# paurrodri/DuplexUMIConsensusReads

Hardware: AMD Instinct MI355X
Metric: consensus bases/sec (whole node) + SSCS kernel HBM GB/s vs peak, 1/2/4/8 GPUs (higher is better)
Workload: dtype f64

## Files before the change

### duplexumiconsensusreads_amd/_lib.py

```python
from __future__ import annotations

import ctypes
import os

import numpy as np

from .batch import DcrBatch, DcrOut, DcrReadInfo, OutArrays, PackedBatch
from .params import ConsensusParams, DcrParams, build_dcr_params

HERE = os.path.dirname(os.path.abspath(__file__))
LIB_PATH = os.environ.get("DCR_LIB", os.path.join(HERE, "libdcr.so"))

EXPORTS = {
    "dcr_abi_version": (ctypes.c_int, []),
    "dcr_last_error": (ctypes.c_char_p, []),
    "dcr_create": (ctypes.c_void_p, [ctypes.c_int, ctypes.c_void_p]),
    "dcr_destroy": (None, [ctypes.c_void_p]),
    "dcr_set_params": (ctypes.c_int, [ctypes.c_void_p, ctypes.c_void_p]),
    "dcr_set_options": (ctypes.c_int, [ctypes.c_void_p, ctypes.c_int]),
    "dcr_reserve": (ctypes.c_int, [ctypes.c_void_p, ctypes.c_void_p]),
    "dcr_stream": (ctypes.c_void_p, [ctypes.c_void_p]),
    "dcr_run_batch": (ctypes.c_int, [ctypes.c_void_p, ctypes.c_void_p, ctypes.c_void_p, ctypes.c_void_p]),
    "dcr_run_batch_host": (ctypes.c_int, [ctypes.c_void_p, ctypes.c_void_p, ctypes.c_void_p,
                                          ctypes.c_void_p]),
    "dcr_sync": (ctypes.c_int, [ctypes.c_void_p]),
    "dcr_read_info_host": (ctypes.c_int, [ctypes.c_void_p, ctypes.c_void_p, ctypes.c_int64]),
    "dcr_last_timing": (ctypes.c_int, [ctypes.c_void_p, ctypes.c_void_p]),
    "dcr_last_kernel_timing": (ctypes.c_int, [ctypes.c_void_p, ctypes.c_void_p]),
    "dcr_host_alloc": (ctypes.c_void_p, [ctypes.c_size_t]),
    "dcr_host_free": (None, [ctypes.c_void_p]),
    "dcr_submit": (ctypes.c_int, [ctypes.c_void_p, ctypes.c_int, ctypes.c_void_p, ctypes.c_void_p, ctypes.c_void_p,
                                  ctypes.c_void_p]),
    "dcr_wait": (ctypes.c_int, [ctypes.c_void_p, ctypes.c_int]),
    "dcr_submit_write": (ctypes.c_int, [ctypes.c_void_p, ctypes.c_int, ctypes.c_void_p, ctypes.c_void_p,
                                        ctypes.c_void_p]),
    "dcr_wait_write": (ctypes.c_int, [ctypes.c_void_p, ctypes.c_int, ctypes.c_void_p]),
    "dcr_submit_write_ss": (ctypes.c_int, [ctypes.c_void_p, ctypes.c_int, ctypes.c_void_p, ctypes.c_void_p,
                                           ctypes.c_void_p, ctypes.c_void_p, ctypes.c_void_p]),
    "dcr_wait_write_ss": (ctypes.c_int, [ctypes.c_void_p, ctypes.c_int, ctypes.c_void_p, ctypes.c_void_p]),
    "dcr_slot_fetch": (ctypes.c_int, [ctypes.c_void_p, ctypes.c_int, ctypes.c_int, ctypes.c_int64, ctypes.c_int64,
                                      ctypes.c_void_p]),
    "dcr_set_filter": (ctypes.c_int, [ctypes.c_void_p, ctypes.c_void_p]),
    "dcr_slot_filter_out": (ctypes.c_int, [ctypes.c_void_p, ctypes.c_int, ctypes.c_void_p]),
    "dcr_set_base_filter": (ctypes.c_int, [ctypes.c_void_p, ctypes.c_void_p]),
    "dcr_set_base_tags": (ctypes.c_int, [ctypes.c_void_p, ctypes.c_int]),
    "dcr_set_metrics": (ctypes.c_int, [ctypes.c_void_p, ctypes.c_int]),
    "dcr_slot_metrics_out": (ctypes.c_int, [ctypes.c_void_p, ctypes.c_int, ctypes.c_void_p]),
    "dcr_set_base_metrics": (ctypes.c_int, [ctypes.c_void_p, ctypes.c_int]),
    "dcr_slot_base_metrics_out": (ctypes.c_int, [ctypes.c_void_p, ctypes.c_int, ctypes.c_void_p]),
    "dcr_set_mate_overlap": (ctypes.c_int, [ctypes.c_void_p, ctypes.c_int]),
    "dcr_slot_overlap_out": (ctypes.c_int, [ctypes.c_void_p, ctypes.c_int, ctypes.c_void_p]),
    "dcr_set_allele_sites": (ctypes.c_int, [ctypes.c_void_p, ctypes.c_void_p, ctypes.c_int64, ctypes.c_int]),
    "dcr_allele_counts_fetch": (ctypes.c_int, [ctypes.c_void_p, ctypes.c_void_p]),
    "dcr_inflater_create": (ctypes.c_void_p, [ctypes.c_int]),
    "dcr_inflater_destroy": (None, [ctypes.c_void_p]),
    "dcr_inflater_hook": (ctypes.c_int, [ctypes.c_void_p, ctypes.c_void_p]),
    "dcr_inflater_run": (ctypes.c_int, [ctypes.c_void_p, ctypes.c_void_p, ctypes.c_int64, ctypes.c_void_p,
                                        ctypes.c_int32, ctypes.c_void_p, ctypes.c_int64]),
    "dcr_inflater_last": (ctypes.c_int, [ctypes.c_void_p, ctypes.c_void_p, ctypes.c_void_p]),
    "dcr_inflater_totals": (ctypes.c_int, [ctypes.c_void_p, ctypes.c_void_p, ctypes.c_int]),
    "dcr_inflate_stream_open": (ctypes.c_void_p, [ctypes.c_void_p, ctypes.c_void_p]),
    "dcr_inflate_stream_add": (ctypes.c_int, [ctypes.c_void_p, ctypes.c_void_p, ctypes.c_int32, ctypes.c_int32]),
    "dcr_inflate_stream_fetch": (ctypes.c_int, [ctypes.c_void_p, ctypes.c_int64, ctypes.c_int64, ctypes.c_void_p]),
    "dcr_inflate_stream_close": (None, [ctypes.c_void_p]),
}

KERNELS = ("k_recmeta<ss>", "k_consensus_fast<ss>", "k_consensus_exact<ss>", "k_consensus_general<ss>",
           "k_recmeta<ds>", "k_consensus_fast<ds>", "k_consensus_exact<ds>", "k_consensus_general<ds>")

_lib = None

READ_INFO_DTYPE = np.dtype([("seq_start", "<i8"), ("len", "<i4"), ("n_cig", "<i4"), ("status", "<i4"),
                            ("has_ins", "<i4")])
assert READ_INFO_DTYPE.itemsize == ctypes.sizeof(DcrReadInfo)


class DcrError(RuntimeError):
    pass


def load():
    global _lib
    if _lib is None:
        try:
            import torch
        except ImportError:
            pass
        path = os.environ.get("DCR_LIB_PATH", LIB_PATH)
        if not os.path.exists(path):
            raise DcrError(f"{path} not built — run __graft_entry__.build() (hipcc --offload-arch=gfx950)")
        lib = ctypes.CDLL(path)
        for name, (res, args) in EXPORTS.items():
            fn = getattr(lib, name)
            fn.restype = res
            fn.argtypes = args
        if lib.dcr_abi_version() != 1:
            raise DcrError("libdcr.so ABI mismatch")
        _lib = lib
    return _lib


def _check(rc):
    if rc != 0:
        raise DcrError(f"libdcr error {rc}: {load().dcr_last_error().decode()}")


class Context:

    def __init__(self, params: ConsensusParams = ConsensusParams(), device: int = 0, want_info: bool = False):
        lib = load()
        self.params = params
        self._p = build_dcr_params(params)
        self.device = device
        self._ctx = lib.dcr_create(device, ctypes.byref(self._p))
        if not self._ctx:
            raise DcrError(f"dcr_create failed: {lib.dcr_last_error().decode()}")
        self.want_info = want_info
        self.filter = None
        self.metrics = False
        self.base_tags = False
        self.base_metrics = False
        self.mate_overlap = 0
        self.allele_sites = 0
        if want_info:
            _check(lib.dcr_set_options(self._ctx, 1))

    def close(self):
        if getattr(self, "_ctx", None):
            load().dcr_destroy(self._ctx)
            self._ctx = None

    def __del__(self):
        try:
            self.close()
        except Exception:
            pass

    def set_params(self, params: ConsensusParams):
        self.params = params
        self._p = build_dcr_params(params)
        _check(load().dcr_set_params(self._ctx, ctypes.byref(self._p)))

    def set_filter(self, flt):
        if flt == self.filter:
            return
        s = flt.as_struct() if flt is not None else None
        _check(load().dcr_set_filter(self._ctx, ctypes.byref(s) if s is not None else None))
        b = flt.as_base_struct() if flt is not None else None
        _check(load().dcr_set_base_filter(self._ctx, ctypes.byref(b) if b is not None else None))
        self.filter = flt

    def set_metrics(self, on):
        if bool(on) == self.metrics:
            return
        _check(load().dcr_set_metrics(self._ctx, 1 if on else 0))
        self.metrics = bool(on)

    def set_base_tags(self, on):
        if bool(on) == self.base_tags:
            return
        _check(load().dcr_set_base_tags(self._ctx, 1 if on else 0))
        self.base_tags = bool(on)

    def set_base_metrics(self, on):
        if bool(on) == self.base_metrics:
            return
        _check(load().dcr_set_base_metrics(self._ctx, 1 if on else 0))
        self.base_metrics = bool(on)

    def set_mate_overlap(self, mode):
        mode = int(mode or 0)
        if mode == self.mate_overlap:
            return
        _check(load().dcr_set_mate_overlap(self._ctx, mode))
        self.mate_overlap = mode

    def set_allele_sites(self, keys, min_base_quality=0):
        n = 0 if keys is None else len(keys)
        if n == 0:
            if self.allele_sites:
                _check(load().dcr_set_allele_sites(self._ctx, None, 0, 0))
            self.allele_sites = 0
            return
        keys = np.ascontiguousarray(keys, np.int64)
        _check(load().dcr_set_allele_sites(self._ctx, keys.ctypes.data, n, int(min_base_quality)))
        self.allele_sites = n

    def allele_counts(self):
        from .params import ALLELE_COLS
        out = np.zeros((max(self.allele_sites, 1), ALLELE_COLS), np.uint64)
        _check(load().dcr_allele_counts_fetch(self._ctx, out.ctypes.data))
        return out[:self.allele_sites]

    @property
    def stream(self):
        return load().dcr_stream(self._ctx)

    def run_host(self, packed: PackedBatch, want_info=None):
        ss = OutArrays(4 * packed.n_fam, packed.ss_cols)
        ds = OutArrays(2 * packed.n_fam, packed.ds_cols)
        b = packed.as_struct()
        so, do = ss.as_struct(), ds.as_struct()
        _check(load().dcr_run_batch_host(self._ctx, ctypes.byref(b), ctypes.byref(so), ctypes.byref(do)))
        if want_info is None:
            want_info = self.want_info
        info = self.read_info(packed.n_reads) if want_info else None
        return ss, ds, info

    def read_info(self, n):
        arr = np.zeros(max(n, 1), dtype=READ_INFO_DTYPE)
        _check(load().dcr_read_info_host(self._ctx, arr.ctypes.data, n))
        return {k: arr[k][:n].copy() for k in READ_INFO_DTYPE.names}

    def reserve(self, batch_struct: DcrBatch):
        _check(load().dcr_reserve(self._ctx, ctypes.byref(batch_struct)))

    def run_device(self, batch_struct: DcrBatch, ss: DcrOut, ds: DcrOut):
        _check(load().dcr_run_batch(self._ctx, ctypes.byref(batch_struct), ctypes.byref(ss), ctypes.byref(ds)))

    def sync(self):
        _check(load().dcr_sync(self._ctx))

    def last_timing(self):
        ms = (ctypes.c_float * 4)()
        _check(load().dcr_last_timing(self._ctx, ms))
        return dict(prep=ms[0], single_strand=ms[1], duplex=ms[2], total=ms[3])

    def last_kernel_timing(self):
        ms = (ctypes.c_float * len(KERNELS))()
        _check(load().dcr_last_kernel_timing(self._ctx, ms))
        return dict(zip(KERNELS, ms))


BGZF_MEMBER_DTYPE = np.dtype([("in_off", "<i8"), ("out_off", "<i8"), ("in_len", "<u4"), ("isize", "<u4"),
                              ("crc", "<u4"), ("pad", "<u4")])


class InflateHook(ctypes.Structure):
    _fields_ = [("user", ctypes.c_void_p), ("run", ctypes.c_void_p), ("host_alloc", ctypes.c_void_p),
                ("host_free", ctypes.c_void_p), ("stream_open", ctypes.c_void_p), ("stream_add", ctypes.c_void_p),
                ("stream_fetch", ctypes.c_void_p), ("stream_close", ctypes.c_void_p)]


def bgzf_members(data) -> tuple:
    buf = memoryview(data)
    out, p, o = [], 0, 0
    while p < len(buf):
        if bytes(buf[p:p + 4]) != b"\x1f\x8b\x08\x04":
            raise ValueError(f"not a BGZF block at {p}")
        xlen = int.from_bytes(buf[p + 10:p + 12], "little")
        bsize, q = None, p + 12
        while q + 4 <= p + 12 + xlen:
            slen = int.from_bytes(buf[q + 2:q + 4], "little")
            if bytes(buf[q:q + 2]) == b"BC" and slen == 2:
                bsize = int.from_bytes(buf[q + 4:q + 6], "little") + 1
            q += 4 + slen
        if bsize is None:
            raise ValueError("BGZF block without BC field")
        crc = int.from_bytes(buf[p + bsize - 8:p + bsize - 4], "little")
        isize = int.from_bytes(buf[p + bsize - 4:p + bsize], "little")
        out.append((p + 12 + xlen, o, bsize - 12 - xlen - 8, isize, crc, 0))
        o += isize
        p += bsize
    return np.array(out, dtype=BGZF_MEMBER_DTYPE), o


class Inflater:

    def __init__(self, device: int = 0):
        lib = load()
        self.device = device
        self._h = lib.dcr_inflater_create(device)
        if not self._h:
            raise DcrError(f"dcr_inflater_create failed: {lib.dcr_last_error().decode()}")

    @property
    def handle(self):
        return self._h

    def hook(self) -> InflateHook:
        h = InflateHook()
        _check(load().dcr_inflater_hook(self._h, ctypes.byref(h)))
        return h

    def run(self, data, members, out_bytes):
        src = np.frombuffer(data, np.uint8) if not isinstance(data, np.ndarray) else data
        m = np.ascontiguousarray(members, dtype=BGZF_MEMBER_DTYPE)
        out = np.zeros(max(out_bytes, 1), np.uint8)
        rc = load().dcr_inflater_run(self._h, src.ctypes.data, src.nbytes, m.ctypes.data, len(m), out.ctypes.data,
                                     out_bytes)
        if rc < 0:
            raise DcrError(f"dcr_inflater_run: {load().dcr_last_error().decode()}")
        return rc, out[:out_bytes]

    def last(self):
        ms, n = ctypes.c_float(), ctypes.c_int32()
        _check(load().dcr_inflater_last(self._h, ctypes.byref(ms), ctypes.byref(n)))
        return ms.value, n.value

    def totals(self, reset=False):
        out = (ctypes.c_double * 4)()
        _check(load().dcr_inflater_totals(self._h, out, int(reset)))
        return {"kernel_ms": out[0], "runs": int(out[1]), "members": int(out[2]), "bytes": int(out[3])}

    def close(self):
        if getattr(self, "_h", None):
            load().dcr_inflater_destroy(self._h)
            self._h = None

    def __del__(self):
        try:
            self.close()
        except Exception:
            pass


def backend(ctx: Context):
    def run(packed, params):
        if params != ctx.params:
            ctx.set_params(params)
        return ctx.run_host(packed)
    return run
```

### duplexumiconsensusreads_amd/csrc/dcr_inflate.hip

```cpp
#include <hip/hip_runtime.h>

#include <condition_variable>
#include <cstring>
#include <deque>
#include <mutex>
#include <thread>
#include <string>
#include <unordered_map>
#include <vector>

#include "../../include/dcr_inflate.h"
#include "dcr_deflate.h"
#include "dcr_internal.h"
#include "dcr_span_stream.h"

#ifndef DINF_STAMP
#define DINF_STAMP 0
#endif

namespace dinf {

struct IStamp {
    uint64_t t = 0;
    uint32_t acc[8] = {0, 0, 0, 0, 0, 0, 0, 0};
    uint32_t cnt[8] = {0, 0, 0, 0, 0, 0, 0, 0};
    __device__ __forceinline__ void start() {
        if (DINF_STAMP) t = __builtin_amdgcn_s_memtime();
    }
    __device__ __forceinline__ void lap(int k) {
        if (DINF_STAMP) {
            const uint64_t now = __builtin_amdgcn_s_memtime();
            acc[k] += (uint32_t)(now - t);
            t = now;
        }
    }
    __device__ __forceinline__ void count(int k, uint32_t v = 1) {
        if (DINF_STAMP) cnt[k] += v;
    }
};

#ifndef DINF_WG_PER_CU
#define DINF_WG_PER_CU 16
#endif
#ifndef DINF_RING
#define DINF_RING 4096
#endif
#ifndef DINF_LB
#define DINF_LB 9
#endif
constexpr int kW = 64;
constexpr int kLB = DINF_LB;
constexpr int kDB = 8;
constexpr int kCB = 7;
constexpr uint32_t kRing = DINF_RING;
constexpr uint32_t kRM = kRing - 1;
constexpr uint32_t kPiece = kRing / 2;
constexpr uint32_t kStripe = kPiece / kW;
static_assert((kRing & (kRing - 1)) == 0 && kRing >= 2048, "ring: a power of two");
static_assert(kPiece + 322 + 320 <= kRing, "the ring holds the unwritten bytes");
constexpr int kPad = 1024;

enum : uint32_t { K_LIT = 0, K_PAIR = 1, K_LEN = 2, K_EOB = 3, K_DIST = 4, K_BAD = 7 };

enum : uint8_t { ST_OK = 0, ST_STREAM = 1, ST_SIZE = 2, ST_CRC = 3, ST_GUARD = 4 };
constexpr uint32_t kGuard = 1u << 21;

struct alignas(16) WaveLds {
    uint32_t lit[1 << kLB];
    uint32_t dist[1 << kDB];
    uint8_t ring[kRing];
    uint32_t crc_tab[256];
    uint16_t lsym[288], dsym[32];
    uint16_t lcnt[16], dcnt[16];
    uint8_t lens[320];
    uint8_t cl_lens[20];
};

struct Args {
    const uint8_t *in;
    uint8_t *out;
    const dcr_bgzf_member *m;
    uint8_t *status;
    uint32_t *dbg;
    int32_t n;
    uint32_t x8n_piece;
};

__device__ __forceinline__ uint32_t uni(uint32_t v) { return __builtin_amdgcn_readfirstlane(v); }
__device__ __forceinline__ int lane_id() { return (int)(threadIdx.x & (kW - 1)); }
__device__ __forceinline__ uint32_t lane_read(uint32_t v, uint32_t l) {
    return (uint32_t)__builtin_amdgcn_readlane((int)v, (int)l);
}

__device__ __forceinline__ uint32_t lit_entry(uint32_t sym) {
    if (sym < 256) return (K_LIT << 5) | (sym << 8);
    if (sym == 256) return K_EOB << 5;
    if (sym < 286) return (K_LEN << 5) | ((uint32_t)dfl::kLenExtra[sym - 257] << 8) | ((uint32_t)dfl::kLenBase[sym - 257] << 16);
    return K_BAD << 5;
}
__device__ __forceinline__ uint32_t dist_entry(uint32_t sym) {
    if (sym < 30) return (K_DIST << 5) | ((uint32_t)dfl::kDistExtra[sym] << 8) | ((uint32_t)dfl::kDistBase[sym] << 16);
    return K_BAD << 5;
}

template <int TB, int KIND>
__device__ __noinline__ bool build_table(const uint8_t *lens, int n, uint32_t *tab, uint16_t *cnt_out, uint16_t *sym_out) {
    const int lane = lane_id();
    const uint64_t lt = (1ull << lane) - 1;
    uint32_t mycnt = 0;
    for (int c0 = 0; c0 < n; c0 += kW) {
        const int i = c0 + lane;
        const uint32_t l = i < n ? lens[i] : 0;
#pragma unroll
        for (int L = 1; L <= 15; ++L) {
            const uint32_t k = (uint32_t)__popcll(__ballot(l == (uint32_t)L));
            if (lane == L) mycnt += k;
        }
    }
    if (lane == 0) mycnt = 0;
    uint32_t kr = lane >= 1 && lane <= 15 ? mycnt << (15 - lane) : 0;
    for (int d = 32; d >= 1; d >>= 1) kr += __shfl_xor(kr, d, kW);
    kr = uni(kr);
    if (kr > 32768u) return false;
    if (kr != 32768u) {
        const bool one_bit = kr == 16384u && lane_read(mycnt, 1) == 1;
        if (KIND == 2 || !(one_bit || (KIND == 1 && kr == 0))) return false;
    }
    uint32_t offs = 0, first = 0;
#pragma unroll
    for (int l = 1; l <= 15; ++l) {
        const uint32_t cl = lane_read(mycnt, l);
        if (l < lane && lane < 16) {
            offs += cl;
            first += cl << (lane - l);
        }
    }
    if (lane < 16) cnt_out[lane] = (uint16_t)mycnt;
    uint32_t run = offs;
    for (int c0 = 0; c0 < n; c0 += kW) {
        const int i = c0 + lane;
        const uint32_t l = i < n ? lens[i] : 0;
#pragma unroll
        for (int L = 1; L <= 15; ++L) {
            const uint64_t m = __ballot(l == (uint32_t)L);
            const uint32_t base = lane_read(run, L);
            if (l == (uint32_t)L) sym_out[base + __popcll(m & lt)] = (uint16_t)i;
            if (lane == L) run += (uint32_t)__popcll(m);
        }
    }
    uint32_t fL[TB + 1], cL[TB + 1], oL[TB + 1];
#pragma unroll
    for (int L = 1; L <= TB; ++L) {
        fL[L] = lane_read(first, L);
        cL[L] = lane_read(mycnt, L);
        oL[L] = lane_read(offs, L);
    }
    bool any_long = false;
    {
        uint32_t longer = 0;
        for (int l = TB + 1; l <= 15; ++l) longer += lane_read(mycnt, l);
        any_long = longer != 0;
    }
    for (int e = lane; e < (1 << TB); e += kW) {
        const uint32_t c = __builtin_bitreverse32((uint32_t)e) >> (32 - TB);
        uint32_t ent = any_long ? 0u : (K_BAD << 5);
#pragma unroll
// ... 221 lines not shown
                d.nb -= n;
                const uint32_t sym = e >> 8;
                uint32_t rep = 1, val = sym;
                if (sym == 16) {
                    if (i == 0) { st = ST_STREAM; break; }
                    val = uni(s.lens[i - 1]);
                    rep = 3 + getbits(d, 2);
                } else if (sym == 17) {
                    val = 0;
                    rep = 3 + getbits(d, 3);
                } else if (sym == 18) {
                    val = 0;
                    rep = 11 + getbits(d, 7);
                }
                if (i + rep > total) { st = ST_STREAM; break; }
                for (uint32_t r = lane; r < rep; r += kW) s.lens[i + r] = (uint8_t)val;
                i += rep;
            }
            if (st != ST_OK) break;
            if (uni(s.lens[256]) == 0) { st = ST_STREAM; break; }
            if (!uni(build_table<kLB, 0>(s.lens, (int)hlit, s.lit, s.lcnt, s.lsym))) { st = ST_STREAM; break; }
            if (!uni(build_table<kDB, 1>(s.lens + hlit, (int)hdist, s.dist, s.dcnt, s.dsym))) { st = ST_STREAM; break; }
        }
        sp.lap(0);
        for (;;) {
            if (d.nb < 32) refill(d);
            uint32_t e = uni(s.lit[(uint32_t)d.bb & ((1u << kLB) - 1)]);
            uint32_t n = e & 31;
            if (n == 0) {
                const int sym = slow_decode(d, s.lcnt, s.lsym, n);
                if (sym < 0) { st = ST_STREAM; break; }
                e = lit_entry((uint32_t)sym) | n;
            }
            d.bb >>= n;
            d.nb -= n;
            const uint32_t kind = (e >> 5) & 7;
            if (kind == K_LIT || kind == K_PAIR) {
                sp.count(kind == K_PAIR ? 1 : 0);
                o.lbuf = lane == (int)o.nlit ? (e >> 8) & 0xff : o.lbuf;
                ++o.nlit;
                if (kind == K_PAIR) {
                    o.lbuf = lane == (int)o.nlit ? (e >> 16) & 0xff : o.lbuf;
                    ++o.nlit;
                }
                if (o.nlit >= kW - 1) {
                    if (o.opos + o.nlit > o.isize) { st = ST_SIZE; break; }
                    sp.lap(1);
                    flush_lits(s, o);
                    keep_room(o, a, lsh);
                    sp.lap(4);
                }
                continue;
            }
            if (kind == K_EOB) break;
            if (kind != K_LEN) { st = ST_STREAM; break; }
            const uint32_t ex = (e >> 8) & 7;
            const uint32_t len = (e >> 16) + ((uint32_t)d.bb & ((1u << ex) - 1));
            d.bb >>= ex;
            d.nb -= ex;
            if (d.nb < 32) refill(d);
            uint32_t de = uni(s.dist[(uint32_t)d.bb & ((1u << kDB) - 1)]);
            uint32_t dn = de & 31;
            if (dn == 0) {
                const int sym = slow_decode(d, s.dcnt, s.dsym, dn);
                if (sym < 0) { st = ST_STREAM; break; }
                de = dist_entry((uint32_t)sym) | dn;
            }
            if (((de >> 5) & 7) != K_DIST) { st = ST_STREAM; break; }
            d.bb >>= dn;
            d.nb -= dn;
            const uint32_t dex = (de >> 8) & 15;
            const uint32_t dist = (de >> 16) + ((uint32_t)d.bb & ((1u << dex) - 1));
            d.bb >>= dex;
            d.nb -= dex;
            if (o.opos + o.nlit + len > o.isize) { st = ST_SIZE; break; }
            sp.lap(2);
            sp.count(2);
            sp.count(3, len);
            flush_lits(s, o);
            if (dist > o.opos) { st = ST_STREAM; break; }
            if (dist >= kW && dist <= kRingDist) {
                for (uint32_t c0 = 0; c0 < len; c0 += kW) {
                    const uint32_t i = c0 + lane;
                    const uint8_t v = s.ring[(o.opos - dist + i) & kRM];
                    s.ring[(o.opos + i) & kRM] = v;
                }
            } else if (dist < kW) {
                const float rd = __builtin_amdgcn_rcpf((float)dist);
                const uint32_t rep = (uint32_t)lane - dist * (uint32_t)(((float)lane + 0.5f) * rd);
                const uint32_t step = dist * uni((uint32_t)(((float)kW + 0.5f) * rd));
                const uint8_t v = s.ring[(o.opos - dist + rep) & kRM];
                for (uint32_t c0 = 0; c0 < len; c0 += step) s.ring[(o.opos + c0 + lane) & kRM] = v;
            } else {
                asm volatile("s_waitcnt vmcnt(0)" ::: "memory");
                for (uint32_t c0 = 0; c0 < len; c0 += kW) {
                    const uint32_t i = c0 + lane;
                    if (i < len) s.ring[(o.opos + i) & kRM] = o.g[o.opos - dist + i];
                }
            }
            o.opos += len;
            sp.lap(3);
            keep_room(o, a, lsh);
            sp.lap(4);
        }
        sp.lap(1);
        if (st != ST_OK) break;
        if (o.opos + o.nlit > o.isize) { st = ST_SIZE; break; }
        flush_lits(s, o);
        keep_room(o, a, lsh);
    }
    if (st == ST_OK && (bits_used(d) + 7) / 8 > M.in_len) st = ST_STREAM;
    if (st == ST_OK && o.opos != o.isize) st = ST_SIZE;
    if (st == ST_OK) {
        while (o.gpos < o.opos) {
            const uint32_t m = min(kPiece, o.opos - o.gpos);
            o.crc = uni(write_piece(o.g, o.gpos, m, o.crc, lsh, a.x8n_piece));
            o.gpos += m;
        }
        const uint32_t crc = ~(dfl::multmodp(dfl::x8nmodp(o.isize), 0xffffffffu) ^ o.crc);
        if (o.isize == 0) {
            if (M.crc != 0) st = ST_CRC;
        } else if (crc != M.crc) {
            st = ST_CRC;
        }
    }
    sp.lap(5);
    if (DINF_STAMP && lane == 0 && a.dbg) {
        for (int k = 0; k < 6; ++k) a.dbg[16 * mi + k] = sp.acc[k];
        for (int k = 0; k < 4; ++k) a.dbg[16 * mi + 8 + k] = sp.cnt[k];
        a.dbg[16 * mi + 12] = guard;
        a.dbg[16 * mi + 13] = o.opos;
    }
    if (lane == 0) {
        a.status[mi] = st;
        if (a.dbg && !DINF_STAMP) {
            a.dbg[4 * mi] = st | where << 8;
            a.dbg[4 * mi + 1] = bits_used(d);
            a.dbg[4 * mi + 2] = o.opos;
            a.dbg[4 * mi + 3] = guard;
        }
    }
}

__global__ __launch_bounds__(64) void k_inflate(Args a) {
    WaveLds &s = *reinterpret_cast<WaveLds *>(smem);
    const int lane = lane_id();
    for (int i = lane; i < 256; i += kW) s.crc_tab[i] = dfl::crc_byte((uint32_t)i);
    const uint32_t lsh = dfl::x8nmodp(kPiece - kStripe * (uint32_t)(lane + 1));
    for (int mi = (int)blockIdx.x; mi < a.n; mi += (int)gridDim.x) inflate_one(a, s, mi, lsh);
}

}

struct InflSlots {
    static constexpr int kSlots = 4;
    uint8_t *d_in[kSlots] = {}, *d_out[kSlots] = {}, *d_st[kSlots] = {};
    dcr_bgzf_member *d_m[kSlots] = {};
    size_t cap_in[kSlots] = {}, cap_out[kSlots] = {}, cap_m[kSlots] = {}, cap_dst[kSlots] = {};
    uint8_t *h_stage[kSlots] = {}, *h_st[kSlots] = {};
    size_t cap_stage[kSlots] = {}, cap_hst[kSlots] = {};
    hipStream_t s_k = nullptr, s_out = nullptr;
    bool busy = false;
    void release() {
        for (int i = 0; i < kSlots; ++i) {
            if (d_in[i]) (void)hipFree(d_in[i]);
            if (d_out[i]) (void)hipFree(d_out[i]);
            if (d_st[i]) (void)hipFree(d_st[i]);
            if (d_m[i]) (void)hipFree(d_m[i]);
            if (h_stage[i]) (void)hipHostFree(h_stage[i]);
            if (h_st[i]) (void)hipHostFree(h_st[i]);
        }
        if (s_k) (void)hipStreamDestroy(s_k);
        if (s_out) (void)hipStreamDestroy(s_out);
    }
};

struct dcr_inflater {
    int device = 0;
    int grid_cap = 1 << 30;
    int n_cu = 1;
    hipStream_t stream = nullptr;
    hipEvent_t ev0 = nullptr, ev1 = nullptr;
    uint8_t *d_in = nullptr, *d_out = nullptr, *d_st = nullptr;
    dcr_bgzf_member *d_m = nullptr;
    uint32_t *d_dbg = nullptr;
    size_t cap_in = 0, cap_out = 0, cap_m = 0, cap_dbg = 0;
    size_t cap_st = 0;
    dinf::Args base{};
    float last_ms = 0;
    int32_t last_n = 0;
    double tot[4] = {0, 0, 0, 0};
    double stamp[16] = {};
    struct InflSlots *slots = nullptr;
    std::mutex mu;
    std::unordered_multimap<size_t, void *> free_host;
    std::unordered_map<void *, size_t> live_host;
};

namespace {
template <class T>
hipError_t grow(T *&p, size_t &cap, size_t n) {
    if (n <= cap) return hipSuccess;
    if (p) (void)hipFree(p);
    p = nullptr;
    cap = 0;
    hipError_t e = hipMalloc((void **)&p, n * sizeof(T));
    if (e == hipSuccess) cap = n;
    return e;
}
int hip_fail(hipError_t e, const char *what) {
    return dcr::set_error(DCR_EHIP, std::string(what) + ": " + hipGetErrorString(e));
}
}

extern "C" {

dcr_inflater *dcr_inflater_create(int device) {
    int n = 0;
    if (hipGetDeviceCount(&n) != hipSuccess || device < 0 || device >= n) {
        dcr::set_error(DCR_ENODEV, "dcr_inflater_create: no such device");
        return nullptr;
    }
    hipDeviceProp_t prop;
    if (hipGetDeviceProperties(&prop, device) != hipSuccess || std::strncmp(prop.gcnArchName, "gfx950", 6) != 0) {
        dcr::set_error(DCR_ENODEV, "dcr_inflater_create: not a gfx950 device");
        return nullptr;
    }
    auto *h = new dcr_inflater;
    h->device = device;
    if (hipSetDevice(device) != hipSuccess || hipStreamCreateWithFlags(&h->stream, hipStreamNonBlocking) != hipSuccess ||
        hipEventCreate(&h->ev0) != hipSuccess || hipEventCreate(&h->ev1) != hipSuccess ||
        hipFuncSetAttribute((const void *)dinf::k_inflate, hipFuncAttributeMaxDynamicSharedMemorySize,
                            (int)sizeof(dinf::WaveLds)) != hipSuccess) {
        dcr::set_error(DCR_EHIP, "dcr_inflater_create: HIP setup failed");
        dcr_inflater_destroy(h);
        return nullptr;
    }
    h->base.x8n_piece = dfl::x8nmodp(dinf::kPiece);
    h->n_cu = std::max(1, prop.multiProcessorCount);
    if (DINF_WG_PER_CU > 0) h->grid_cap = DINF_WG_PER_CU * h->n_cu;
    return h;
}

void dcr_inflater_destroy(dcr_inflater *h) {
    if (!h) return;
    (void)hipSetDevice(h->device);
    if (h->stream) (void)hipStreamSynchronize(h->stream);
    if (h->d_in) (void)hipFree(h->d_in);
    if (h->d_out) (void)hipFree(h->d_out);
    if (h->d_st) (void)hipFree(h->d_st);
    if (h->d_m) (void)hipFree(h->d_m);
    if (h->d_dbg) (void)hipFree(h->d_dbg);
    for (auto &kv : h->free_host) (void)hipHostFree(kv.second);
    for (auto &kv : h->live_host) (void)hipHostFree(kv.first);
    if (h->slots) {
        h->slots->release();
        delete h->slots;
    }
    if (h->ev0) (void)hipEventDestroy(h->ev0);
    if (h->ev1) (void)hipEventDestroy(h->ev1);
    if (h->stream) (void)hipStreamDestroy(h->stream);
    delete h;
}

int dcr_inflater_run(dcr_inflater *h, const uint8_t *in, int64_t in_bytes, const dcr_bgzf_member *m, int32_t n,
                     uint8_t *out, int64_t out_bytes) {
    if (!h || n < 0 || in_bytes < 0 || out_bytes < 0 || (n && (!in || !m || !out)))
        return -dcr::set_error(DCR_EARG, "dcr_inflater_run: bad arguments");
    if (n == 0) return 0;
    for (int32_t i = 0; i < n; ++i)
        if (m[i].in_off < 0 || m[i].in_off + (int64_t)m[i].in_len > in_bytes || m[i].isize > 65536 ||
            m[i].out_off < 0 || m[i].out_off + (int64_t)m[i].isize > out_bytes)
            return -dcr::set_error(DCR_EARG, "dcr_inflater_run: member " + std::to_string(i) + " outside the buffers");
    std::lock_guard<std::mutex> g(h->mu);
    hipError_t e;
    if ((e = hipSetDevice(h->device)) != hipSuccess) return -hip_fail(e, "hipSetDevice");
    if ((e = grow(h->d_in, h->cap_in, (size_t)in_bytes + dinf::kPad)) != hipSuccess ||
        (e = grow(h->d_out, h->cap_out, (size_t)out_bytes + 16)) != hipSuccess ||
        (e = grow(h->d_m, h->cap_m, (size_t)n)) != hipSuccess ||
        (e = grow(h->d_st, h->cap_st, (size_t)n)) != hipSuccess ||
        (e = grow(h->d_dbg, h->cap_dbg, (size_t)n * (DINF_STAMP ? 16 : 4))) != hipSuccess)
        return -hip_fail(e, "dcr_inflater_run: device buffers");
    std::vector<uint8_t> st((size_t)n);
    hipStream_t s = h->stream;
    if ((e = hipMemcpyAsync(h->d_in, in, (size_t)in_bytes, hipMemcpyHostToDevice, s)) != hipSuccess ||
        (e = hipMemcpyAsync(h->d_m, m, (size_t)n * sizeof(dcr_bgzf_member), hipMemcpyHostToDevice, s)) != hipSuccess)
        return -hip_fail(e, "dcr_inflater_run: upload");
    dinf::Args a = h->base;
    a.in = h->d_in;
    a.out = h->d_out;
    a.m = h->d_m;
    a.status = h->d_st;
    a.dbg = h->d_dbg;
    a.n = n;
    (void)hipEventRecord(h->ev0, s);
    hipLaunchKernelGGL(dinf::k_inflate, dim3((unsigned)std::min(n, h->grid_cap)), dim3(64), sizeof(dinf::WaveLds), s,
                       a);
    if ((e = hipGetLastError()) != hipSuccess) return -hip_fail(e, "k_inflate launch");
    (void)hipEventRecord(h->ev1, s);
    if ((e = hipMemcpyAsync(out, h->d_out, (size_t)out_bytes, hipMemcpyDeviceToHost, s)) != hipSuccess ||
        (e = hipMemcpyAsync(st.data(), h->d_st, (size_t)n, hipMemcpyDeviceToHost, s)) != hipSuccess)
        return -hip_fail(e, "dcr_inflater_run: download");
    if ((e = hipStreamSynchronize(s)) != hipSuccess) return -hip_fail(e, "dcr_inflater_run: sync");
    (void)hipEventElapsedTime(&h->last_ms, h->ev0, h->ev1);
    h->last_n = n;
    h->tot[0] += h->last_ms;
    h->tot[1] += 1;
    h->tot[2] += n;
    h->tot[3] += (double)out_bytes;
    if (DINF_STAMP) {
        std::vector<uint32_t> dbg((size_t)n * 16);
        (void)hipMemcpy(dbg.data(), h->d_dbg, dbg.size() * 4, hipMemcpyDeviceToHost);
        for (int32_t i = 0; i < n; ++i)
            for (int k = 0; k < 16; ++k) h->stamp[k] += dbg[(size_t)i * 16 + k];
    }
    for (int32_t i = 0; i < n; ++i)
        if (st[(size_t)i] != dinf::ST_OK) {
            uint32_t dbg[4] = {0, 0, 0, 0};
            (void)hipMemcpy(dbg, h->d_dbg + 4 * (size_t)i, sizeof(dbg), hipMemcpyDeviceToHost);
            const int k = st[(size_t)i];
            dcr::set_error(DCR_EARG, "BGZF member " + std::to_string(i) +
                                         (k == dinf::ST_CRC    ? ": CRC32 mismatch"
                                          : k == dinf::ST_SIZE ? ": ISIZE mismatch"
                                          : k == dinf::ST_GUARD ? ": decoder iteration guard"
                                                                : ": invalid deflate stream") +
                                         " (loop " + std::to_string(dbg[0] >> 8) + ", input bits " +
                                         std::to_string(dbg[1]) + ", output " + std::to_string(dbg[2]) +
                                         ", iterations " + std::to_string(dbg[3]) + ")");
            return i + 1;
        }
    return 0;
}

int dcr_inflater_last(dcr_inflater *h, float *kernel_ms, int32_t *n_members) {
    if (!h) return dcr::set_error(DCR_EARG, "dcr_inflater_last: null inflater");
    if (kernel_ms) *kernel_ms = h->last_ms;
    if (n_members) *n_members = h->last_n;
    return 0;
}

int dcr_inflater_totals(dcr_inflater *h, double *out4, int reset) {
    if (!h || !out4) return dcr::set_error(DCR_EARG, "dcr_inflater_totals: null argument");
    std::lock_guard<std::mutex> g(h->mu);
    for (int i = 0; i < 4; ++i) out4[i] = h->tot[i];
    if (reset)
        for (double &t : h->tot) t = 0;
    return 0;
}

extern "C" int dcr_inflater_stamps(dcr_inflater *h, double *out16, int reset) {
    if (!h || !out16) return dcr::set_error(DCR_EARG, "dcr_inflater_stamps: null argument");
    std::lock_guard<std::mutex> g(h->mu);
    for (int i = 0; i < 16; ++i) out16[i] = h->stamp[i];
    if (reset)
        for (double &t : h->stamp) t = 0;
    return DINF_STAMP;
}

namespace {
hipError_t pinned_grow(uint8_t *&p, size_t &cap, size_t n) {
    if (n <= cap) return hipSuccess;
    if (p) (void)hipHostFree(p);
    p = nullptr;
    cap = 0;
    hipError_t e = hipHostMalloc((void **)&p, n, hipHostMallocDefault);
    if (e == hipSuccess) cap = n;
    return e;
}

struct HipSpanBackend {
    using Event = hipEvent_t;
    dcr_inflater *h;
    InflSlots &S;
    bool new_events(Event &start, Event &done) {
        return hipEventCreateWithFlags(&done, hipEventBlockingSync) == hipSuccess &&
               hipEventCreate(&start) == hipSuccess;
    }
    void free_events(Event &start, Event &done) {
        if (start) (void)hipEventDestroy(start);
        if (done) (void)hipEventDestroy(done);
        start = done = nullptr;
    }
    bool ensure(int slot, size_t nin, size_t nout, int32_t n) {
        (void)hipSetDevice(h->device);
        return pinned_grow(S.h_stage[slot], S.cap_stage[slot], nin + 16) == hipSuccess &&
               pinned_grow(S.h_st[slot], S.cap_hst[slot], (size_t)n) == hipSuccess &&
               grow(S.d_in[slot], S.cap_in[slot], nin + dinf::kPad) == hipSuccess &&
               grow(S.d_out[slot], S.cap_out[slot], nout + 16) == hipSuccess &&
               grow(S.d_m[slot], S.cap_m[slot], (size_t)n) == hipSuccess &&
               grow(S.d_st[slot], S.cap_dst[slot], (size_t)n) == hipSuccess;
    }
    uint8_t *stage(int slot) { return S.h_stage[slot]; }
    bool launch(int slot, const dcr_bgzf_member *rel, int32_t n, size_t nin, Event start, Event done) {
        dinf::Args a = h->base;
        a.in = S.d_in[slot];
        a.out = S.d_out[slot];
        a.m = S.d_m[slot];
        a.status = S.d_st[slot];
        a.dbg = nullptr;
        a.n = n;
        if (hipMemcpyAsync(S.d_in[slot], S.h_stage[slot], nin, hipMemcpyHostToDevice, S.s_k) != hipSuccess ||
            hipMemcpyAsync(S.d_m[slot], rel, (size_t)n * sizeof(dcr_bgzf_member), hipMemcpyHostToDevice, S.s_k) !=
                hipSuccess ||
            hipEventRecord(start, S.s_k) != hipSuccess)
            return false;
        hipLaunchKernelGGL(dinf::k_inflate, dim3((unsigned)std::min(n, h->grid_cap)), dim3(64), sizeof(dinf::WaveLds),
                           S.s_k, a);
        return hipGetLastError() == hipSuccess &&
               hipMemcpyAsync(S.h_st[slot], S.d_st[slot], (size_t)n, hipMemcpyDeviceToHost, S.s_k) == hipSuccess &&
               hipEventRecord(done, S.s_k) == hipSuccess;
    }
    bool wait(Event start, Event done, float *ms) {
        if (hipEventSynchronize(done) != hipSuccess) return false;
        if (ms) {
            *ms = 0;
            (void)hipEventElapsedTime(ms, start, done);
        }
        return true;
    }
    const uint8_t *status(int slot) { return S.h_st[slot]; }
    bool copy_out(uint8_t *dst, int slot, int64_t off, int64_t n) {
        return hipMemcpyAsync(dst, S.d_out[slot] + off, (size_t)n, hipMemcpyDeviceToHost, S.s_out) == hipSuccess;
    }
    bool sync_out() { return hipStreamSynchronize(S.s_out) == hipSuccess; }
    void drain() {
        (void)hipSetDevice(h->device);
        if (S.s_k) (void)hipStreamSynchronize(S.s_k);
        if (S.s_out) (void)hipStreamSynchronize(S.s_out);
    }
    void account(float ms, int32_t members, int64_t bytes) {
        std::lock_guard<std::mutex> g(h->mu);
        if (members) {
            h->tot[0] += ms;
            h->tot[1] += 1;
            h->tot[2] += members;
        }
        h->tot[3] += (double)bytes;
    }
    void error(const std::string &msg) { dcr::set_error(DCR_EARG, msg); }
};
}

static_assert(InflSlots::kSlots == dcr_span::kSlots, "one device slot per protocol slot");

struct dcr_inflate_stream {
    HipSpanBackend be;
    dcr_span::Stream<HipSpanBackend> s;
    dcr_inflate_stream(dcr_inflater *h, const uint8_t *file) : be{h, *h->slots}, s(be, file) {}
};

extern "C" dcr_inflate_stream *dcr_inflate_stream_open(dcr_inflater *h, const uint8_t *file) {
    if (!h || !file) {
        dcr::set_error(DCR_EARG, "dcr_inflate_stream_open: bad arguments");
        return nullptr;
    }
    {
        std::lock_guard<std::mutex> g(h->mu);
        if (!h->slots) h->slots = new InflSlots;
        if (h->slots->busy) {
            dcr::set_error(DCR_EARG, "dcr_inflate_stream_open: the inflater's stream is in use");
            return nullptr;
        }
        h->slots->busy = true;
    }
    InflSlots &S = *h->slots;
    (void)hipSetDevice(h->device);
    if ((!S.s_k && hipStreamCreateWithFlags(&S.s_k, hipStreamNonBlocking) != hipSuccess) ||
        (!S.s_out && hipStreamCreateWithFlags(&S.s_out, hipStreamNonBlocking) != hipSuccess)) {
        std::lock_guard<std::mutex> g(h->mu);
        S.busy = false;
        dcr::set_error(DCR_EHIP, "dcr_inflate_stream_open: HIP setup failed");
        return nullptr;
    }
    auto *st = new dcr_inflate_stream(h, file);
    st->s.start();
    return st;
}

extern "C" int dcr_inflate_stream_add(dcr_inflate_stream *st, const dcr_bgzf_member *m, int32_t n, int32_t last) {
    if (!st || n < 0 || (n && !m)) return dcr::set_error(DCR_EARG, "dcr_inflate_stream_add: bad arguments");
    for (int32_t i = 0; i < n; ++i)
        if (m[i].isize > 65536 || m[i].in_off < 0 || m[i].out_off < 0)
            return dcr::set_error(DCR_EARG, "dcr_inflate_stream_add: member out of range");
    return st->s.add(m, n, last);
}

extern "C" int dcr_inflate_stream_fetch(dcr_inflate_stream *st, int64_t out_off, int64_t n, uint8_t *dst) {
    if (!st || n < 0 || (n && !dst)) return -1;
    (void)hipSetDevice(st->be.h->device);
    return st->s.fetch(out_off, n, dst);
}

extern "C" void dcr_inflate_stream_close(dcr_inflate_stream *st) {
    if (!st) return;
    st->s.close();
    dcr_inflater *h = st->be.h;
    delete st;
    std::lock_guard<std::mutex> g(h->mu);
    h->slots->busy = false;
}

static void *hook_stream_open(void *u, const uint8_t *file) {
    return dcr_inflate_stream_open((dcr_inflater *)u, file);
}
static int hook_stream_add(void *s, const dcr_bgzf_member *m, int32_t n, int32_t last) {
    return dcr_inflate_stream_add((dcr_inflate_stream *)s, m, n, last);
}
static int hook_stream_fetch(void *s, int64_t off, int64_t n, uint8_t *dst) {
    return dcr_inflate_stream_fetch((dcr_inflate_stream *)s, off, n, dst);
}
static void hook_stream_close(void *s) { dcr_inflate_stream_close((dcr_inflate_stream *)s); }

static int hook_run(void *u, const uint8_t *in, int64_t in_bytes, const dcr_bgzf_member *m, int32_t n, uint8_t *out,
                    int64_t out_bytes) {
    const int r = dcr_inflater_run((dcr_inflater *)u, in, in_bytes, m, n, out, out_bytes);
    return r < 0 ? -1 : r;
}
static void *hook_alloc(void *u, size_t bytes) {
    auto *h = (dcr_inflater *)u;
    std::lock_guard<std::mutex> g(h->mu);
    auto it = h->free_host.find(bytes);
    void *p = nullptr;
    if (it != h->free_host.end()) {
        p = it->second;
        h->free_host.erase(it);
    } else {
        (void)hipSetDevice(h->device);
        if (hipHostMalloc(&p, bytes, hipHostMallocDefault) != hipSuccess) return nullptr;
    }
    h->live_host[p] = bytes;
    return p;
}
static void hook_free(void *u, void *p) {
    auto *h = (dcr_inflater *)u;
    std::lock_guard<std::mutex> g(h->mu);
    auto it = h->live_host.find(p);
    if (it == h->live_host.end()) return;
    h->free_host.emplace(it->second, p);
    h->live_host.erase(it);
}

int dcr_inflater_hook(dcr_inflater *h, dcr_inflate_hook *hook) {
    if (!h || !hook) return dcr::set_error(DCR_EARG, "dcr_inflater_hook: null argument");
    hook->user = h;
    hook->run = hook_run;
    hook->host_alloc = hook_alloc;
    hook->host_free = hook_free;
    hook->stream_open = hook_stream_open;
    hook->stream_add = hook_stream_add;
    hook->stream_fetch = hook_stream_fetch;
    hook->stream_close = hook_stream_close;
    return 0;
}

}
```

### duplexumiconsensusreads_amd/csrc/dcr_ingest.cpp

```cpp
#include <zlib.h>
#include <tmmintrin.h>
#include <sys/stat.h>

#include <cctype>
#include <cmath>
#include <chrono>
#include <condition_variable>
#include <deque>
#include <mutex>
#include <thread>
#include <cstdio>
#include <cstdlib>
#include <cstring>
#include <memory>
#include <string>
#include <vector>

#include "../../include/dcr_io.h"
#include "../../include/dcr_inflate.h"
#include "dcr_host.h"

using namespace dcrh;

namespace {

thread_local std::string g_err;

int fail(int code, const std::string &m) {
    g_err = m;
    return code;
}

struct TLDecomp {
    libdeflate_decompressor *d = nullptr;
    ~TLDecomp() {
        if (d) libdeflate_free_decompressor(d);
    }
    libdeflate_decompressor *get() {
        if (!d) d = libdeflate_alloc_decompressor();
        return d;
    }
};
thread_local TLDecomp tl_dec;

struct PyRandom {
    uint32_t mt[624];
    int index = 625;
    bool seeded = false;

    uint32_t genrand() {
        static const uint32_t mag01[2] = {0x0u, 0x9908b0dfu};
        const int N = 624, M = 397;
        uint32_t y;
        if (index >= N) {
            int kk;
            for (kk = 0; kk < N - M; kk++) {
                y = (mt[kk] & 0x80000000u) | (mt[kk + 1] & 0x7fffffffu);
                mt[kk] = mt[kk + M] ^ (y >> 1) ^ mag01[y & 1u];
            }
            for (; kk < N - 1; kk++) {
                y = (mt[kk] & 0x80000000u) | (mt[kk + 1] & 0x7fffffffu);
                mt[kk] = mt[kk + (M - N)] ^ (y >> 1) ^ mag01[y & 1u];
            }
            y = (mt[N - 1] & 0x80000000u) | (mt[0] & 0x7fffffffu);
            mt[N - 1] = mt[M - 1] ^ (y >> 1) ^ mag01[y & 1u];
            index = 0;
        }
        y = mt[index++];
        y ^= (y >> 11);
        y ^= (y << 7) & 0x9d2c5680u;
        y ^= (y << 15) & 0xefc60000u;
        y ^= (y >> 18);
        return y;
    }
    static int bit_length(uint32_t n) {
        int k = 0;
        while (n) { ++k; n >>= 1; }
        return k;
    }
    uint32_t randbelow(uint32_t n) {
        if (!n) return 0;
        const int k = bit_length(n);
        uint32_t r = genrand() >> (32 - k);
        while (r >= n) r = genrand() >> (32 - k);
        return r;
    }
    void sample(int n, int k, std::vector<int> &out) {
        out.assign((size_t)k, 0);
        long setsize = 21;
        if (k > 5) setsize += (long)std::pow(4.0, std::ceil(std::log((double)k * 3) / std::log(4.0)));
        if (n <= setsize) {
            std::vector<int> pool((size_t)n);
            for (int i = 0; i < n; ++i) pool[(size_t)i] = i;
            for (int i = 0; i < k; ++i) {
                const int j = (int)randbelow((uint32_t)(n - i));
                out[(size_t)i] = pool[(size_t)j];
                pool[(size_t)j] = pool[(size_t)(n - i - 1)];
            }
        } else {
            std::vector<char> sel((size_t)n, 0);
            for (int i = 0; i < k; ++i) {
                int j = (int)randbelow((uint32_t)n);
                while (sel[(size_t)j]) j = (int)randbelow((uint32_t)n);
                sel[(size_t)j] = 1;
                out[(size_t)i] = j;
            }
        }
    }
};

struct SeqTable {
    uint16_t pair[256];
    SeqTable() {
        const char *a = "=ACMGRSVTWYHKDBN";
        for (int b = 0; b < 256; ++b) pair[b] = (uint16_t)((uint8_t)a[b >> 4] | ((uint8_t)a[b & 15] << 8));
    }
};
const SeqTable kSeq;

inline void decode_seq(const uint8_t *s, int32_t l_seq, uint8_t *d) {
    const int32_t half = l_seq >> 1;
    int32_t i = 0;
    const __m128i tab = _mm_loadu_si128((const __m128i *)"=ACMGRSVTWYHKDBN");
    const __m128i m = _mm_set1_epi8(15);
    for (; i + 16 <= half; i += 16) {
        const __m128i v = _mm_loadu_si128((const __m128i *)(s + i));
        const __m128i hi = _mm_shuffle_epi8(tab, _mm_and_si128(_mm_srli_epi16(v, 4), m));
        const __m128i lo = _mm_shuffle_epi8(tab, _mm_and_si128(v, m));
        _mm_storeu_si128((__m128i *)(d + 2 * i), _mm_unpacklo_epi8(hi, lo));
        _mm_storeu_si128((__m128i *)(d + 2 * i + 16), _mm_unpackhi_epi8(hi, lo));
    }
    for (; i < half; ++i) std::memcpy(d + 2 * i, &kSeq.pair[s[i]], 2);
    if (l_seq & 1) d[l_seq - 1] = (uint8_t)(kSeq.pair[s[half]] & 0xff);
}

struct Rec {
    size_t off;
    uint32_t len;
    int32_t tid, pos;
    uint16_t flag, n_cig;
    uint8_t mapq;
    int32_t l_seq;
    uint32_t o_cig, o_seq, o_qual;
    uint32_t o_mi, o_rx;
    uint16_t l_mi, l_rx;
    uint8_t mi_type, rx_type;
    uint16_t l_code;
    int8_t pf;
    uint8_t fmsg;
    uint8_t perr;
    uint8_t eqx;
    int8_t subk;
    int64_t end_kept;
    char code[24];
};

const char *const kParseErr[] = {"", "malformed BAM record (l_seq < 0)",
                                 "malformed BAM record (fields past block_size)",
                                 "malformed BAM aux field (unterminated string)", "malformed BAM aux array",
                                 "malformed BAM aux field type", "malformed BAM aux field (past block_size)"};
struct FilterMsg { int kind; const char *msg; };
const FilterMsg kFilterMsg[] = {
    {0, ""},
    {DCR_ERR_EXIT, "ERROR: family code tag (MI) not found in file"},
    {DCR_ERR_EXIT, "ERROR: family code tag (RX) not found in file"},
    {DCR_ERR_TYPE, "argument of type 'NoneType' is not iterable"},
    {DCR_ERR_EXIT, "ERROR: unexpected symbols (P, N, B, *) were found in CIGAR strings."},
    {DCR_ERR_EXIT, "ERROR: softclips (S) found in the middle of the read."}};

inline void copy_read(const uint8_t *w, size_t rec, dcr_host_batch *b, int64_t i, int64_t dst_base, int64_t dst_cig) {
    const uint8_t *r = w + rec + 4;
    const uint32_t l_rn = r[8];
    const uint32_t n_cig = rd16(r + 12);
// ... 109 lines not shown
        return (fl & 1) && (fl & 2) && !(fl & 4) && !(fl & 8) && !(fl & 2048) && !(fl & 512) &&
               (int)r.mapq >= min_map_quality;
    }

    int32_t clip_total(const uint8_t *wb, const Rec &r) const {
        const uint8_t *c = at(wb, r, r.o_cig);
        const int n = r.n_cig;
        if (n == 0) return 0;
        auto op = [&](int i) { return (int)(rd32(c + 4 * i) & 15); };
        auto ln = [&](int i) { return (int32_t)(rd32(c + 4 * i) >> 4); };
        const int first = 0, last = n - 1;
        int32_t c5 = 0;
        if (op(first) == 4) c5 = ln(first);
        else if (op(first) == 5 && n > 1 && op(first + 1) == 4) c5 = ln(first + 1);
        const int i5 = op(first) == 4 ? first : first + 1;
        int c3i = -1;
        if (op(last) == 4) c3i = last;
        else if (op(last) == 5 && n > 1) c3i = last - 1;
        int32_t c3 = 0;
        if (c3i >= first && op(c3i) == 4 && !(c5 > 0 && c3i == i5)) c3 = ln(c3i);
        return c5 + c3;
    }

    bool eqx_after_trim(const uint8_t *wb, const Rec &r) const {
        const uint8_t *c = at(wb, r, r.o_cig);
        bool any = false;
        for (uint32_t i = 0; i < r.n_cig; ++i) {
            const uint32_t op = rd32(c + 4 * i) & 15;
            any |= (op == 7 || op == 8);
        }
        if (!any || r.l_seq == 0) return false;
        int32_t s5 = 0, s3 = 0;
        bool inseq = false, modified = false;
        int64_t expanded = 0;
        for (uint32_t i = 0; i < r.n_cig; ++i) {
            const uint32_t w = rd32(c + 4 * i), op = w & 15, ln = w >> 4;
            if (op == 5) modified = true;
            else if (op == 4) {
                modified = true;
                if (!inseq) s5 = (int32_t)ln; else s3 = (int32_t)ln;
            } else {
                inseq = true;
                expanded += ln;
            }
        }
        (void)modified;
        int32_t b = s5, e = r.l_seq - s3;
        if (s3 == 0) e = r.l_seq;
        if (e < b) e = b;
        const uint8_t *sq = at(wb, r, r.o_seq), *ql = at(wb, r, r.o_qual);
        int32_t tn = 0;
        for (int32_t i = e - 1; i >= b; --i) {
            const int code = (sq[i >> 1] >> ((i & 1) ? 0 : 4)) & 15;
            if (code == 15 || (int)ql[i] < min_base_quality) ++tn;
            else break;
        }
        int64_t keep = expanded - tn;
        if (keep < 0) keep = std::max<int64_t>(0, expanded + keep);
        int64_t pos = 0;
        for (uint32_t i = 0; i < r.n_cig && pos < keep; ++i) {
            const uint32_t w = rd32(c + 4 * i), op = w & 15, ln = w >> 4;
            if (op == 4 || op == 5) continue;
            if (op == 7 || op == 8) return true;
            pos += ln;
        }
        return false;
    }

};

struct FamSum {
    int64_t n = 0, nb = 0, nc = 0, bytes = 0;
    int64_t cnt[4] = {0, 0, 0, 0}, nbk[4] = {0, 0, 0, 0}, nck[4] = {0, 0, 0, 0};
    int64_t mn[4] = {0, 0, 0, 0}, mx[4] = {0, 0, 0, 0};
    int16_t eqx[4] = {0, 0, 0, 0};
    const Rec *first[4] = {nullptr, nullptr, nullptr, nullptr};

    void add(const Rec *r) {
        ++n;
        nb += r->l_seq;
        nc += r->n_cig;
        bytes += r->len;
        const int k = r->subk;
        if (k < 0) return;
        if (!first[k]) {
            first[k] = r;
            mn[k] = r->pos;
            mx[k] = r->end_kept;
        } else {
            if (r->pos < mn[k]) mn[k] = r->pos;
            if (r->end_kept > mx[k]) mx[k] = r->end_kept;
        }
        ++cnt[k];
        nbk[k] += r->l_seq;
        nck[k] += r->n_cig;
        if (eqx[k] < 0x7fff && r->eqx) ++eqx[k];
    }
    void append(const FamSum &b) {
        n += b.n;
        nb += b.nb;
        nc += b.nc;
        bytes += b.bytes;
        for (int k = 0; k < 4; ++k) {
            if (!b.first[k]) continue;
            if (!first[k]) {
                first[k] = b.first[k];
                mn[k] = b.mn[k];
                mx[k] = b.mx[k];
            } else {
                mn[k] = std::min(mn[k], b.mn[k]);
                mx[k] = std::max(mx[k], b.mx[k]);
            }
            cnt[k] += b.cnt[k];
            nbk[k] += b.nbk[k];
            nck[k] += b.nck[k];
            eqx[k] = (int16_t)std::min(0x7fff, (int)eqx[k] + (int)b.eqx[k]);
        }
    }
};

inline bool same_code(const uint8_t *wb, const Rec &a, const Rec &b) {
    if (a.l_code != b.l_code) return false;
    if (a.l_code <= sizeof a.code) {
        uint64_t x[3], y[3];
        std::memcpy(x, a.code, sizeof x);
        std::memcpy(y, b.code, sizeof y);
        return ((x[0] ^ y[0]) | (x[1] ^ y[1]) | (x[2] ^ y[2])) == 0;
    }
    return std::memcmp(wb + a.off + a.o_mi, wb + b.off + b.o_mi, a.l_code) == 0;
}

struct Run {
    uint32_t first = 0, n = 0;
    bool slow = false;
    bool cont = false;
    FamSum sum;
};
inline bool plain(const Rec &r) { return r.perr == 0 && r.pf == 1 && r.mi_type == 'Z'; }

struct Chunk {
    HugeBuf buf;
    uint8_t *pin = nullptr;
    uint8_t *data() { return pin ? pin : buf.data(); }
    size_t len = 0;
    bool eof = false;
    std::string err;
    bool indexed = false;
    std::vector<Rec> recs;
    std::vector<size_t> offs;
    bool chained = false;
    std::vector<Run> runs;
    std::vector<std::vector<Run>> item_runs;
    std::vector<size_t> item_at;
};

class RecsCache {
  public:
    static RecsCache &get() {
        static RecsCache c;
        return c;
    }
    void take(Chunk &c) {
        std::lock_guard<std::mutex> g(mu_);
        if (spare_.empty()) return;
        Spare &s = spare_.back();
        c.recs = std::move(s.recs);
        c.runs = std::move(s.runs);
        c.item_runs = std::move(s.item_runs);
        spare_.pop_back();
    }
    void give(Chunk &c) {
        std::lock_guard<std::mutex> g(mu_);
        if (spare_.size() >= 16 || c.recs.capacity() == 0) return;
        c.recs.clear();
        c.runs.clear();
        spare_.push_back(Spare{std::move(c.recs), std::move(c.runs), std::move(c.item_runs)});
    }

  private:
    struct Spare {
        std::vector<Rec> recs;
        std::vector<Run> runs;
        std::vector<std::vector<Run>> item_runs;
    };
    std::mutex mu_;
    std::vector<Spare> spare_;
};

class PoolCache {
  public:
    static PoolCache &get() {
        static PoolCache *c = new PoolCache;
        return *c;
    }
    std::unique_ptr<Pool> take(int n) {
        {
            std::lock_guard<std::mutex> g(mu_);
            for (size_t i = 0; i < spare_.size(); ++i)
                if (spare_[i]->size() == std::max(1, n)) {
                    std::unique_ptr<Pool> p = std::move(spare_[i]);
                    spare_.erase(spare_.begin() + (long)i);
                    return p;
                }
        }
        return std::unique_ptr<Pool>(new Pool(n));
    }
    void give(std::unique_ptr<Pool> p) {
        if (!p) return;
        {
            std::lock_guard<std::mutex> g(mu_);
            if (spare_.size() < 16) {
                spare_.push_back(std::move(p));
                return;
            }
        }
        p.reset();
    }

  private:
    std::mutex mu_;
    std::vector<std::unique_ptr<Pool>> spare_;
};

std::mutex g_hook_mu;
dcr_inflate_hook g_hook{};
bool g_hook_set = false;

inline int env_threads(const char *name, int dflt) {
    const char *v = std::getenv(name);
    const int n = v ? std::atoi(v) : 0;
    return n > 0 ? std::min(n, 64) : dflt;
}

class Inflater {
  public:
    static constexpr size_t kHead = (size_t)8 << 20;
    static constexpr size_t kWant = (size_t)32 << 20;
    static constexpr size_t kWantGpu = (size_t)64 << 20;

    Inflater(FILE *f, int n_threads, const RecParser &rp, bool ranged = false, uint64_t start_coff = 0,
             uint32_t start_uoff = 0, int64_t end_coff = -1, uint32_t end_uoff = 0, bool host_only = false)
        : f_(f), pool_(PoolCache::get().take(env_threads("DCR_INFLATE_THREADS", n_threads))),
          spool_(PoolCache::get().take(env_threads("DCR_SCAN_THREADS", std::max(1, n_threads / 2)))), rp_(rp),
          end_coff_(end_coff),
          end_uoff_(end_uoff) {
        for (auto &c : chunks_) RecsCache::get().take(c);
        if (ranged) {
            st_ = kRec;
            skip_ = start_uoff;
        }
        struct stat sb;
        const int fd = fileno(f_);
        if (fd >= 0 && fstat(fd, &sb) == 0 && S_ISREG(sb.st_mode) && sb.st_size > 0) {
            void *p = mmap(nullptr, (size_t)sb.st_size, PROT_READ, MAP_PRIVATE, fd, 0);
            if (p != MAP_FAILED) {
                map_ = (const uint8_t *)p;
                map_len_ = (size_t)sb.st_size;
                cbeg_ = ranged ? (size_t)std::min<uint64_t>(start_coff, map_len_) : 0;
                cend_ = map_len_;
                file_eof_ = true;
            }
        }
        if (!map_) {
            if (ranged) {
                std::fseek(f_, (long)start_coff, SEEK_SET);
                cpos_ = start_coff;
            }
            cbuf_.resize((size_t)48 << 20);
        }
        {
            std::lock_guard<std::mutex> g(g_hook_mu);
            const char *e = std::getenv("DCR_GPU_INFLATE");
            if (g_hook_set && !host_only && !(e && std::strcmp(e, "0") == 0)) {
                hook_ = g_hook;
                gpu_ = true;
            }
        }
        want_max_ = gpu_ ? kWantGpu : kWant;
        for (auto &c : chunks_) {
            if (gpu_ && hook_.host_alloc) c.pin = (uint8_t *)hook_.host_alloc(hook_.user, kHead + want_max_ + 0x10000);
            if (!c.pin) c.buf.resize(kHead + want_max_ + 0x10000);
            empty_.push_back(&c);
        }
        if (const char *he = std::getenv("DCR_HOST_CHUNK_EVERY")) host_every_ = std::max(0, std::atoi(he));
        if (gpu_ && map_ && hook_.stream_open) open_stream();
        if (gpu_ && !stream_) {
            stage_cap_ = want_max_ + ((size_t)1 << 20);
            if (hook_.host_alloc) stage_pin_ = (uint8_t *)hook_.host_alloc(hook_.user, stage_cap_);
            if (!stage_pin_) stage_.resize(stage_cap_);
        }
        th_ = std::thread([this] { loop(); });
        sth_ = std::thread([this] { scan_loop(); });
        pth_ = std::thread([this] { parse_loop(); });
    }
    ~Inflater() {
        {
            std::lock_guard<std::mutex> g(mu_);
            stop_ = true;
        }
        cv_.notify_all();
        th_.join();
        sth_.join();
        pth_.join();
        stop_members_ = true;
        if (mth_.joinable()) mth_.join();
        if (stream_) hook_.stream_close(stream_);
        if (map_) {
            uint8_t *p = (uint8_t *)map_;
            const size_t len = map_len_;
            std::thread([p, len] {
                constexpr size_t kSlice = (size_t)16 << 20;
                for (size_t o = 0; o < len; o += kSlice) munmap(p + o, std::min(kSlice, len - o));
            }).detach();
        }
        if (hook_.host_free) {
            for (auto &c : chunks_)
                if (c.pin) hook_.host_free(hook_.user, c.pin);
            if (stage_pin_) hook_.host_free(hook_.user, stage_pin_);
        }
        for (auto &c : chunks_) RecsCache::get().give(c);
        PoolCache::get().give(std::move(pool_));
        PoolCache::get().give(std::move(spool_));
    }
    bool gpu() const { return gpu_; }

    void open_stream() {
        stream_ = hook_.stream_open(hook_.user, map_);
        if (!stream_) return;
        stream_out_ = 0;
        const size_t p0 = cbeg_, p_end = cend_;
        mth_ = std::thread([this, p0, p_end] { scan_members(p0, p_end); });
    }
    bool host_chunk(size_t k) const { return host_every_ > 1 && k % (size_t)host_every_ == (size_t)host_every_ - 1; }
    void scan_members(size_t p, const size_t cend) {
        std::vector<dcr_bgzf_member> ms;
        int64_t out = 0;
        size_t batch = 128;
        size_t ck = 0, ctotal = 0, cwant = want_;
        auto flush = [&](bool last) {
            hook_.stream_add(stream_, ms.data(), (int32_t)ms.size(), last ? 1 : 0);
            ms.clear();
        };
        while (p + 18 <= cend && !stop_members_.load(std::memory_order_relaxed)) {
            if (end_coff_ >= 0 && p >= (uint64_t)end_coff_) {
                if (p != (uint64_t)end_coff_ || end_uoff_ == 0) break;
            }
            const uint8_t *h = map_ + p;
            if (h[0] != 0x1f || h[1] != 0x8b || h[2] != 8 || !(h[3] & 4)) break;
            const size_t xlen = rd16(h + 10);
            if (cend - p < 12 + xlen) break;
            long bsize = -1;
            for (size_t i = 0; i + 4 <= xlen;) {
                const uint8_t *sf = h + 12 + i;
                const size_t slen = rd16(sf + 2);
                if (sf[0] == 66 && sf[1] == 67 && slen == 2) bsize = rd16(sf + 4);
                i += 4 + slen;
            }
            if (bsize < 0) break;
            const size_t blen = (size_t)bsize + 1;
            if (blen < 12 + xlen + 8 || cend - p < blen) break;
            const uint32_t isize = rd32(h + blen - 4);
            if (isize > 0x10000) break;
            if (ctotal + 0x10000 > cwant) {
                ++ck;
                ctotal = 0;
                cwant = want_max_;
            }
            ctotal += isize;
            if (!host_chunk(ck)) {
                ms.push_back(dcr_bgzf_member{(int64_t)(p + 12 + xlen), out, (uint32_t)(blen - 12 - xlen - 8), isize,
                                             rd32(h + blen - 8), 0});
                out += isize;
            }
            const bool last_of_range = end_coff_ >= 0 && p == (uint64_t)end_coff_;
            p += blen;
            if (last_of_range) break;
            if (ms.size() >= batch) {
                flush(false);
                batch = 1024;
            }
        }
        flush(true);
    }

    Chunk *next() {
        std::unique_lock<std::mutex> lk(mu_);
        cv_.wait(lk, [&] { return !full_.empty(); });
        Chunk *c = full_.front();
        full_.pop_front();
        return c;
    }
    void give_back(Chunk *c) {
        {
            std::lock_guard<std::mutex> g(mu_);
            empty_.push_back(c);
        }
        cv_.notify_all();
    }
    double scan_s = 0, index_parse_s = 0, runs_s = 0;

  private:
    void loop() {
        for (;;) {
            Chunk *c;
            {
                std::unique_lock<std::mutex> lk(mu_);
                cv_.wait(lk, [&] { return stop_ || !empty_.empty(); });
                if (stop_) return;
                c = empty_.front();
                empty_.pop_front();
            }
            fill(*c);
            const bool last = c->eof || !c->err.empty();
            {
                std::lock_guard<std::mutex> g(mu_);
                inflated_.push_back(c);
            }
            cv_.notify_all();
            if (last) return;
        }
    }
    void scan_loop() {
        for (;;) {
            Chunk *c;
            {
                std::unique_lock<std::mutex> lk(mu_);
                cv_.wait(lk, [&] { return stop_ || !inflated_.empty(); });
                if (stop_) return;
                c = inflated_.front();
                inflated_.pop_front();
            }
            chain(*c);
            const bool last = c->eof || !c->err.empty();
            {
                std::lock_guard<std::mutex> g(mu_);
                chained_.push_back(c);
            }
            cv_.notify_all();
            if (last) return;
        }
    }
    void parse_loop() {
        for (;;) {
            Chunk *c;
            {
                std::unique_lock<std::mutex> lk(mu_);
                cv_.wait(lk, [&] { return stop_ || !chained_.empty(); });
                if (stop_) return;
                c = chained_.front();
                chained_.pop_front();
            }
            parse(*c);
            const bool last = c->eof || !c->err.empty();
            {
                std::lock_guard<std::mutex> g(mu_);
                full_.push_back(c);
            }
            cv_.notify_all();
            if (last) return;
        }
    }

    void chain(Chunk &c) {
        c.recs.clear();
        c.runs.clear();
        c.indexed = false;
        c.chained = false;
        std::vector<size_t> &offs_ = c.offs;
        offs_.clear();
        if (dead_ || !c.err.empty()) { dead_ = true; return; }
        const double t0 = prof_ ? now() : 0;
        const uint8_t *d = c.data() + kHead;
        const size_t n = c.len;
        size_t pos = 0;
        auto field = [&](uint32_t &v) -> bool {
            while (nfld_ < 4 && pos < n) fld_[nfld_++] = d[pos++];
            if (nfld_ < 4) return false;
            v = rd32(fld_);
            nfld_ = 0;
            return true;
        };
        for (;;) {
            if (skip_) {
                const size_t a = (size_t)std::min<uint64_t>(skip_, n - pos);
                pos += a;
                skip_ -= a;
                if (skip_) break;
            }
            uint32_t v;
            if (st_ == kRec) {
                if (nfld_ == 0) {
                    while (pos + 4 <= n) {
                        __builtin_prefetch(d + pos + 16384);
                        __builtin_prefetch(d + pos + 16384 + 64);
                        __builtin_prefetch(d + pos + 16384 + 128);
                        __builtin_prefetch(d + pos + 16384 + 192);
                        const int32_t bs = rdi32(d + pos);
                        if (bs < 32) { dead_ = true; return; }
                        if (pos + 4 + (size_t)bs > n) break;
                        offs_.push_back(pos);
                        pos += 4 + (size_t)bs;
                    }
                    if (pos + 4 <= n) {
                        skip_ = pos + 4 + (uint64_t)(uint32_t)rdi32(d + pos) - n;
                        pos = n;
                        break;
                    }
                }
                if (!field(v)) break;
                if ((int32_t)v < 32) { dead_ = true; return; }
                skip_ = v;
                continue;
            }
            if (!field(v)) break;
            const int32_t iv = (int32_t)v;
            switch (st_) {
                case kMagic:
                    if (v != 0x014d4142u) { dead_ = true; return; }
                    st_ = kLText;
                    break;
                case kLText:
                    if (iv < 0) { dead_ = true; return; }
                    skip_ = v;
                    st_ = kNRef;
                    break;
                case kNRef:
                    if (iv < 0) { dead_ = true; return; }
                    nref_left_ = iv;
                    st_ = nref_left_ ? kLName : kRec;
                    break;
                default:
                    if (iv < 0) { dead_ = true; return; }
                    skip_ = (uint64_t)v + 4;
                    st_ = --nref_left_ ? kLName : kRec;
                    break;
            }
        }
        c.chained = true;
        if (prof_) scan_s += now() - t0;
    }
    void parse(Chunk &c) {
        if (!c.chained) return;
        const double t1 = prof_ ? now() : 0;
        const std::vector<size_t> &offs_ = c.offs;
        c.recs.resize(offs_.size());
        const std::vector<Rec> &R = c.recs;
        const uint8_t *base = c.data();
        const size_t chunk = 512;
        const size_t items = (offs_.size() + chunk - 1) / chunk;
        if (c.item_runs.size() < items) c.item_runs.resize(items);
        spool_->run(items, [&](size_t k) {
            const size_t b = k * chunk, e = std::min(offs_.size(), (k + 1) * chunk);
            for (size_t i = b; i < e; ++i)
                c.recs[i].perr = (uint8_t)rp_.parse_at(base, kHead + offs_[i], c.recs[i]);
            std::vector<Run> &L = c.item_runs[k];
            L.clear();
            for (size_t i = b; i < e; ++i) {
                const Rec &r = R[i];
                const bool pl = plain(r);
                if (i == b || !pl || !plain(R[i - 1]) || !same_code(base, r, R[i - 1])) {
                    L.emplace_back();
                    L.back().first = (uint32_t)i;
                    L.back().slow = !pl;
                }
                ++L.back().n;
                L.back().sum.add(&r);
            }
            return true;
        });
        const double t2 = prof_ ? now() : 0;
        c.item_at.resize(items + 1);
        size_t total = 0;
        for (size_t k = 0; k < items; ++k) {
            std::vector<Run> &L = c.item_runs[k];
            const size_t b = k * chunk;
            L[0].cont = k > 0 && !L[0].slow && plain(R[b - 1]) && same_code(base, R[b], R[b - 1]);
            c.item_at[k] = total;
            total += L.size() - (L[0].cont ? 1 : 0);
        }
        c.item_at[items] = total;
        c.runs.resize(total);
        spool_->run(items, [&](size_t k) {
            const std::vector<Run> &L = c.item_runs[k];
            size_t at = c.item_at[k];
            for (size_t j = L[0].cont ? 1 : 0; j < L.size(); ++j) {
                Run &u = c.runs[at++];
                u = L[j];
                if (j + 1 < L.size()) continue;
                for (size_t m = k + 1; m < items && c.item_runs[m][0].cont; ++m) {
                    u.n += c.item_runs[m][0].n;
                    u.sum.append(c.item_runs[m][0].sum);
                    if (c.item_runs[m].size() > 1) break;
                }
            }
            return true;
        });
        c.indexed = true;
        if (prof_) {
            index_parse_s += t2 - t1;
            runs_s += now() - t2;
        }
    }
    static double now() {
        return std::chrono::duration<double>(std::chrono::steady_clock::now().time_since_epoch()).count();
    }

    void top_up() {
        cpos_ += cbeg_;
        std::memmove(cbuf_.data(), cbuf_.data() + cbeg_, cend_ - cbeg_);
        cend_ -= cbeg_;
        cbeg_ = 0;
        while (!file_eof_ && cend_ < cbuf_.size()) {
            const size_t got = std::fread(cbuf_.data() + cend_, 1, cbuf_.size() - cend_, f_);
            cend_ += got;
            if (got == 0) file_eof_ = true;
        }
    }
    void fill(Chunk &c) {
        c.len = 0;
        c.eof = false;
        c.err.clear();
        struct Blk { size_t coff, clen, doff; uint32_t isize, crc; };
        std::vector<Blk> blks;
        size_t total = 0, cut = SIZE_MAX;
        if (range_done_) { c.eof = true; return; }
        if (!file_eof_ && cend_ - cbeg_ < cbuf_.size() / 2) top_up();
        for (;;) {
            while (!range_done_ && cend_ - cbeg_ >= 18 && total + 0x10000 <= want_) {
                if (end_coff_ >= 0 && cpos_ + cbeg_ >= (uint64_t)end_coff_) {
                    range_done_ = true;
                    if (cpos_ + cbeg_ != (uint64_t)end_coff_ || end_uoff_ == 0) break;
                    cut = total + end_uoff_;
                }
                const uint8_t *h = cdata() + cbeg_;
                if (h[0] != 0x1f || h[1] != 0x8b || h[2] != 8 || !(h[3] & 4)) { c.err = "not a BGZF file"; return; }
                const size_t xlen = rd16(h + 10);
                if (cend_ - cbeg_ < 12 + xlen) break;
                long bsize = -1;
                for (size_t i = 0; i + 4 <= xlen;) {
                    const uint8_t *sf = h + 12 + i;
                    const size_t slen = rd16(sf + 2);
                    if (sf[0] == 66 && sf[1] == 67 && slen == 2) bsize = rd16(sf + 4);
                    i += 4 + slen;
                }
                if (bsize < 0) { c.err = "BGZF block without BC field"; return; }
                const size_t blen = (size_t)bsize + 1;
                if (blen < 12 + xlen + 8) { c.err = "BGZF block size too small"; return; }
                if (cend_ - cbeg_ < blen) break;
                Blk b;
                b.coff = cbeg_ + 12 + xlen;
                b.clen = blen - 12 - xlen - 8;
                b.crc = rd32(h + blen - 8);
                b.isize = rd32(h + blen - 4);
                if (b.isize > 0x10000) { c.err = "BGZF ISIZE above 64 KiB"; return; }
                b.doff = Inflater::kHead + total;
                total += b.isize;
                blks.push_back(b);
                cbeg_ += blen;
            }
            if (!blks.empty() || range_done_) break;
            if (file_eof_) {
                if (cend_ > cbeg_) { c.err = "truncated BGZF block at the end of the file"; return; }
                break;
            }
            top_up();
        }
        uint8_t *dst = c.data();
        const uint8_t *src = cdata();
        auto host_inflate = [&](size_t i) {
            const Blk &b = blks[i];
            if (b.isize == 0) return b.clen <= 2;
            size_t got = 0;
            if (libdeflate_deflate_decompress(tl_dec.get(), src + b.coff, b.clen, dst + b.doff, b.isize, &got) != 0 ||
                got != b.isize)
                return false;
            return libdeflate_crc32(0, dst + b.doff, b.isize) == b.crc;
        };
        bool ok = true;
        const bool host_k = stream_ && !blks.empty() && host_chunk(fill_k_);
        if (!blks.empty()) ++fill_k_;
        if (host_k) {
            ok = pool_->run(blks.size(), host_inflate);
        } else if (stream_ && !blks.empty()) {
            const size_t out_blocks = blks.back().doff + blks.back().isize - kHead;
            const int rc = hook_.stream_fetch(stream_, stream_out_, (int64_t)out_blocks, dst + kHead);
            if (rc != 0) {
                c.err = rc > 0 ? "BGZF block failed to inflate or CRC mismatch" : "GPU inflate failed";
                return;
            }
            stream_out_ += (int64_t)out_blocks;
            if (host_every_ > 1 && libdeflate_crc32(0, dst + blks[0].doff, blks[0].isize) != blks[0].crc) {
                c.err = "GPU inflate stream out of step with the reader";
                return;
            }
        } else if (gpu_ && !blks.empty()) {
            const size_t n = blks.size();
            const size_t k = std::min(n, std::max<size_t>(1, (size_t)(frac_ * (double)n + 0.5)));
            const size_t g0 = blks[0].coff, g1 = blks[k - 1].coff + blks[k - 1].clen;
            const size_t nb = g1 - g0;
            uint8_t *stage = stage_pin_ ? stage_pin_ : stage_.data();
            if (nb > stage_cap_) { c.err = "BGZF chunk larger than its staging buffer"; return; }
            const size_t piece = (size_t)1 << 20;
            pool_->run((nb + piece - 1) / piece, [&](size_t q) {
                const size_t a = q * piece, m = std::min(piece, nb - a);
                std::memcpy(stage + a, src + g0 + a, m);
                return true;
            });
            mem_.resize(k);
            for (size_t i = 0; i < k; ++i) {
                const Blk &b = blks[i];
                mem_[i] = dcr_bgzf_member{(int64_t)(b.coff - g0), (int64_t)(b.doff - kHead), (uint32_t)b.clen,
                                          b.isize, b.crc, 0};
            }
            const size_t out_k = blks[k - 1].doff + blks[k - 1].isize - kHead;
            int rc = 0;
            double t_gpu = 0, t_host = 0;
            std::thread gt([&] {
                const double t0 = now();
                rc = hook_.run(hook_.user, stage, (int64_t)nb, mem_.data(), (int32_t)k, dst + kHead, (int64_t)out_k);
                t_gpu = now() - t0;
            });
            const double th = now();
            if (k < n) ok = pool_->run(n - k, [&](size_t i) { return host_inflate(k + i); });
            t_host = now() - th;
            gt.join();
            if (rc != 0) {
                c.err = rc > 0 ? "BGZF block failed to inflate or CRC mismatch" : "GPU inflate failed";
                return;
            }
            if (k < n && t_gpu > 0 && t_host > 0) {
                frac_ *= std::sqrt(t_host / t_gpu);
                frac_ = std::min(0.95, std::max(0.05, frac_));
            } else if (k == n && t_gpu > 0) {
                frac_ = 0.95;
            }
        } else {
            ok = pool_->run(blks.size(), host_inflate);
        }
        if (!ok) { c.err = "BGZF block failed to inflate or CRC mismatch"; return; }
        c.len = total;
        if (blks.empty() && file_eof_ && cend_ == cbeg_) c.eof = true;
        want_ = want_max_;
        if (range_done_) {
            if (cut != SIZE_MAX) {
                if (cut > total) { c.err = "range end past the end of its BGZF block"; return; }
                c.len = cut;
            }
            c.eof = true;
        }
    }

    FILE *f_;
    std::unique_ptr<Pool> pool_, spool_;
    RecParser rp_;
    int64_t end_coff_;
    uint32_t end_uoff_;
    uint64_t cpos_ = 0;
    const uint8_t *map_ = nullptr;
    size_t map_len_ = 0;
    const uint8_t *cdata() const { return map_ ? map_ : cbuf_.data(); }
    bool range_done_ = false;
    size_t want_ = (size_t)4 << 20;
    size_t want_max_ = kWant;
    bool gpu_ = false;
    dcr_inflate_hook hook_{};
    uint8_t *stage_pin_ = nullptr;
    HugeBuf stage_;
    size_t stage_cap_ = 0;
    std::vector<dcr_bgzf_member> mem_;
    void *stream_ = nullptr;
    std::thread mth_;
    std::atomic<bool> stop_members_{false};
    int64_t stream_out_ = 0;
    double frac_ = 0.5;
    int host_every_ = 0;
    size_t fill_k_ = 0;
    HugeBuf cbuf_;
    size_t cbeg_ = 0, cend_ = 0;
    bool file_eof_ = false;
    Chunk chunks_[5];
    std::deque<Chunk *> empty_, inflated_, chained_, full_;
    std::mutex mu_;
    std::condition_variable cv_;
    bool stop_ = false;
    std::thread th_, sth_, pth_;
    enum { kMagic, kLText, kNRef, kLName, kRec } st_ = kMagic;
    uint8_t fld_[4] = {0, 0, 0, 0};
    int nfld_ = 0;
    uint64_t skip_ = 0;
    int32_t nref_left_ = 0;
    bool dead_ = false;
    const bool prof_ = std::getenv("DCR_INGEST_PROF") != nullptr;
};

struct IngestProf {
    bool on = std::getenv("DCR_INGEST_PROF") != nullptr;
    double wait_chunk = 0, scan = 0, parse = 0, walk_total = 0, complete = 0, tasks_wait = 0;
    double walk_in = 0, prefetch = 0;
    int64_t indexed = 0;
    int64_t fams = 0, run_fams = 0;
    static double now() {
        return std::chrono::duration<double>(std::chrono::steady_clock::now().time_since_epoch()).count();
    }
};

struct dcr_ingest {
    FILE *f = nullptr;
    IngestProf prof;
    dcr_ingest_cfg cfg{};
    std::unique_ptr<Pool> pool;
    std::unique_ptr<Pool> ppool;
    std::unique_ptr<Inflater> infl;
    RecParser rp;
    const uint8_t *wb = nullptr;
    size_t wpos = 0, wend = 0;
    Chunk *cur = nullptr;
    size_t ci = 0;
    HugeBuf big[2];
    int big_i = 0;
    bool data_eof = false;
    std::vector<uint8_t> header;
    std::vector<const Rec *> fam;
    std::vector<Rec> fam_store;
    std::string umi2_;
    bool mid_end = false;
    std::vector<int32_t> sample_calls;
    dcr_state_gate_fn gate_fn = nullptr;
    void *gate_user = nullptr;
    bool gate_open = false;
    bool started = false;
    bool finished = false;
    bool errored = false;
    int64_t passed = 0, excluded = 0, processed = 0, filtered = 0, records = 0;
    PyRandom rng;
    std::vector<int> idx_tmp;

    ~dcr_ingest() {
        pk_stop_thread();
        if (prof.on)
            std::fprintf(stderr,
                         "[ingest] walk %.3f s: chunk wait %.3f, serial scan %.3f, parse %.3f, "
                         "families %.3f, family tasks wait %.3f, record loop %.3f; scanner stage: chain %.3f, "
                         "parse %.3f, runs %.3f; indexed records %lld of %lld; run path %lld of %lld families\n",
                         prof.walk_total, prof.wait_chunk, prof.scan, prof.parse, prof.complete, prof.tasks_wait,
                         prof.walk_in - prof.prefetch - prof.complete, infl ? infl->scan_s : 0.0,
                         infl ? infl->index_parse_s : 0.0, infl ? infl->runs_s : 0.0, (long long)prof.indexed,
                         (long long)records, (long long)prof.run_fams, (long long)prof.fams);
        infl.reset();
        if (f) std::fclose(f);
        PoolCache::get().give(std::move(pool));
        PoolCache::get().give(std::move(ppool));
    }

    int need(size_t n) {
        while (wend - wpos < n) {
            if (data_eof) return 0;
            {
                const size_t keep0 = fam.empty() ? wpos : std::min(wpos, fam.front()->off);
                if (!cur || wend - keep0 > Inflater::kHead) {
                    if (flush_tasks() < 0) return -1;
                } else {
                    kick_tasks(true);
                    release_retired();
                }
            }
            const double tw = prof.on ? IngestProf::now() : 0;
            Chunk *nx = infl->next();
            if (prof.on) prof.wait_chunk += IngestProf::now() - tw;
            if (!nx->err.empty()) {
                g_err = nx->err;
                data_eof = true;
                return -1;
            }
            const size_t keep = fam.empty() ? wpos : std::min(wpos, fam.front()->off);
            const size_t left = wend - keep;
            size_t base;
            const uint8_t *nbuf;
            if (left <= Inflater::kHead) {
                base = Inflater::kHead - left;
                if (left) std::memcpy(nx->data() + base, wb + keep, left);
                nbuf = nx->data();
            } else {
                HugeBuf &bg = big[big_i];
                big_i ^= 1;
                bg.resize(left + nx->len + 16);
                std::memcpy(bg.data(), wb + keep, left);
                std::memcpy(bg.data() + left, nx->data() + Inflater::kHead, nx->len);
                base = 0;
                nbuf = bg.data();
            }
            for (auto &r : fam_store) r.off = r.off - keep + base;
            wpos = wpos - keep + base;
            wend = base + left + nx->len;
            wb = nbuf;
            if (cur) {
                if (tasks.size() > tk_done_seen()) retired.push_back(Retired{cur, tasks.size()});
                else infl->give_back(cur);
            }
            ci = 0;
            if (nbuf == nx->data()) cur = nx;
            else { cur = nullptr; infl->give_back(nx); }
            if (nx->eof) data_eof = true;
        }
        return 1;
    }

    dcr_host_batch *hb = nullptr;
    std::thread pk_th;
    std::mutex pk_mu;
    std::condition_variable pk_cv;
    size_t tk_sub = 0, tk_done = 0;
    static constexpr size_t kTkReads = 8192, kItemReads = 1024;
    size_t tk_reads = 0;
    size_t tk_unchecked = 0;
    bool pk_quit = false;
    dcr_host_batch *pk_b = nullptr;

    void pk_start_thread() {
        pk_th = std::thread([this] {
            for (;;) {
                size_t t0, t1;
                dcr_host_batch *b;
                {
                    std::unique_lock<std::mutex> lk(pk_mu);
                    pk_cv.wait(lk, [&] { return pk_quit || tk_sub > tk_done; });
                    if (pk_quit) return;
// ... 853 lines not shown
    int32_t n_ref = 0;
    {
        SplitReader rd;
        rd.f = f;
        rd.fsize = fsize;
        if (!rd.have(12) || std::memcmp(rd.data.data(), "BAM\1", 4) != 0) return fail(DCR_IO_EFORMAT, "not a BAM file");
        const size_t l_text = (size_t)rdi32(rd.data.data() + 4);
        if (!rd.have(12 + l_text)) return fail(DCR_IO_EFORMAT, "truncated BAM header");
        n_ref = rdi32(rd.data.data() + 8 + l_text);
    }
    RecParser rp;
    rp.min_map_quality = cfg->min_map_quality;
    rp.min_base_quality = cfg->min_base_quality;
    int64_t last = 0;
    for (int32_t part = 1; part < n_parts; ++part) {
        SplitReader rd;
        rd.f = f;
        rd.fsize = fsize;
        uint64_t b0;
        if (!rd.find_block(fsize * (uint64_t)part / (uint64_t)n_parts, b0) || b0 == 0) continue;
        rd.next = b0;
        size_t c = SIZE_MAX;
        for (size_t o = 0; o < 0x20000 && rd.have(o + 36); ++o) {
            size_t q = o, nx;
            int k = 0;
            while (k < 8 && record_ok(rd, q, n_ref, nx)) { q = nx; ++k; }
            if (k == 8) { c = o; break; }
        }
        if (c == SIZE_MAX) continue;
        std::string prev;
        bool have_prev = false;
        size_t found = SIZE_MAX;
        for (size_t o = c, nx; o < ((size_t)64 << 20); o = nx) {
            if (!record_ok(rd, o, n_ref, nx)) break;
            Rec r;
            if (rp.parse_at(rd.data.data(), o, r) != 0 || r.pf < 0) break;
            if (r.pf == 0) continue;
            if (r.mi_type != 'Z') break;
            const char *cp = r.l_code <= sizeof r.code ? r.code : (const char *)rd.data.data() + o + r.o_mi;
            const std::string code(cp, r.l_code);
            if (have_prev && code != prev) { found = o; break; }
            prev = code;
            have_prev = true;
        }
        if (found == SIZE_MAX) continue;
        const int64_t v = rd.voff(found);
        if (v > last) {
            voff[part - 1] = v;
            last = v;
        }
    }
    return DCR_IO_OK;
}

int64_t dcr_bam_header(const char *path, uint8_t *out, int64_t cap) {
    if (!path) { g_err = "NULL argument"; return -1; }
    FILE *f = std::fopen(path, "rb");
    if (!f) { g_err = std::string("cannot open ") + path; return -1; }
    struct Closer { FILE *f; ~Closer() { std::fclose(f); } } closer{f};
    SplitReader rd;
    rd.f = f;
    std::fseek(f, 0, SEEK_END);
    rd.fsize = (uint64_t)std::ftell(f);
    if (!rd.have(12) || std::memcmp(rd.data.data(), "BAM\1", 4) != 0) { g_err = "not a BAM file"; return -1; }
    const int32_t l_text = rdi32(rd.data.data() + 4);
    if (l_text < 0 || !rd.have(12 + (size_t)l_text)) { g_err = "truncated BAM header"; return -1; }
    size_t p = 8 + (size_t)l_text;
    const int32_t n_ref = rdi32(rd.data.data() + p);
    p += 4;
    for (int32_t i = 0; i < n_ref; ++i) {
        if (!rd.have(p + 4)) { g_err = "truncated BAM header"; return -1; }
        const int32_t ln = rdi32(rd.data.data() + p);
        if (ln < 0 || !rd.have(p + 8 + (size_t)ln)) { g_err = "truncated BAM header"; return -1; }
        p += 8 + (size_t)ln;
    }
    if (out && (int64_t)p <= cap) std::memcpy(out, rd.data.data(), p);
    return (int64_t)p;
}

int64_t dcr_ingest_sample_calls(dcr_ingest *ing, int32_t *out, int64_t cap) {
    if (!ing) return -1;
    const int64_t n = (int64_t)ing->sample_calls.size() / 2;
    if (out)
        for (int64_t i = 0; i < std::min(n, cap); ++i) {
            out[2 * i] = ing->sample_calls[(size_t)(2 * i)];
            out[2 * i + 1] = ing->sample_calls[(size_t)(2 * i + 1)];
        }
    return n;
}

int dcr_py_replay(uint32_t *mt, int32_t *index, const int32_t *calls, int64_t n_calls) {
    if (!mt || !index || (n_calls > 0 && !calls) || *index < 0 || *index > 624) return fail(DCR_IO_EARG, "bad arguments");
    PyRandom r;
    std::memcpy(r.mt, mt, sizeof r.mt);
    r.index = *index;
    std::vector<int> v;
    for (int64_t i = 0; i < n_calls; ++i) {
        const int n = calls[2 * i], k = calls[2 * i + 1];
        if (n < 0 || k < 0 || k > n) return fail(DCR_IO_EARG, "bad sample call");
        r.sample(n, k, v);
    }
    std::memcpy(mt, r.mt, sizeof r.mt);
    *index = r.index;
    return DCR_IO_OK;
}

void dcr_ingest_close(dcr_ingest *ing) { delete ing; }

int64_t dcr_ingest_header(dcr_ingest *ing, const uint8_t **bytes) {
    if (!ing || !bytes) return -1;
    *bytes = ing->header.data();
    return (int64_t)ing->header.size();
}

int dcr_ingest_set_rng(dcr_ingest *ing, const uint32_t *mt, int32_t index) {
    if (!ing || !mt || index < 0 || index > 624) return fail(DCR_IO_EARG, "bad RNG state");
    std::memcpy(ing->rng.mt, mt, sizeof ing->rng.mt);
    ing->rng.index = index;
    return DCR_IO_OK;
}

int dcr_ingest_get_rng(dcr_ingest *ing, uint32_t *mt, int32_t *index) {
    if (!ing || !mt || !index) return fail(DCR_IO_EARG, "NULL argument");
    std::memcpy(mt, ing->rng.mt, sizeof ing->rng.mt);
    *index = ing->rng.index;
    return DCR_IO_OK;
}

int dcr_ingest_set_state_gate(dcr_ingest *ing, dcr_state_gate_fn fn, void *user) {
    if (!ing) return fail(DCR_IO_EARG, "NULL argument");
    ing->gate_fn = fn;
    ing->gate_user = user;
    ing->gate_open = false;
    return DCR_IO_OK;
}

int dcr_ingest_next(dcr_ingest *ing, dcr_host_batch *hb) {
    if (!ing || !hb) return fail(DCR_IO_EARG, "NULL argument");
    if (hb->cap_fam < 1 || hb->cap_tab < 1 || hb->cap_reads < 1 || !hb->sub_off || !hb->names)
        return fail(DCR_IO_EARG, "batch capacities not set");
    return ing->next(hb);
}

int dcr_ingest_counters(dcr_ingest *ing, int64_t *out) {
    if (!ing || !out) return fail(DCR_IO_EARG, "NULL argument");
    out[0] = ing->passed;
    out[1] = ing->excluded;
    out[2] = ing->processed;
    out[3] = ing->filtered;
    out[4] = ing->records;
    return DCR_IO_OK;
}

int dcr_py_sample(uint32_t *mt, int32_t *index, int32_t n, int32_t k, int32_t *out) {
    if (!mt || !index || !out || n < 0 || k < 0 || k > n) return fail(DCR_IO_EARG, "bad sample arguments");
    PyRandom r;
    std::memcpy(r.mt, mt, sizeof r.mt);
    r.index = *index;
    std::vector<int> v;
    r.sample(n, k, v);
    for (int i = 0; i < k; ++i) out[i] = v[(size_t)i];
    std::memcpy(mt, r.mt, sizeof r.mt);
    *index = r.index;
    return DCR_IO_OK;
}

}
```

### duplexumiconsensusreads_amd/csrc/dcr_span_stream.h

```cpp
#ifndef DCR_SPAN_STREAM_H
#define DCR_SPAN_STREAM_H

#include <algorithm>
#include <condition_variable>
#include <cstdint>
#include <cstring>
#include <deque>
#include <mutex>
#include <string>
#include <thread>
#include <vector>

#include "../../include/dcr_inflate.h"

namespace dcr_span {

constexpr int kSlots = 4;

constexpr int32_t kSpanMembers = 4096;
constexpr size_t kSpanIn = (size_t)128 << 20;
constexpr size_t kSpanOut = (size_t)kSpanMembers * 65536;

inline int32_t span_members(size_t k) { return k == 0 ? 128 : k == 1 ? 1024 : kSpanMembers; }

template <class B>
struct Stream {
    using Event = typename B::Event;
    struct Span {
        int32_t m0 = 0, m1 = 0;
        int64_t out0 = 0, out1 = 0, in0 = 0, in1 = 0;
        bool launched = false;
        bool checked = false;
        int rc = 0;
        Event start{}, done{};
    };

    B &be;
    const uint8_t *file;
    std::vector<dcr_bgzf_member> m;
    bool m_done = false;
    std::deque<Span> spans;
    std::vector<dcr_bgzf_member> rel[kSlots];
    std::thread producer;
    std::mutex mu;
    std::condition_variable cv;
    int64_t fetched = 0;
    bool stop = false, produced = false;
    int err = 0;

    Stream(B &b, const uint8_t *f) : be(b), file(f) {}
    ~Stream() { close(); }

    void start() {
        for (int slot = 0; slot < kSlots; ++slot)
            if (!be.ensure(slot, kSpanIn, kSpanOut, kSpanMembers)) {
                be.error("dcr_inflate_stream: slot buffers could not be allocated");
                err = -1;
                return;
            }
        producer = std::thread([this] { produce(); });
    }

    int add(const dcr_bgzf_member *mm, int32_t n, int32_t last) {
        {
            std::lock_guard<std::mutex> g(mu);
            m.insert(m.end(), mm, mm + n);
            if (last) m_done = true;
        }
        cv.notify_all();
        return 0;
    }

    void fail_producer() {
        std::lock_guard<std::mutex> g(mu);
        err = -1;
        cv.notify_all();
    }

    void produce() {
        int32_t mnext = 0;
        for (size_t k = 0;; ++k) {
            const int32_t want = span_members(k);
            Span *spp;
            Span *prev = nullptr;
            {
                std::unique_lock<std::mutex> lk(mu);
                cv.wait(lk, [&] { return stop || m_done || (int32_t)m.size() - mnext >= want; });
                if (stop || (m_done && mnext == (int32_t)m.size())) break;
                Span sp;
                sp.m0 = mnext;
                sp.m1 = std::min((int32_t)m.size(), mnext + want);
                for (int32_t i = sp.m0 + 1; i < sp.m1; ++i)
                    if (m[i].in_off > m[i - 1].in_off + (int64_t)m[i - 1].in_len + 64 ||
                        m[i].in_off + (int64_t)m[i].in_len - m[sp.m0].in_off > (int64_t)kSpanIn - 16) {
                        sp.m1 = i;
                        break;
                    }
                sp.out0 = m[sp.m0].out_off;
                sp.out1 = m[sp.m1 - 1].out_off + m[sp.m1 - 1].isize;
                sp.in0 = m[sp.m0].in_off;
                sp.in1 = sp.in0;
                for (int32_t i = sp.m0; i < sp.m1; ++i)
                    sp.in1 = std::max<int64_t>(sp.in1, m[i].in_off + m[i].in_len);
                if (!be.new_events(sp.start, sp.done)) {
                    err = -1;
                    cv.notify_all();
                    return;
                }
                spans.push_back(sp);
                spp = &spans.back();
                if (k >= (size_t)kSlots) {
                    prev = &spans[k - kSlots];
                    cv.wait(lk, [&] { return stop || fetched >= prev->out1; });
                    if (stop) break;
                }
            }
            if (prev && !be.wait(prev->start, prev->done, nullptr)) {
                fail_producer();
                return;
            }
            Span &sp = *spp;
            mnext = sp.m1;
            const int slot = (int)(k % kSlots);
            const int32_t n = sp.m1 - sp.m0;
            const size_t nin = (size_t)(sp.in1 - sp.in0), nout = (size_t)(sp.out1 - sp.out0);
            if (!be.ensure(slot, nin, nout, n)) {
                fail_producer();
                return;
            }
            std::memcpy(be.stage(slot), file + sp.in0, nin);
            auto &r = rel[slot];
            {
                std::lock_guard<std::mutex> g(mu);
                r.assign(m.begin() + sp.m0, m.begin() + sp.m1);
            }
            for (auto &x : r) {
                x.in_off -= sp.in0;
                x.out_off -= sp.out0;
            }
            if (!be.launch(slot, r.data(), n, nin, sp.start, sp.done)) {
                fail_producer();
                return;
            }
            {
                std::lock_guard<std::mutex> g(mu);
                sp.launched = true;
            }
            cv.notify_all();
        }
        std::lock_guard<std::mutex> g(mu);
        produced = true;
        cv.notify_all();
    }

    int fetch(int64_t out_off, int64_t n, uint8_t *dst) {
        if (n == 0) return 0;
        const int64_t end = out_off + n;
        bool queued = false;
        auto leave = [&](int rc) {
            if (queued) be.sync_out();
            return rc;
        };
        for (size_t k = 0;; ++k) {
            Span *spp;
            {
                std::unique_lock<std::mutex> lk(mu);
                cv.wait(lk, [&] { return spans.size() > k || produced || err; });
                if (spans.size() <= k) {
                    if (!err) be.error("dcr_inflate_stream_fetch: range past the stream's members");
                    else be.error("dcr_inflate_stream_fetch: the stream failed");
                    return leave(-1);
                }
                spp = &spans[k];
                if (spp->out0 >= end) break;
                if (spp->out1 <= out_off) continue;
                cv.wait(lk, [&] { return spp->launched || err; });
                if (!spp->launched) return leave(-1);
            }
            Span &sp = *spp;
            const int slot = (int)(k % kSlots);
            if (!sp.checked) {
                float ms = 0;
                if (!be.wait(sp.start, sp.done, &ms)) return leave(-1);
                const uint8_t *st = be.status(slot);
                for (int32_t i = 0; i < sp.m1 - sp.m0; ++i)
                    if (st[i] != 0) {
                        sp.rc = sp.m0 + i + 1;
                        break;
                    }
                sp.checked = true;
                be.account(ms, sp.m1 - sp.m0, 0);
            }
            if (sp.rc) {
                be.error("BGZF member " + std::to_string(sp.rc - 1) + " failed to inflate or CRC mismatch");
                return leave(sp.rc);
            }
            const int64_t a = std::max(out_off, sp.out0), b = std::min(end, sp.out1);
            if (!be.copy_out(dst + (a - out_off), slot, a - sp.out0, b - a)) return leave(-1);
            queued = true;
            if (b == sp.out1) {
                if (!be.sync_out()) return -1;
                queued = false;
                {
                    std::lock_guard<std::mutex> g(mu);
                    fetched = std::max(fetched, sp.out1);
                }
                cv.notify_all();
            }
            if (sp.out1 >= end) break;
        }
        if (queued && !be.sync_out()) return -1;
        {
            std::lock_guard<std::mutex> g(mu);
            fetched = std::max(fetched, end);
        }
        cv.notify_all();
        be.account(0, 0, n);
        return 0;
    }

    void close() {
        {
            std::lock_guard<std::mutex> g(mu);
            stop = true;
        }
        cv.notify_all();
        if (producer.joinable()) producer.join();
        be.drain();
        for (auto &sp : spans) be.free_events(sp.start, sp.done);
        spans.clear();
    }
};

}

#endif
```

### duplexumiconsensusreads_amd/native_io.py

```python
from __future__ import annotations

import ctypes
import os

import numpy as np

from .batch import BATCH_FIELDS, BATCH_DTYPES, DcrBatch, PackedBatch

HERE = os.path.dirname(os.path.abspath(__file__))
LIB_PATH = os.environ.get("DCR_IO_LIB", os.path.join(HERE, "libdcr_io.so"))

_i32, _i64, _vp = ctypes.c_int32, ctypes.c_int64, ctypes.c_void_p

END_FULL, END_EOF, END_ERROR = 0, 1, 2
INGEST_HOST_INFLATE, INGEST_SS_META = 1, 2
ERR_NAMES = {1: "exit", 2: "TypeError", 3: "IndexError", 4: "ValueError", 5: "AttributeError"}
FAM_PROCESSED, FAM_FILTERED = 0, 1
FAIL_NAMES = {1: "IndexError", 2: "TypeError", 3: "ValueError", 4: "OverflowError", 5: "exit",
              7: "UnicodeEncodeError"}


class IngestCfg(ctypes.Structure):
    _fields_ = [("min_map_quality", _i32), ("min_reads", _i32), ("max_reads", _i32),
                ("min_base_quality", _i32), ("n_threads", _i32), ("flags", _i32)]


_HB_ARRAYS = [
    ("sub_off", np.int32, "4f1"), ("read_pos", np.int32, "r"), ("read_mapq", np.uint8, "r"),
    ("seq_off", np.int64, "r"), ("seq_len", np.int32, "r"), ("cig_off", np.int32, "r"),
    ("cig_n", np.int32, "r"), ("cigar", np.uint32, "c"), ("bases", np.uint8, "b"), ("quals", np.uint8, "b"),
    ("ss_col_off", np.int64, "4f1"), ("ds_col_off", np.int64, "2f1"),
    ("fam_tid", np.int32, "f"), ("fam_code", np.int64, "f"), ("fam_rx", np.int64, "2f"),
    ("fam_eqx", np.uint16, "4f"),
    ("tab_kind", np.int32, "t"), ("tab_proc", np.int32, "t"), ("tab_sampled", np.int32, "t"),
    ("tab_code", np.int64, "t"), ("tab_exc_cut", np.int64, "t"), ("tab_filt_cut", np.int64, "t"),
    ("names", np.uint8, "n"), ("side_exc", np.uint8, "s"), ("side_filt", np.uint8, "s"),
    ("sub_flag", np.uint16, "4f"), ("sub_mi", np.int64, "4f"), ("sub_rx", np.int64, "4f"),
]
_SS_META = ("sub_flag", "sub_mi", "sub_rx")


class HostBatchStruct(ctypes.Structure):
    _fields_ = ([("cap_fam", _i32), ("cap_tab", _i32), ("cap_reads", _i32), ("reserved0", _i32),
                 ("cap_cigar", _i64), ("cap_bases", _i64), ("cap_names", _i64), ("cap_side", _i64)]
                + [(n, _vp) for n, _, _ in _HB_ARRAYS]
                + [("n_fam", _i32), ("n_reads", _i32), ("n_cigar", _i64), ("n_bases", _i64),
                   ("ss_cols", _i64), ("ds_cols", _i64), ("n_tab", _i32), ("end_kind", _i32),
                   ("n_names", _i64), ("n_side_exc", _i64), ("n_side_filt", _i64),
                   ("err_kind", _i32), ("reserved1", _i32), ("err_msg", ctypes.c_char * 512)])


class SynthIn(ctypes.Structure):
    _fields_ = [("n_fam", _i32), ("tid", _i32), ("fam_id0", _i64)] + [
        (n, _vp) for n in ("sub_off", "read_pos", "read_mapq", "seq_off", "seq_len", "cig_off", "cig_n", "cigar",
                           "bases", "quals", "umis")]


class FmtOut(ctypes.Structure):
    _fields_ = [(n, _vp) for n in ("status", "pos", "mapq", "len", "n_cig", "n_de", "D", "M", "E", "seq", "qual",
                                   "cigar", "d", "e")]


_lib = None


class IOError_(RuntimeError):
    pass


def load():
    global _lib
    if _lib is None:
        if not os.path.exists(LIB_PATH):
            raise IOError_(f"{LIB_PATH} not built - run __graft_entry__.build()")
        lib = ctypes.CDLL(LIB_PATH)
        sig = {
            "dcr_io_abi_version": (_i32, []),
            "dcr_io_last_error": (ctypes.c_char_p, []),
            "dcr_ingest_open": (_vp, [ctypes.c_char_p, _vp]),
            "dcr_ingest_close": (None, [_vp]),
            "dcr_ingest_header": (_i64, [_vp, ctypes.POINTER(_vp)]),
            "dcr_ingest_set_rng": (_i32, [_vp, _vp, _i32]),
            "dcr_ingest_get_rng": (_i32, [_vp, _vp, _vp]),
            "dcr_ingest_next": (_i32, [_vp, _vp]),
            "dcr_ingest_counters": (_i32, [_vp, _vp]),
            "dcr_py_sample": (_i32, [_vp, _vp, _i32, _i32, _vp]),
            "dcr_bgzw_open": (_vp, [ctypes.c_char_p, _i32, _i32]),
            "dcr_bgzw_write": (_i32, [_vp, _vp, _i64]),
            "dcr_bgzw_close": (_i32, [_vp]),
            "dcr_bgzw_put_blocks": (_i32, [_vp, _vp, _i64, _i64]),
            "dcr_bgzw_sizes": (_i32, [_vp, _vp]),
            "dcr_fmt_scan": (_i32, [_vp, _vp, _vp, _vp, _i32, _vp, _vp]),
            "dcr_fmt_write": (_i32, [_vp, _vp, _vp, _vp, _i32]),
            "dcr_fmt_write_ss": (_i32, [_vp, _vp, _vp, _i32]),
            "dcr_fmt_filter": (_i32, [_vp, _vp, _vp, _vp, _i32, _vp]),
            "dcr_fmt_metrics": (_i32, [_vp, _vp, _vp, _i32, _vp, _vp]),
            "dcr_fmt_mate_overlap": (_i32, [_vp, _vp, _i32, _i32, _vp]),
            "dcr_fmt_allele_counts": (_i32, [_vp, _vp, _vp, ctypes.c_int64, _i32, _i32, _vp, _vp]),
            "dcr_fmt_write_filt": (_i32, [_vp, _vp, _vp, _vp, _i32, _vp]),
            "dcr_fmt_write_ss_filt": (_i32, [_vp, _vp, _vp, _i32, _vp]),
            "dcr_synth_write": (_i32, [_vp, _vp, _i32]),
            "dcr_deflate_emulate": (_i64, [_vp, _i64, _vp]),
            "dcr_deflate_lengths_ab": (_i32, [_vp, _i32, _vp, _vp]),
            "dcr_split_points": (_i32, [ctypes.c_char_p, _i32, _vp, _vp]),
            "dcr_ingest_open_range": (_vp, [ctypes.c_char_p, _vp, _i64, _i64]),
            "dcr_ingest_sample_calls": (_i64, [_vp, _vp, _i64]),
            "dcr_py_replay": (_i32, [_vp, _vp, _vp, _i64]),
            "dcr_bam_header": (_i64, [ctypes.c_char_p, _vp, _i64]),
            "dcr_io_set_inflate_hook": (_i32, [_vp]),
            "dcr_ingest_gpu_inflate": (_i32, [_vp]),
            "dcr_ingest_set_state_gate": (_i32, [_vp, _vp, _vp]),
        }
        for name, (res, args) in sig.items():
            fn = getattr(lib, name)
            fn.restype = res
            fn.argtypes = args
        if lib.dcr_io_abi_version() != 1:
            raise IOError_("libdcr_io.so ABI mismatch")
        _lib = lib
    return _lib


def _err(what):
    return IOError_(f"{what}: {load().dcr_io_last_error().decode(errors='replace')}")


def numpy_alloc(nbytes):
    return np.zeros(max(nbytes, 1), np.uint8)


class HostBatch:

    def __init__(self, reads=1 << 20, avg_len=160, side_bytes=64 << 20, alloc=numpy_alloc, ss_meta=False):
        self.reads = reads
        self.ss_meta = ss_meta
        f = max(reads // 4 + 16, 16)
        t = 2 * f
        caps = {"r": reads, "f": f, "4f": 4 * f, "4f1": 4 * f + 1, "2f": 2 * f, "2f1": 2 * f + 1, "t": t,
                "c": 8 * reads, "b": avg_len * reads, "n": 96 * t + (128 * 4 * f if ss_meta else 0) + (1 << 16),
                "s": side_bytes}
        host_only = {"side_exc", "side_filt", "tab_kind", "tab_proc", "tab_sampled", "tab_code", "tab_exc_cut",
                     "tab_filt_cut"}
        lay, off = [], 0
        for name, dt, ln in _HB_ARRAYS:
            if name in host_only or (name in _SS_META and not ss_meta):
                continue
            nb = np.dtype(dt).itemsize * caps[ln]
            off = (off + 255) & ~255
            lay.append((name, dt, off, caps[ln]))
            off += nb
        self.mem = alloc(off)
        s = HostBatchStruct()
        s.cap_fam, s.cap_tab, s.cap_reads = f, t, reads
        s.cap_cigar, s.cap_bases, s.cap_names, s.cap_side = caps["c"], caps["b"], caps["n"], caps["s"]
        self.a = {}
        base = self.mem.ctypes.data
        for name, dt, o, n in lay:
            self.a[name] = self.mem[o:o + n * np.dtype(dt).itemsize].view(dt)
            setattr(s, name, base + o)
        for name, dt, ln in _HB_ARRAYS:
            if name in host_only:
                self.a[name] = np.empty(caps[ln], dt)
                setattr(s, name, self.a[name].ctypes.data)
        self.s = s

    @property
    def n_fam(self):
        return self.s.n_fam

    @property
    def end_kind(self):
        return self.s.end_kind

    def packed(self) -> PackedBatch:
        s = self.s
        F, n = s.n_fam, s.n_reads
        lens = {"sub_off": 4 * F + 1, "read_pos": n, "read_mapq": n, "seq_off": n, "seq_len": n, "cig_off": n,
                "cig_n": n, "cigar": s.n_cigar, "bases": s.n_bases, "quals": s.n_bases,
                "ss_col_off": 4 * F + 1, "ds_col_off": 2 * F + 1}
        pb = PackedBatch.__new__(PackedBatch)
        for k in BATCH_FIELDS:
            setattr(pb, k, self.a[k][:lens[k]])
        pb.n_fam, pb.n_reads = F, n
        return pb

    def batch_struct(self) -> DcrBatch:
        s = self.s
        b = DcrBatch()
        b.n_fam, b.n_reads, b.n_cigar, b.n_bases = s.n_fam, s.n_reads, s.n_cigar, s.n_bases
        b.ss_cols, b.ds_cols = s.ss_cols, s.ds_cols
        for k in BATCH_FIELDS:
            setattr(b, k, self.a[k].ctypes.data)
        return b

    def name(self, off):
        nm = self.a["names"]
        e = int(off)
        while nm[e] != 0:
            e += 1
        return nm[int(off):e].tobytes().decode("latin-1")

    def table(self):
        s, a = self.s, self.a
        return [(int(a["tab_kind"][t]), int(a["tab_proc"][t]), int(a["tab_sampled"][t]), self.name(a["tab_code"][t]),
                 int(a["tab_exc_cut"][t]), int(a["tab_filt_cut"][t])) for t in range(s.n_tab)]

    def side(self, which):
        n = self.s.n_side_exc if which == "exc" else self.s.n_side_filt
        return self.a["side_exc" if which == "exc" else "side_filt"][:n]

    def error(self):
        return ERR_NAMES.get(self.s.err_kind), self.s.err_msg.decode(errors="replace")


_HOOK = None


def set_inflate_hook(hook):
    global _HOOK
    if load().dcr_io_set_inflate_hook(ctypes.byref(hook) if hook is not None else None) != 0:
        raise _err("set_inflate_hook")
    _HOOK = hook


_GATE_FN = ctypes.CFUNCTYPE(ctypes.c_int, ctypes.c_void_p, ctypes.POINTER(ctypes.c_uint32),
                            ctypes.POINTER(ctypes.c_int32))


class Ingest:

    def __init__(self, path, min_map_quality=20, min_reads=1, max_reads=100, min_base_quality=20, n_threads=0,
                 start_voff=0, end_voff=-1, host_inflate=False, ss_meta=False):
        lib = load()
        cfg = IngestCfg(min_map_quality, min_reads, max_reads, min_base_quality, n_threads,
                        (INGEST_HOST_INFLATE if host_inflate else 0) | (INGEST_SS_META if ss_meta else 0))
        if start_voff == 0 and end_voff == -1:
            self._h = lib.dcr_ingest_open(os.fsencode(path), ctypes.byref(cfg))
        else:
            self._h = lib.dcr_ingest_open_range(os.fsencode(path), ctypes.byref(cfg), int(start_voff), int(end_voff))
        if not self._h:
            raise _err(f"cannot read {path}")
        p = _vp()
        n = lib.dcr_ingest_header(self._h, ctypes.byref(p))
        self.header = ctypes.string_at(p.value, n) if n > 0 else b""

    @property
    def gpu_inflate(self) -> bool:
        return bool(load().dcr_ingest_gpu_inflate(self._h))

    def sample_calls(self):
        lib = load()
        n = lib.dcr_ingest_sample_calls(self._h, None, 0)
        out = np.zeros(2 * max(n, 1), np.int32)
        lib.dcr_ingest_sample_calls(self._h, out.ctypes.data, n)
        return [(int(out[2 * i]), int(out[2 * i + 1])) for i in range(n)]

    def set_rng_state(self, state):
        words = np.asarray(state[1][:624], np.uint32)
        if load().dcr_ingest_set_rng(self._h, words.ctypes.data, int(state[1][624])) != 0:
            raise _err("set_rng")

    def set_state_gate(self, fn):
        lib = load()
        if fn is None:
            self._gate = None
            lib.dcr_ingest_set_state_gate(self._h, None, None)
            return

        def gate(_user, mt, index):
            try:
                st = fn()
                words = np.asarray(st[1][:624], np.uint32)
                ctypes.memmove(mt, words.ctypes.data, 624 * 4)
                index[0] = int(st[1][624])
                return 0
            except BaseException as e:
                self.gate_error = e
                return 1
        self.gate_error = None
        self._gate = _GATE_FN(gate)
        if lib.dcr_ingest_set_state_gate(self._h, ctypes.cast(self._gate, _vp), None) != 0:
            raise _err("set_state_gate")

    def rng_state(self, template):
        words = np.zeros(624, np.uint32)
        idx = ctypes.c_int32()
        if load().dcr_ingest_get_rng(self._h, words.ctypes.data, ctypes.byref(idx)) != 0:
            raise _err("get_rng")
        return (template[0], tuple(int(x) for x in words) + (idx.value,), template[2])

    def next(self, hb: HostBatch) -> HostBatch:
        rc = load().dcr_ingest_next(self._h, ctypes.byref(hb.s))
        if rc != 0:
            raise _err("ingest")
        return hb

    def counters(self):
        out = np.zeros(5, np.int64)
        load().dcr_ingest_counters(self._h, out.ctypes.data)
        return dict(passed=int(out[0]), excluded=int(out[1]), processed=int(out[2]), filtered=int(out[3]),
                    records=int(out[4]))

    def close(self):
        if getattr(self, "_h", None):
            load().dcr_ingest_close(self._h)
            self._h = None

    def __del__(self):
        try:
            self.close()
        except Exception:
            pass


class BgzfWriter:

    def __init__(self, path, header: bytes, level=6, n_threads=0):
        lib = load()
        self._h = lib.dcr_bgzw_open(os.fsencode(path), level, n_threads)
        if not self._h:
            raise _err(f"cannot write {path}")
        try:
            self.write(header)
        except BaseException:
            lib.dcr_bgzw_close(self._h)
            self._h = None
            raise

    def write(self, data):
        if isinstance(data, np.ndarray):
            ptr, n = data.ctypes.data, data.nbytes
        else:
            buf = ctypes.create_string_buffer(bytes(data), len(data))
            ptr, n = ctypes.addressof(buf), len(data)
        if n and load().dcr_bgzw_write(self._h, ptr, n) != 0:
            raise _err("BGZF write")

    def put_blocks(self, blocks: np.ndarray, raw_bytes: int):
        if load().dcr_bgzw_put_blocks(self._h, blocks.ctypes.data, blocks.nbytes, raw_bytes) != 0:
            raise _err("BGZF put_blocks")

    def write_consensus(self, hb: HostBatch, ss: FmtOut, ds: FmtOut, n_fam: int, fam_filt=None):
        if n_fam and load().dcr_fmt_write_filt(self._h, ctypes.byref(hb.s), ctypes.byref(ss), ctypes.byref(ds), n_fam,
                                               fam_filt.ctypes.data if fam_filt is not None else None) != 0:
            raise _err("consensus write")

    def write_consensus_ss(self, hb: HostBatch, ss: FmtOut, n_fam: int, fam_filt=None):
        if n_fam and load().dcr_fmt_write_ss_filt(self._h, ctypes.byref(hb.s), ctypes.byref(ss), n_fam,
                                                  fam_filt.ctypes.data if fam_filt is not None else None) != 0:
            raise _err("single-strand consensus write")

    def write_synthetic(self, packed, umis, fam_id0=0, tid=0, n_threads=0):
        si = SynthIn()
        si.n_fam, si.tid, si.fam_id0 = packed.n_fam, tid, fam_id0
        for k in ("sub_off", "read_pos", "read_mapq", "seq_off", "seq_len", "cig_off", "cig_n", "cigar", "bases",
                  "quals"):
            setattr(si, k, getattr(packed, k).ctypes.data)
        u = np.ascontiguousarray(umis, dtype=np.uint8)
        assert u.size >= 16 * packed.n_fam
        si.umis = u.ctypes.data
        if load().dcr_synth_write(self._h, ctypes.byref(si), n_threads) != 0:
            raise _err("synthetic write")

    def sizes(self):
        out = np.zeros(2, np.int64)
        load().dcr_bgzw_sizes(self._h, out.ctypes.data)
        return int(out[0]), int(out[1])

    def close(self):
        if getattr(self, "_h", None):
            rc = load().dcr_bgzw_close(self._h)
            self._h = None
            if rc != 0:
                raise _err("BGZF close")


def fmt_out(arrays) -> FmtOut:
    o = FmtOut()
    for k, _ in FmtOut._fields_:
        v = arrays[k] if isinstance(arrays, dict) else getattr(arrays, k)
        setattr(o, k, v.ctypes.data if isinstance(v, np.ndarray) else int(v))
    return o


def first_failure(hb: HostBatch, ss: FmtOut, ds: FmtOut, n_fam: int, read_status=None):
    kind, which = ctypes.c_int32(), ctypes.c_int32()
    rs = read_status.ctypes.data if read_status is not None else None
    f = load().dcr_fmt_scan(ctypes.byref(hb.s), ctypes.byref(ss), ctypes.byref(ds), rs, n_fam,
                            ctypes.byref(kind), ctypes.byref(which))
    return f, FAIL_NAMES.get(kind.value), which.value


def apply_filter(hb: HostBatch, ss: FmtOut, ds: FmtOut, flt, n_fam: int) -> np.ndarray:
    out = np.zeros(max(n_fam, 1), np.int32)
    s = flt.as_struct()
    if load().dcr_fmt_filter(ctypes.byref(hb.s), ctypes.byref(ss), ctypes.byref(ds), ctypes.byref(s), n_fam,
                             out.ctypes.data) != 0:
        raise _err("consensus filter")
    return out[:n_fam]


def apply_overlap(hb: HostBatch, ss: FmtOut, ds: FmtOut, mode: int, n_fam: int) -> np.ndarray:
    out = np.zeros(max(3 * n_fam, 1), np.int32)
    if load().dcr_fmt_mate_overlap(ctypes.byref(hb.s), ctypes.byref(ds), int(mode), n_fam, out.ctypes.data) != 0:
        raise _err("mate overlap")
    return out[:3 * n_fam]


def allele_counts(hb: HostBatch, ds: FmtOut, keys, min_base_quality: int, n_fam: int, fam_filt=None,
                  table=None) -> np.ndarray:
    from .params import ALLELE_COLS
    keys = np.ascontiguousarray(keys, np.int64)
    if table is None:
        table = np.zeros((len(keys), ALLELE_COLS), np.uint64)
    assert table.dtype == np.uint64 and table.shape == (len(keys), ALLELE_COLS) and table.flags.c_contiguous
    ff = None if fam_filt is None else np.ascontiguousarray(fam_filt, np.int32)
    if load().dcr_fmt_allele_counts(ctypes.byref(hb.s), ctypes.byref(ds), keys.ctypes.data, len(keys),
                                    int(min_base_quality), n_fam, ff.ctypes.data if ff is not None else None,
                                    table.ctypes.data) != 0:
        raise _err("allele counts")
    return table


def metrics(hb: HostBatch, ss: FmtOut, ds: FmtOut, n_fam: int, fam_fail=None) -> np.ndarray:
    from .params import MET_WORDS
    out = np.zeros(MET_WORDS, np.uint64)
    ff = None if fam_fail is None else np.ascontiguousarray(fam_fail, np.int32)
    if load().dcr_fmt_metrics(ctypes.byref(hb.s), ctypes.byref(ss), ctypes.byref(ds), n_fam,
                              ff.ctypes.data if ff is not None else None, out.ctypes.data) != 0:
        raise _err("consensus metrics")
    return out


def deflate_emulate(data: bytes) -> bytes:
    buf = ctypes.create_string_buffer(bytes(data), len(data))
    out = ctypes.create_string_buffer(65536)
    n = load().dcr_deflate_emulate(buf, len(data), out)
    if n < 0:
        raise IOError_("deflate_emulate: bad input size")
    return out.raw[:n]


def split_points(path, n_parts, params):
    cfg = IngestCfg(params.min_map_quality, params.min_reads, params.max_reads, params.min_base_quality, 0, 0)
    out = np.full(max(n_parts - 1, 1), -1, np.int64)
    if load().dcr_split_points(os.fsencode(path), n_parts, ctypes.byref(cfg), out.ctypes.data) != 0:
        raise _err("split_points")
    return [int(v) for v in out[:n_parts - 1]]


def bam_header(path):
    lib = load()
    n = lib.dcr_bam_header(os.fsencode(path), None, 0)
    if n < 0:
        raise _err(f"cannot read {path}")
# ... 23 lines not shown
```

### include/dcr_inflate.h

```cpp
#ifndef DCR_INFLATE_H
#define DCR_INFLATE_H

#include <stddef.h>
#include <stdint.h>

#ifdef __cplusplus
extern "C" {
#endif

typedef struct dcr_bgzf_member {
    int64_t in_off;
    int64_t out_off;
    uint32_t in_len;
    uint32_t isize;
    uint32_t crc;
    uint32_t pad;
} dcr_bgzf_member;

typedef struct dcr_inflate_hook {
    void *user;
    int (*run)(void *user, const uint8_t *in, int64_t in_bytes, const dcr_bgzf_member *m, int32_t n, uint8_t *out,
               int64_t out_bytes);
    void *(*host_alloc)(void *user, size_t bytes);
    void (*host_free)(void *user, void *p);
    void *(*stream_open)(void *user, const uint8_t *file);
    int (*stream_add)(void *stream, const dcr_bgzf_member *m, int32_t n, int32_t last);
    int (*stream_fetch)(void *stream, int64_t out_off, int64_t n, uint8_t *dst);
    void (*stream_close)(void *stream);
} dcr_inflate_hook;

typedef struct dcr_inflater dcr_inflater;
dcr_inflater *dcr_inflater_create(int device);
void dcr_inflater_destroy(dcr_inflater *h);
int dcr_inflater_hook(dcr_inflater *h, dcr_inflate_hook *hook);
int dcr_inflater_run(dcr_inflater *h, const uint8_t *in, int64_t in_bytes, const dcr_bgzf_member *m, int32_t n,
                     uint8_t *out, int64_t out_bytes);
typedef struct dcr_inflate_stream dcr_inflate_stream;
dcr_inflate_stream *dcr_inflate_stream_open(dcr_inflater *h, const uint8_t *file);
int dcr_inflate_stream_add(dcr_inflate_stream *st, const dcr_bgzf_member *m, int32_t n, int32_t last);
int dcr_inflate_stream_fetch(dcr_inflate_stream *st, int64_t out_off, int64_t n, uint8_t *dst);
void dcr_inflate_stream_close(dcr_inflate_stream *st);
int dcr_inflater_last(dcr_inflater *h, float *kernel_ms, int32_t *n_members);
int dcr_inflater_totals(dcr_inflater *h, double *out4, int reset);

#ifdef __cplusplus
}
#endif
#endif
```

### include/dcr_io.h

```cpp
#ifndef DCR_IO_H
#define DCR_IO_H

#include <stddef.h>
#include <stdint.h>

#ifdef __cplusplus
extern "C" {
#endif

#define DCR_IO_ABI_VERSION 1

enum { DCR_IO_OK = 0, DCR_IO_EARG = 1, DCR_IO_EFILE = 2, DCR_IO_EFORMAT = 3, DCR_IO_ECAPACITY = 4 };

enum {
    DCR_END_FULL = 0,
    DCR_END_EOF = 1,
    DCR_END_ERROR = 2
};

enum {
    DCR_ERR_NONE = 0,
    DCR_ERR_EXIT = 1,
    DCR_ERR_TYPE = 2,
    DCR_ERR_INDEX = 3,
    DCR_ERR_VALUE = 4,
    DCR_ERR_ATTRIBUTE = 5
};

enum { DCR_FAM_PROCESSED = 0, DCR_FAM_FILTERED = 1 };

typedef struct dcr_ingest_cfg {
    int32_t min_map_quality;
    int32_t min_reads;
    int32_t max_reads;
    int32_t min_base_quality;
    int32_t n_threads;
    int32_t flags;
} dcr_ingest_cfg;

#define DCR_INGEST_HOST_INFLATE 1
#define DCR_INGEST_SS_META 2

typedef struct dcr_host_batch {
    int32_t cap_fam;
    int32_t cap_tab;
    int32_t cap_reads;
    int32_t reserved0;
    int64_t cap_cigar;
    int64_t cap_bases;
    int64_t cap_names;
    int64_t cap_side;
    int32_t *sub_off;
    int32_t *read_pos;
    uint8_t *read_mapq;
    int64_t *seq_off;
    int32_t *seq_len;
    int32_t *cig_off;
    int32_t *cig_n;
    uint32_t *cigar;
    uint8_t *bases;
    uint8_t *quals;
    int64_t *ss_col_off;
    int64_t *ds_col_off;
    int32_t *fam_tid;
    int64_t *fam_code;
    int64_t *fam_rx;
    uint16_t *fam_eqx;
    int32_t *tab_kind;
    int32_t *tab_proc;
    int32_t *tab_sampled;
    int64_t *tab_code;
    int64_t *tab_exc_cut;
    int64_t *tab_filt_cut;
    char *names;
    uint8_t *side_exc;
    uint8_t *side_filt;
    uint16_t *sub_flag;
    int64_t *sub_mi;
    int64_t *sub_rx;
    int32_t n_fam, n_reads;
    int64_t n_cigar, n_bases, ss_cols, ds_cols;
    int32_t n_tab, end_kind;
    int64_t n_names, n_side_exc, n_side_filt;
    int32_t err_kind, reserved1;
    char err_msg[512];
} dcr_host_batch;

typedef struct dcr_ingest dcr_ingest;

int dcr_io_abi_version(void);
const char *dcr_io_last_error(void);

dcr_ingest *dcr_ingest_open(const char *path, const dcr_ingest_cfg *cfg);
void dcr_ingest_close(dcr_ingest *ing);
int64_t dcr_ingest_header(dcr_ingest *ing, const uint8_t **bytes);
int dcr_ingest_set_rng(dcr_ingest *ing, const uint32_t *mt624, int32_t index);
int dcr_ingest_get_rng(dcr_ingest *ing, uint32_t *mt624, int32_t *index);
int dcr_ingest_next(dcr_ingest *ing, dcr_host_batch *hb);
int dcr_ingest_counters(dcr_ingest *ing, int64_t *out5);

struct dcr_inflate_hook;
int dcr_io_set_inflate_hook(const struct dcr_inflate_hook *hook);
int dcr_ingest_gpu_inflate(dcr_ingest *ing);

int dcr_split_points(const char *path, int32_t n_parts, const dcr_ingest_cfg *cfg, int64_t *voff);
dcr_ingest *dcr_ingest_open_range(const char *path, const dcr_ingest_cfg *cfg, int64_t start_voff, int64_t end_voff);
int64_t dcr_ingest_sample_calls(dcr_ingest *ing, int32_t *out, int64_t cap);
typedef int (*dcr_state_gate_fn)(void *user, uint32_t *mt624, int32_t *index);
int dcr_ingest_set_state_gate(dcr_ingest *ing, dcr_state_gate_fn fn, void *user);
int dcr_py_replay(uint32_t *mt624, int32_t *index, const int32_t *calls, int64_t n_calls);
int64_t dcr_bam_header(const char *path, uint8_t *out, int64_t cap);

int dcr_py_sample(uint32_t *mt624, int32_t *index, int32_t n, int32_t k, int32_t *out);

typedef struct dcr_bgzw dcr_bgzw;
dcr_bgzw *dcr_bgzw_open(const char *path, int level, int n_threads);
int dcr_bgzw_write(dcr_bgzw *w, const void *bytes, int64_t n);
int dcr_bgzw_put_blocks(dcr_bgzw *w, const void *blocks, int64_t n, int64_t raw_bytes);
int dcr_bgzw_close(dcr_bgzw *w);
int dcr_bgzw_sizes(dcr_bgzw *w, int64_t *out2);

typedef struct dcr_fmt_out {
    const uint8_t *status;
    const int32_t *pos, *mapq, *len, *n_cig, *n_de, *D, *M;
    const double *E;
    const uint8_t *seq, *qual;
    const uint32_t *cigar;
    const uint16_t *d, *e;
} dcr_fmt_out;

enum {
    DCR_FAIL_NONE = 0,
    DCR_FAIL_INDEX = 1, DCR_FAIL_TYPE = 2, DCR_FAIL_VALUE = 3, DCR_FAIL_OVERFLOW = 4,
    DCR_FAIL_EXIT_BADCHAR = 5,
    DCR_FAIL_UNICODE = 7
};

int32_t dcr_fmt_scan(const dcr_host_batch *hb, const dcr_fmt_out *ss, const dcr_fmt_out *ds,
                     const int32_t *read_status, int32_t n_fam, int32_t *kind, int32_t *which);
int dcr_fmt_write(dcr_bgzw *w, const dcr_host_batch *hb, const dcr_fmt_out *ss, const dcr_fmt_out *ds,
                  int32_t n_fam);
int dcr_fmt_write_ss(dcr_bgzw *w, const dcr_host_batch *hb, const dcr_fmt_out *ss, int32_t n_fam);

struct dcr_filter;
int dcr_fmt_filter(const dcr_host_batch *hb, const dcr_fmt_out *ss, const dcr_fmt_out *ds,
                   const struct dcr_filter *filter, int32_t n_fam, int32_t *fam_filt);
int dcr_fmt_write_filt(dcr_bgzw *w, const dcr_host_batch *hb, const dcr_fmt_out *ss, const dcr_fmt_out *ds,
                       int32_t n_fam, const int32_t *fam_filt);
int dcr_fmt_write_ss_filt(dcr_bgzw *w, const dcr_host_batch *hb, const dcr_fmt_out *ss, int32_t n_fam,
                          const int32_t *fam_filt);

int dcr_fmt_mate_overlap(const dcr_host_batch *hb, const dcr_fmt_out *ds, int mode, int32_t n_fam,
                         int32_t *fam_ovl);

int dcr_fmt_allele_counts(const dcr_host_batch *hb, const dcr_fmt_out *ds, const int64_t *keys, int64_t n_keys,
                          int min_base_quality, int32_t n_fam, const int32_t *fam_filt, uint64_t *table);

struct dcr_metrics;
int dcr_fmt_metrics(const dcr_host_batch *hb, const dcr_fmt_out *ss, const dcr_fmt_out *ds, int32_t n_fam,
                    const int32_t *fam_fail, struct dcr_metrics *m);

int64_t dcr_deflate_emulate(const uint8_t *in, int64_t n, uint8_t *out);
int dcr_deflate_lengths_ab(const uint32_t *freq, int m, uint32_t *num_a, uint32_t *num_b);

typedef struct dcr_synth_in {
    int32_t n_fam, tid;
    int64_t fam_id0;
    const int32_t *sub_off, *read_pos;
    const uint8_t *read_mapq;
    const int64_t *seq_off;
    const int32_t *seq_len, *cig_off, *cig_n;
    const uint32_t *cigar;
    const uint8_t *bases, *quals;
    const char *umis;
} dcr_synth_in;
int dcr_synth_write(dcr_bgzw *w, const dcr_synth_in *in, int n_threads);

#ifdef __cplusplus
}
#endif
#endif
```

Baseline: 458.3 million.

## Parse BAM record rows on GPU after inflate to offload host record scanning

Adds a GPU pipeline that runs after BGZF inflate and finds BAM record boundaries. It marks plausible candidates, links each one to its successor, and walks the chain from the known start with pointer doubling. It then parses the reachable records into fixed-size rows that the host ingest can use instead of scanning records itself. This is meant to remove serial host-side record parsing from the ingest path. In exchange it adds many small kernel launches per span, extra device buffers, and a fallback when a span is declined.

```diff
diff --git a/duplexumiconsensusreads_amd/_lib.py b/duplexumiconsensusreads_amd/_lib.py
--- a/duplexumiconsensusreads_amd/_lib.py
+++ b/duplexumiconsensusreads_amd/_lib.py
@@ -63,6 +63,13 @@
     "dcr_inflate_stream_add": (ctypes.c_int, [ctypes.c_void_p, ctypes.c_void_p, ctypes.c_int32, ctypes.c_int32]),
     "dcr_inflate_stream_fetch": (ctypes.c_int, [ctypes.c_void_p, ctypes.c_int64, ctypes.c_int64, ctypes.c_void_p]),
     "dcr_inflate_stream_close": (None, [ctypes.c_void_p]),
+    "dcr_inflate_stream_rows_begin": (ctypes.c_int, [ctypes.c_void_p, ctypes.c_int64, ctypes.c_int32, ctypes.c_int32,
+                                                     ctypes.c_int32]),
+    "dcr_inflate_stream_fetch_rows": (ctypes.c_int, [ctypes.c_void_p, ctypes.c_int64, ctypes.c_int64, ctypes.c_void_p,
+                                                     ctypes.c_void_p, ctypes.c_int64, ctypes.c_void_p]),
+    "dcr_inflater_rec_rows": (ctypes.c_int, [ctypes.c_void_p, ctypes.c_void_p, ctypes.c_int64, ctypes.c_int64,
+                                             ctypes.c_char_p, ctypes.c_int32, ctypes.c_int32, ctypes.c_int32, ctypes.c_void_p,
+                                             ctypes.c_int64, ctypes.c_void_p]),
 }
 
 KERNELS = ("k_recmeta<ss>", "k_consensus_fast<ss>", "k_consensus_exact<ss>", "k_consensus_general<ss>",
@@ -234,12 +241,19 @@
 
 BGZF_MEMBER_DTYPE = np.dtype([("in_off", "<i8"), ("out_off", "<i8"), ("in_len", "<u4"), ("isize", "<u4"),
                               ("crc", "<u4"), ("pad", "<u4")])
+REC_ROW_DTYPE = np.dtype([("off", "<u4"), ("len", "<u4"), ("tid", "<i4"), ("pos", "<i4"), ("l_seq", "<i4"),
+                          ("clip", "<i4"), ("o_mi", "<u4"), ("o_rx", "<u4"), ("flag", "<u2"), ("n_cig", "<u2"),
+                          ("l_mi", "<u2"), ("l_rx", "<u2"), ("l_code", "<u2"), ("l_rn", "u1"), ("mapq", "u1"),
+                          ("mi_type", "u1"), ("rx_type", "u1"), ("fmsg", "u1"), ("perr", "u1"), ("eqx", "u1"),
+                          ("pf", "i1"), ("pad", "<u2"), ("code", "u1", (24,))])
+assert REC_ROW_DTYPE.itemsize == 76
 
 
 class InflateHook(ctypes.Structure):
     _fields_ = [("user", ctypes.c_void_p), ("run", ctypes.c_void_p), ("host_alloc", ctypes.c_void_p),
                 ("host_free", ctypes.c_void_p), ("stream_open", ctypes.c_void_p), ("stream_add", ctypes.c_void_p),
-                ("stream_fetch", ctypes.c_void_p), ("stream_close", ctypes.c_void_p)]
+                ("stream_fetch", ctypes.c_void_p), ("stream_close", ctypes.c_void_p),
+                ("stream_rows_begin", ctypes.c_void_p), ("stream_fetch_rows", ctypes.c_void_p)]
 
 
 def bgzf_members(data) -> tuple:
@@ -293,6 +307,18 @@
             raise DcrError(f"dcr_inflater_run: {load().dcr_last_error().decode()}")
         return rc, out[:out_bytes]
 
+    def rec_rows(self, data, start_off, n_ref, min_map_quality=20, min_base_quality=20, cap=None, part=None):
+        src = np.frombuffer(data, np.uint8) if not isinstance(data, np.ndarray) else data
+        cap = src.nbytes // 36 + 1 if cap is None else cap
+        rows = np.zeros(cap, REC_ROW_DTYPE)
+        out = np.zeros(4, np.int64)
+        rc = load().dcr_inflater_rec_rows(self._h, src.ctypes.data, src.nbytes, int(start_off), part, int(n_ref),
+                                          int(min_map_quality), int(min_base_quality), rows.ctypes.data, cap,
+                                          out.ctypes.data)
+        if rc != 0:
+            raise DcrError(f"dcr_inflater_rec_rows: {load().dcr_last_error().decode()}")
+        return rows[:int(out[1])], dict(status=int(out[0]), candidates=int(out[2]), next_start=int(out[3]))
+
     def last(self):
         ms, n = ctypes.c_float(), ctypes.c_int32()
         _check(load().dcr_inflater_last(self._h, ctypes.byref(ms), ctypes.byref(n)))
diff --git a/duplexumiconsensusreads_amd/csrc/dcr_inflate.hip b/duplexumiconsensusreads_amd/csrc/dcr_inflate.hip
--- a/duplexumiconsensusreads_amd/csrc/dcr_inflate.hip
+++ b/duplexumiconsensusreads_amd/csrc/dcr_inflate.hip
@@ -12,6 +12,7 @@
 #include "../../include/dcr_inflate.h"
 #include "dcr_deflate.h"
 #include "dcr_internal.h"
+#include "dcr_rec_rows.h"
 #include "dcr_span_stream.h"
 
 #ifndef DINF_STAMP
@@ -539,6 +540,266 @@
 
 }
 
+namespace rrd {
+
+constexpr uint32_t kTile = 4096;
+constexpr uint32_t kCap = (uint32_t)(dcr_span::kSpanOut / 128);
+constexpr int kGrid = 1024;
+
+struct Work {
+    uint32_t *cand = nullptr, *jump[2] = {nullptr, nullptr}, *bcnt = nullptr, *roff = nullptr, *memfirst = nullptr;
+    uint8_t *reach = nullptr;
+    dcr_rec_row *rows = nullptr;
+    rr::Meta *meta = nullptr;
+    bool alloc() {
+        const size_t nb = dcr_span::kSpanOut / kTile + 2;
+        return hipMalloc((void **)&cand, (size_t)kCap * 4) == hipSuccess &&
+               hipMalloc((void **)&jump[0], ((size_t)kCap + 1) * 4) == hipSuccess &&
+               hipMalloc((void **)&jump[1], ((size_t)kCap + 1) * 4) == hipSuccess &&
+               hipMalloc((void **)&bcnt, nb * 4) == hipSuccess && hipMalloc((void **)&roff, (size_t)kCap * 4) == hipSuccess &&
+               hipMalloc((void **)&memfirst, ((size_t)dcr_span::kSpanMembers + 1) * 4) == hipSuccess &&
+               hipMalloc((void **)&reach, (size_t)kCap + 1) == hipSuccess &&
+               hipMalloc((void **)&rows, (size_t)kCap * sizeof(dcr_rec_row)) == hipSuccess &&
+               hipMalloc((void **)&meta, sizeof(rr::Meta)) == hipSuccess;
+    }
+    void release() {
+        for (void *p : {(void *)cand, (void *)jump[0], (void *)jump[1], (void *)bcnt, (void *)roff, (void *)memfirst,
+                        (void *)reach, (void *)rows, (void *)meta})
+            if (p) (void)hipFree(p);
+        *this = Work{};
+    }
+};
+
+__device__ __forceinline__ uint32_t wave_excl_scan(uint32_t v, uint32_t &total) {
+    uint32_t x = v;
+    const uint32_t lane = threadIdx.x & 63;
+#pragma unroll
+    for (int o = 1; o < 64; o <<= 1) {
+        const uint32_t y = __shfl_up(x, o, 64);
+        if (lane >= (uint32_t)o) x += y;
+    }
+    total = __shfl(x, 63, 64);
+    return x - v;
+}
+
+__device__ __forceinline__ uint32_t plaus_mask(const uint8_t *d, uint64_t nout, uint64_t t, int32_t n_ref) {
+    if (t >= nout) return 0;
+    const uint4 v = *(const uint4 *)(d + t);
+    uint32_t w[5] = {v.x, v.y, v.z, v.w, 0};
+    if (t + 20 <= nout) w[4] = *(const uint32_t *)(d + t + 16);
+    uint32_t mask = 0;
+#pragma unroll
+    for (int k = 0; k < 16; ++k) {
+        const int q = k >> 2, s = (k & 3) * 8;
+        const uint32_t bs = s ? (w[q] >> s) | (w[q + 1] << (32 - s)) : w[q];
+        if (bs >= 32 && t + (uint64_t)k + 4 + (uint64_t)bs <= nout && rr::plausible(d, nout, t + (uint64_t)k, bs, n_ref))
+            mask |= 1u << k;
+    }
+    return mask;
+}
+
+__global__ void k_begin(const uint8_t *d, uint64_t nout, const rr::Cell *cell, rr::Meta *meta) {
+    rr::Meta m{};
+    m.status = rr::OK;
+    int64_t start = 0;
+    if (!rr::chain_start(d, nout, *cell, start)) m.status = rr::NO_START;
+    m.start = start;
+    *meta = m;
+}
+
+__global__ __launch_bounds__(64) void k_cand_count(const uint8_t *d, uint64_t nout, int32_t n_ref, uint32_t *bcnt) {
+    const uint64_t tile = (uint64_t)blockIdx.x * kTile;
+    uint32_t c = 0;
+#pragma unroll
+    for (int g = 0; g < 4; ++g) c += __popc(plaus_mask(d, nout, tile + ((uint64_t)g * 64 + threadIdx.x) * 16, n_ref));
+    uint32_t total;
+    (void)wave_excl_scan(c, total);
+    if (threadIdx.x == 0) bcnt[blockIdx.x] = total;
+}
+
+__global__ __launch_bounds__(1024) void k_scan(uint32_t *a, uint32_t n, uint32_t cap, uint32_t *total, rr::Meta *meta) {
+    __shared__ uint32_t wsum[16];
+    const uint32_t per = (n + 1023) / 1024;
+    const uint32_t b = threadIdx.x * per, e = min(n, b + per);
+    uint32_t s = 0;
+    for (uint32_t i = b; i < e; ++i) s += a[i];
+    uint32_t wt;
+    uint32_t ex = wave_excl_scan(s, wt);
+    if ((threadIdx.x & 63) == 0) wsum[threadIdx.x >> 6] = wt;
+    __syncthreads();
+    uint32_t wbase = 0, all = 0;
+    for (uint32_t w = 0; w < 16; ++w) {
+        if (w < (threadIdx.x >> 6)) wbase += wsum[w];
+        all += wsum[w];
+    }
+    uint32_t run = wbase + ex;
+    for (uint32_t i = b; i < e; ++i) {
+        const uint32_t v = a[i];
+        a[i] = run;
+        run += v;
+    }
+    if (threadIdx.x == 0) {
+        if (all > cap) {
+            *total = 0;
+            meta->status = rr::OVERFLOW;
+        } else {
+            *total = all;
+        }
+    }
+}
+
+__global__ __launch_bounds__(64) void k_cand_write(const uint8_t *d, uint64_t nout, int32_t n_ref, const uint32_t *bcnt,
+                                                  const rr::Meta *meta, uint32_t *cand) {
+    if (meta->status == rr::OVERFLOW) return;
+    const uint64_t tile = (uint64_t)blockIdx.x * kTile;
+    uint32_t base = bcnt[blockIdx.x];
+#pragma unroll 1
+    for (int g = 0; g < 4; ++g) {
+        const uint64_t t = tile + ((uint64_t)g * 64 + threadIdx.x) * 16;
+        uint32_t mask = plaus_mask(d, nout, t, n_ref);
+        uint32_t total;
+        uint32_t at = base + wave_excl_scan((uint32_t)__popc(mask), total);
+        while (mask) {
+            const int k = __ffs(mask) - 1;
+            mask &= mask - 1;
+            if (at < kCap) cand[at] = (uint32_t)(t + (uint64_t)k);
+            ++at;
+        }
+        base += total;
+    }
+}
+
+__global__ __launch_bounds__(256) void k_link(const uint8_t *d, const uint32_t *cand, const rr::Meta *meta, uint32_t *j0,
+                                             uint32_t *j1, uint8_t *reach) {
+    const uint32_t n = meta->n_cand;
+    for (uint32_t i = blockIdx.x * blockDim.x + threadIdx.x; i < n; i += gridDim.x * blockDim.x) {
+        const uint64_t q = (uint64_t)cand[i] + 4 + (uint64_t)rr::ld32(d + cand[i]);
+        const uint32_t j = rr::lower_bound(cand, n, q);
+        j0[i] = (j < n && (uint64_t)cand[j] == q) ? j : n;
+        reach[i] = 0;
+    }
+    if (blockIdx.x == 0 && threadIdx.x == 0) {
+        j0[n] = n;
+        j1[n] = n;
+        reach[n] = 0;
+    }
+}
+
+__global__ void k_seed(const uint32_t *cand, uint64_t nout, rr::Meta *meta, uint8_t *reach) {
+    const uint32_t n = meta->n_cand;
+    uint32_t seed = n;
+    if (meta->status == rr::OK && meta->start >= 0 && (uint64_t)meta->start < nout) {
+        const uint32_t s = rr::lower_bound(cand, n, (uint64_t)meta->start);
+        if (s < n && (int64_t)cand[s] == meta->start) {
+            seed = s;
+            reach[s] = 1;
+        }
+    }
+    meta->seed = seed;
+}
+
+__global__ __launch_bounds__(256) void k_double(const uint32_t *jin, uint32_t *jout, uint8_t *reach,
+                                               const rr::Meta *meta) {
+    const uint32_t n = meta->n_cand;
+    for (uint32_t i = blockIdx.x * blockDim.x + threadIdx.x; i < n; i += gridDim.x * blockDim.x) {
+        const uint32_t j = jin[i];
+        if (j < n && reach[i]) reach[j] = 1;
+        jout[i] = j < n ? jin[j] : n;
+    }
+}
+
+__global__ __launch_bounds__(64) void k_reach_count(const uint8_t *reach, const rr::Meta *meta, uint32_t *bcnt) {
+    const uint32_t n = meta->n_cand;
+    const uint32_t tile = blockIdx.x * kTile;
+    uint32_t c = 0;
+    for (uint32_t g = 0; g < kTile / 64; ++g) {
+        const uint32_t i = tile + g * 64 + threadIdx.x;
+        c += (i < n && reach[i]) ? 1u : 0u;
+    }
+    uint32_t total;
+    (void)wave_excl_scan(c, total);
+    if (threadIdx.x == 0) bcnt[blockIdx.x] = total;
+}
+
+__global__ __launch_bounds__(64) void k_rows_write(const uint8_t *d, const uint32_t *cand, const uint8_t *reach,
+                                                  const uint32_t *bcnt, rr::Cfg cfg, rr::Meta *meta, dcr_rec_row *rows,
+                                                  uint32_t *roff) {
+    if (meta->status != rr::OK) return;
+    const uint32_t n = meta->n_cand, n_rows = meta->n_rows;
+    const uint32_t tile = blockIdx.x * kTile;
+    if (tile >= n) return;
+    uint32_t base = bcnt[blockIdx.x];
+    for (uint32_t g = 0; g < kTile / 64 && tile + g * 64 < n; ++g) {
+        const uint32_t i = tile + g * 64 + threadIdx.x;
+        const uint32_t f = (i < n && reach[i]) ? 1u : 0u;
+        uint32_t total;
+        const uint32_t j = base + wave_excl_scan(f, total);
+        if (f && j < kCap) {
+            const uint32_t off = cand[i];
+            dcr_rec_row w;
+            rr::row_parse(d + off, off, cfg, w);
+            rows[j] = w;
+            roff[j] = off;
+            if (j + 1 == n_rows) meta->end_q = (int64_t)off + (int64_t)w.len;
+        }
+        base += total;
+    }
+}
+
+__global__ void k_end(const uint8_t *d, uint64_t nout, rr::Meta *meta, rr::Cell *cell) {
+    rr::Cell next{};
+    int64_t next_start = 0;
+    int32_t st = meta->status;
+    if (st == rr::OK) {
+        const uint64_t q = meta->n_rows ? (uint64_t)meta->end_q : (uint64_t)meta->start;
+        st = rr::chain_end(d, nout, q, next, next_start);
+    }
+    if (st != rr::OK) {
+        next = rr::Cell{};
+        meta->n_rows = 0;
+    }
+    meta->status = st;
+    meta->next_start = next_start;
+    *cell = next;
+}
+
+__global__ __launch_bounds__(256) void k_memfirst(const dcr_bgzf_member *m, int32_t n_members, const uint32_t *roff,
+                                                 const rr::Meta *meta, uint32_t *memfirst) {
+    const int32_t i = (int32_t)(blockIdx.x * blockDim.x + threadIdx.x);
+    if (i > n_members) return;
+    const uint32_t n_rows = meta->n_rows;
+    memfirst[i] = i == n_members ? n_rows : rr::lower_bound(roff, n_rows, (uint64_t)m[i].out_off);
+}
+
+inline bool enqueue(hipStream_t s, const uint8_t *d, uint64_t nout, const dcr_bgzf_member *d_m, int32_t n_members,
+                    const Work &W, rr::Cell *d_cell, const rr::Cfg &cfg) {
+    const uint32_t nb = (uint32_t)((nout + kTile - 1) / kTile);
+    const uint64_t bound = std::min<uint64_t>(kCap, nout / 36 + 1);
+    const uint32_t nbc = (uint32_t)((bound + kTile - 1) / kTile);
+    int rounds = 1;
+    while (((uint64_t)1 << rounds) < bound + 1) ++rounds;
+    hipLaunchKernelGGL(k_begin, dim3(1), dim3(1), 0, s, d, nout, d_cell, W.meta);
+    if (nb) {
+        hipLaunchKernelGGL(k_cand_count, dim3(nb), dim3(64), 0, s, d, nout, cfg.n_ref, W.bcnt);
+        hipLaunchKernelGGL(k_scan, dim3(1), dim3(1024), 0, s, W.bcnt, nb, kCap, &W.meta->n_cand, W.meta);
+        hipLaunchKernelGGL(k_cand_write, dim3(nb), dim3(64), 0, s, d, nout, cfg.n_ref, W.bcnt, W.meta, W.cand);
+    }
+    hipLaunchKernelGGL(k_link, dim3(kGrid), dim3(256), 0, s, d, W.cand, W.meta, W.jump[0], W.jump[1], W.reach);
+    hipLaunchKernelGGL(k_seed, dim3(1), dim3(1), 0, s, W.cand, nout, W.meta, W.reach);
+    for (int r = 0; r < rounds; ++r)
+        hipLaunchKernelGGL(k_double, dim3(kGrid), dim3(256), 0, s, W.jump[r & 1], W.jump[(r + 1) & 1], W.reach, W.meta);
+    hipLaunchKernelGGL(k_reach_count, dim3(nbc), dim3(64), 0, s, W.reach, W.meta, W.bcnt);
+    hipLaunchKernelGGL(k_scan, dim3(1), dim3(1024), 0, s, W.bcnt, nbc, kCap, &W.meta->n_rows, W.meta);
+    hipLaunchKernelGGL(k_rows_write, dim3(nbc), dim3(64), 0, s, d, W.cand, W.reach, W.bcnt, cfg, W.meta, W.rows, W.roff);
+    hipLaunchKernelGGL(k_end, dim3(1), dim3(1), 0, s, d, nout, W.meta, d_cell);
+    if (n_members > 0)
+        hipLaunchKernelGGL(k_memfirst, dim3((unsigned)(n_members + 256) / 256), dim3(256), 0, s, d_m, n_members, W.roff,
+                           W.meta, W.memfirst);
+    return hipGetLastError() == hipSuccess;
+}
+
+}
+
 struct InflSlots {
     static constexpr int kSlots = 4;
     uint8_t *d_in[kSlots] = {}, *d_out[kSlots] = {}, *d_st[kSlots] = {};
@@ -548,7 +809,32 @@
     size_t cap_stage[kSlots] = {}, cap_hst[kSlots] = {};
     hipStream_t s_k = nullptr, s_out = nullptr;
     bool busy = false;
+    rrd::Work rw[kSlots];
+    uint8_t *h_rmeta[kSlots] = {};
+    rr::Cell *d_cell = nullptr;
+    bool rows_ready = false;
+    static constexpr size_t kRmeta = sizeof(rr::Meta) + ((size_t)dcr_span::kSpanMembers + 1) * 4;
+    bool rows_alloc() {
+        if (rows_ready) return true;
+        bool ok = hipMalloc((void **)&d_cell, sizeof(rr::Cell)) == hipSuccess;
+        for (int i = 0; ok && i < kSlots; ++i)
+            ok = rw[i].alloc() && hipHostMalloc((void **)&h_rmeta[i], kRmeta, hipHostMallocDefault) == hipSuccess;
+        if (!ok) rows_release();
+        rows_ready = ok;
+        return ok;
+    }
+    void rows_release() {
+        for (int i = 0; i < kSlots; ++i) {
+            rw[i].release();
+            if (h_rmeta[i]) (void)hipHostFree(h_rmeta[i]);
+            h_rmeta[i] = nullptr;
+        }
+        if (d_cell) (void)hipFree(d_cell);
+        d_cell = nullptr;
+        rows_ready = false;
+    }
     void release() {
+        rows_release();
         for (int i = 0; i < kSlots; ++i) {
             if (d_in[i]) (void)hipFree(d_in[i]);
             if (d_out[i]) (void)hipFree(d_out[i]);
@@ -759,6 +1045,19 @@
     using Event = hipEvent_t;
     dcr_inflater *h;
     InflSlots &S;
+    static constexpr bool kRows = true;
+    bool rows_on = false;
+    rr::Cfg rcfg{};
+    const rr::Meta &rows_meta(int slot) const { return *(const rr::Meta *)S.h_rmeta[slot]; }
+    uint32_t rows_count(int slot) const { return rows_meta(slot).status == rr::OK ? rows_meta(slot).n_rows : 0; }
+    bool rows_declined(int slot) const { return rows_meta(slot).status != rr::OK; }
+    uint32_t rows_first(int slot, int32_t i) const {
+        return ((const uint32_t *)(S.h_rmeta[slot] + sizeof(rr::Meta)))[i];
+    }
+    bool rows_copy_out(dcr_rec_row *dst, int slot, uint32_t first, uint32_t count) {
+        return hipMemcpyAsync(dst, S.rw[slot].rows + first, (size_t)count * sizeof(dcr_rec_row), hipMemcpyDeviceToHost,
+                              S.s_out) == hipSuccess;
+    }
     bool new_events(Event &start, Event &done) {
         return hipEventCreateWithFlags(&done, hipEventBlockingSync) == hipSuccess &&
                hipEventCreate(&start) == hipSuccess;
@@ -793,8 +1092,17 @@
             return false;
         hipLaunchKernelGGL(dinf::k_inflate, dim3((unsigned)std::min(n, h->grid_cap)), dim3(64), sizeof(dinf::WaveLds),
                            S.s_k, a);
-        return hipGetLastError() == hipSuccess &&
-               hipMemcpyAsync(S.h_st[slot], S.d_st[slot], (size_t)n, hipMemcpyDeviceToHost, S.s_k) == hipSuccess &&
+        if (hipGetLastError() != hipSuccess) return false;
+        if (rows_on) {
+            const uint64_t nout = (uint64_t)(rel[n - 1].out_off + (int64_t)rel[n - 1].isize);
+            if (!rrd::enqueue(S.s_k, S.d_out[slot], nout, S.d_m[slot], n, S.rw[slot], S.d_cell, rcfg) ||
+                hipMemcpyAsync(S.h_rmeta[slot], S.rw[slot].meta, sizeof(rr::Meta), hipMemcpyDeviceToHost, S.s_k) !=
+                    hipSuccess ||
+                hipMemcpyAsync(S.h_rmeta[slot] + sizeof(rr::Meta), S.rw[slot].memfirst, ((size_t)n + 1) * 4,
+                               hipMemcpyDeviceToHost, S.s_k) != hipSuccess)
+                return false;
+        }
+        return hipMemcpyAsync(S.h_st[slot], S.d_st[slot], (size_t)n, hipMemcpyDeviceToHost, S.s_k) == hipSuccess &&
                hipEventRecord(done, S.s_k) == hipSuccess;
     }
     bool wait(Event start, Event done, float *ms) {
@@ -878,6 +1186,81 @@
     return st->s.fetch(out_off, n, dst);
 }
 
+extern "C" int dcr_inflate_stream_rows_begin(dcr_inflate_stream *st, int64_t start_off, int32_t n_ref,
+                                             int32_t min_map_quality, int32_t min_base_quality) {
+    if (!st || start_off < 0 || n_ref < 0) return -1;
+    dcr_inflater *h = st->be.h;
+    InflSlots &S = *h->slots;
+    (void)hipSetDevice(h->device);
+    {
+        std::lock_guard<std::mutex> g(st->s.mu);
+        if (!st->s.m.empty() || st->s.err) return -1;
+    }
+    if (!S.rows_alloc()) return -1;
+    rr::Cell c{};
+    c.start = start_off;
+    c.valid = 1;
+    if (hipMemcpy(S.d_cell, &c, sizeof c, hipMemcpyHostToDevice) != hipSuccess) return -1;
+    st->be.rcfg = rr::Cfg{n_ref, min_map_quality, min_base_quality};
+    st->be.rows_on = true;
+    return 0;
+}
+
+extern "C" int dcr_inflate_stream_fetch_rows(dcr_inflate_stream *st, int64_t out_off, int64_t n, uint8_t *dst,
+                                             dcr_rec_row *rows, int64_t rows_cap, dcr_rows_info *info) {
+    if (!st || n < 0 || (n && !dst) || !info || rows_cap < 0 || (rows_cap && !rows)) return -1;
+    (void)hipSetDevice(st->be.h->device);
+    *info = dcr_rows_info{};
+    dcr_span::RowSink sink{rows, rows_cap, info};
+    return st->s.fetch(out_off, n, dst, st->be.rows_on ? &sink : nullptr);
+}
+
+extern "C" int dcr_inflater_rec_rows(dcr_inflater *h, const uint8_t *bytes, int64_t n, int64_t start_off,
+                                     const uint8_t *part, int32_t n_ref, int32_t min_map_quality,
+                                     int32_t min_base_quality, dcr_rec_row *rows, int64_t cap, int64_t *out4) {
+    if (!h || n < 0 || (n && !bytes) || start_off < -4 || (start_off < 0 && !part) || n_ref < 0 || cap < 0 || (cap && !rows) || !out4 ||
+        (uint64_t)n > dcr_span::kSpanOut)
+        return -dcr::set_error(DCR_EARG, "dcr_inflater_rec_rows: bad arguments");
+    std::lock_guard<std::mutex> g(h->mu);
+    hipError_t e;
+    if ((e = hipSetDevice(h->device)) != hipSuccess) return -hip_fail(e, "hipSetDevice");
+    rrd::Work W;
+    uint8_t *d = nullptr;
+    rr::Cell *d_cell = nullptr;
+    int rc = 0;
+    rr::Meta meta{};
+    rr::Cell c{};
+    c.start = start_off < 0 ? 0 : start_off;
+    c.valid = 1;
+    if (start_off < 0) {
+        c.npart = (int32_t)(-1 - start_off);
+        for (int i = 0; i < c.npart; ++i) c.part[i] = part[i];
+    }
+    hipStream_t s = h->stream;
+    if (!W.alloc() || hipMalloc((void **)&d, (size_t)n + 16) != hipSuccess ||
+        hipMalloc((void **)&d_cell, sizeof c) != hipSuccess) {
+        rc = -dcr::set_error(DCR_EHIP, "dcr_inflater_rec_rows: device buffers");
+    } else if ((e = hipMemcpyAsync(d, bytes, (size_t)n, hipMemcpyHostToDevice, s)) != hipSuccess ||
+               (e = hipMemcpyAsync(d_cell, &c, sizeof c, hipMemcpyHostToDevice, s)) != hipSuccess ||
+               !rrd::enqueue(s, d, (uint64_t)n, nullptr, 0, W, d_cell, rr::Cfg{n_ref, min_map_quality, min_base_quality}) ||
+               (e = hipMemcpyAsync(&meta, W.meta, sizeof meta, hipMemcpyDeviceToHost, s)) != hipSuccess ||
+               (e = hipStreamSynchronize(s)) != hipSuccess) {
+        rc = -hip_fail(e, "dcr_inflater_rec_rows");
+    } else {
+        const int64_t k = std::min<int64_t>(cap, meta.status == rr::OK ? (int64_t)meta.n_rows : 0);
+        if (k > 0 && (e = hipMemcpy(rows, W.rows, (size_t)k * sizeof(dcr_rec_row), hipMemcpyDeviceToHost)) != hipSuccess)
+            rc = -hip_fail(e, "dcr_inflater_rec_rows: download");
+        out4[0] = meta.status;
+        out4[1] = meta.status == rr::OK ? (int64_t)meta.n_rows : 0;
+        out4[2] = meta.n_cand;
+        out4[3] = meta.next_start;
+    }
+    W.release();
+    if (d) (void)hipFree(d);
+    if (d_cell) (void)hipFree(d_cell);
+    return rc;
+}
+
 extern "C" void dcr_inflate_stream_close(dcr_inflate_stream *st) {
     if (!st) return;
     st->s.close();
@@ -897,6 +1280,13 @@
     return dcr_inflate_stream_fetch((dcr_inflate_stream *)s, off, n, dst);
 }
 static void hook_stream_close(void *s) { dcr_inflate_stream_close((dcr_inflate_stream *)s); }
+static int hook_stream_rows_begin(void *s, int64_t start_off, int32_t n_ref, int32_t mq, int32_t bq) {
+    return dcr_inflate_stream_rows_begin((dcr_inflate_stream *)s, start_off, n_ref, mq, bq);
+}
+static int hook_stream_fetch_rows(void *s, int64_t off, int64_t n, uint8_t *dst, dcr_rec_row *rows, int64_t cap,
+                                  dcr_rows_info *info) {
+    return dcr_inflate_stream_fetch_rows((dcr_inflate_stream *)s, off, n, dst, rows, cap, info);
+}
 
 static int hook_run(void *u, const uint8_t *in, int64_t in_bytes, const dcr_bgzf_member *m, int32_t n, uint8_t *out,
                     int64_t out_bytes) {
@@ -937,6 +1327,8 @@
     hook->stream_add = hook_stream_add;
     hook->stream_fetch = hook_stream_fetch;
     hook->stream_close = hook_stream_close;
+    hook->stream_rows_begin = hook_stream_rows_begin;
+    hook->stream_fetch_rows = hook_stream_fetch_rows;
     return 0;
 }
 
diff --git a/duplexumiconsensusreads_amd/csrc/dcr_ingest.cpp b/duplexumiconsensusreads_amd/csrc/dcr_ingest.cpp
--- a/duplexumiconsensusreads_amd/csrc/dcr_ingest.cpp
+++ b/duplexumiconsensusreads_amd/csrc/dcr_ingest.cpp
@@ -19,6 +19,7 @@
 #include "../../include/dcr_io.h"
 #include "../../include/dcr_inflate.h"
 #include "dcr_host.h"
+#include "dcr_rec_rows.h"
 
 using namespace dcrh;
 
@@ -434,7 +435,100 @@
     std::vector<Run> runs;
     std::vector<std::vector<Run>> item_runs;
     std::vector<size_t> item_at;
+    dcr_rec_row *rows = nullptr;
+    dcr_rows_info rinfo{};
 };
+
+inline void rec_from_row(const dcr_rec_row &w, size_t off, Rec &rc) {
+    rc.off = off;
+    rc.len = w.len;
+    rc.tid = w.tid;
+    rc.pos = w.pos;
+    rc.flag = w.flag;
+    rc.n_cig = w.n_cig;
+    rc.mapq = w.mapq;
+    rc.l_seq = w.l_seq;
+    rc.o_cig = 36u + w.l_rn;
+    rc.o_seq = rc.o_cig + 4u * w.n_cig;
+    rc.o_qual = rc.o_seq + (uint32_t)((w.l_seq + 1) >> 1);
+    rc.o_mi = w.o_mi;
+    rc.o_rx = w.o_rx;
+    rc.l_mi = w.l_mi;
+    rc.l_rx = w.l_rx;
+    rc.mi_type = w.mi_type;
+    rc.rx_type = w.rx_type;
+    rc.l_code = w.l_code;
+    rc.pf = w.pf;
+    rc.fmsg = w.fmsg;
+    rc.perr = w.perr;
+    rc.eqx = w.eqx;
+    {
+        const bool rev = w.flag & 16, r1 = w.flag & 64, r2 = w.flag & 128;
+        rc.subk = (int8_t)((!rev && r1) ? 0 : (!rev && r2) ? 1 : (rev && r1) ? 2 : (rev && r2) ? 3 : -1);
+    }
+    rc.end_kept = (int64_t)w.pos + w.l_seq - w.clip;
+    std::memcpy(rc.code, w.code, sizeof rc.code);
+}
+struct RowCursor {
+    const dcr_rec_row *rows;
+    const dcr_rows_info &info;
+    int s = 0;
+    int64_t j = 0;
+    RowCursor(const dcr_rec_row *r, const dcr_rows_info &in, int64_t first) : rows(r), info(in) {
+        while (s < info.n_seg) {
+            const dcr_rows_seg &g = info.seg[s];
+            const dcr_rec_row *a = rows + g.first;
+            if (g.count > 0 && g.base + (int64_t)a[g.count - 1].off >= first) {
+                int64_t lo = 0, hi = g.count;
+                while (lo < hi) {
+                    const int64_t mid = lo + (hi - lo) / 2;
+                    if (g.base + (int64_t)a[mid].off < first) lo = mid + 1;
+                    else hi = mid;
+                }
+                j = lo;
+                return;
+            }
+            ++s;
+        }
+    }
+    const dcr_rec_row *at(int64_t off) {
+        while (s < info.n_seg) {
+            const dcr_rows_seg &g = info.seg[s];
+            const dcr_rec_row *a = rows + g.first;
+            while (j < g.count && g.base + (int64_t)a[j].off < off) ++j;
+            if (j < g.count) return g.base + (int64_t)a[j].off == off ? &a[j++] : nullptr;
+            ++s;
+            j = 0;
+        }
+        return nullptr;
+    }
+};
+inline void row_from_rec(const Rec &rc, uint32_t off, uint8_t l_rn, dcr_rec_row &w) {
+    std::memset(&w, 0, sizeof w);
+    w.off = off;
+    w.len = rc.len;
+    w.tid = rc.tid;
+    w.pos = rc.pos;
+    w.l_seq = rc.l_seq;
+    w.flag = rc.flag;
+    w.n_cig = rc.n_cig;
+    w.l_rn = l_rn;
+    w.mapq = rc.mapq;
+    w.perr = rc.perr;
+    if (rc.perr) return;
+    w.clip = (int32_t)((int64_t)rc.pos + rc.l_seq - rc.end_kept);
+    w.o_mi = rc.o_mi;
+    w.o_rx = rc.o_rx;
+    w.l_mi = rc.l_mi;
+    w.l_rx = rc.l_rx;
+    w.l_code = rc.l_code;
+    w.mi_type = rc.mi_type;
+    w.rx_type = rc.rx_type;
+    w.fmsg = rc.fmsg;
+    w.eqx = rc.eqx;
+    w.pf = rc.pf;
+    std::memcpy(w.code, rc.code, sizeof w.code);
+}
 
 class RecsCache {
   public:
@@ -596,8 +690,10 @@
             }).detach();
         }
         if (hook_.host_free) {
-            for (auto &c : chunks_)
+            for (auto &c : chunks_) {
                 if (c.pin) hook_.host_free(hook_.user, c.pin);
+                if (c.rows) hook_.host_free(hook_.user, c.rows);
+            }
             if (stage_pin_) hook_.host_free(hook_.user, stage_pin_);
         }
         for (auto &c : chunks_) RecsCache::get().give(c);
@@ -611,7 +707,81 @@
         if (!stream_) return;
         stream_out_ = 0;
         const size_t p0 = cbeg_, p_end = cend_;
+        rows_begin(p0, p_end);
         mth_ = std::thread([this, p0, p_end] { scan_members(p0, p_end); });
+    }
+    static constexpr size_t kRowsCap = kWantGpu / 192;
+    static constexpr size_t kHeaderMax = (size_t)16 << 20;
+    void rows_begin(size_t p, const size_t cend) {
+        if (!hook_.stream_rows_begin || !hook_.stream_fetch_rows || !hook_.host_alloc || host_every_ > 1) return;
+        int64_t start = -1;
+        int32_t n_ref = 0x7fffffff;
+        if (st_ == kRec) {
+            start = (int64_t)skip_;
+        } else {
+            std::vector<uint8_t> hd;
+            size_t need = 12;
+            int stage = 0;
+            size_t at = 0;
+            int32_t left = 0;
+            while (start < 0 && hd.size() < kHeaderMax) {
+                while (hd.size() >= need && start < 0) {
+                    if (stage == 0) {
+                        if (std::memcmp(hd.data(), "BAM\1", 4) != 0 || rdi32(hd.data() + 4) < 0) return;
+                        at = 8 + (size_t)rdi32(hd.data() + 4);
+                        need = at + 4;
+                        stage = 1;
+                    } else if (stage == 1) {
+                        n_ref = rdi32(hd.data() + at);
+                        if (n_ref < 0) return;
+                        left = n_ref;
+                        at += 4;
+                        stage = 2;
+                        need = at + (left ? 4 : 0);
+                        if (!left) start = (int64_t)at;
+                    } else {
+                        const int32_t ln = rdi32(hd.data() + at);
+                        if (ln < 0) return;
+                        if (hd.size() < at + 8 + (size_t)ln) { need = at + 8 + (size_t)ln; break; }
+                        at += 8 + (size_t)ln;
+                        if (--left == 0) start = (int64_t)at;
+                        else need = at + 4;
+                    }
+                }
+                if (start >= 0) break;
+                if (p + 18 > cend) return;
+                const uint8_t *h = map_ + p;
+                if (h[0] != 0x1f || h[1] != 0x8b || h[2] != 8 || !(h[3] & 4)) return;
+                const size_t xlen = rd16(h + 10);
+                if (cend - p < 12 + xlen) return;
+                long bsize = -1;
+                for (size_t i = 0; i + 4 <= xlen;) {
+                    const uint8_t *sf = h + 12 + i;
+                    const size_t slen = rd16(sf + 2);
+                    if (sf[0] == 66 && sf[1] == 67 && slen == 2) bsize = rd16(sf + 4);
+                    i += 4 + slen;
+                }
+                if (bsize < 0) return;
+                const size_t blen = (size_t)bsize + 1;
+                if (blen < 12 + xlen + 8 || cend - p < blen) return;
+                const uint32_t isize = rd32(h + blen - 4);
+                if (isize > 0x10000) return;
+                const size_t old = hd.size();
+                hd.resize(old + isize);
+                size_t got = 0;
+                if (isize && (libdeflate_deflate_decompress(tl_dec.get(), h + 12 + xlen, blen - 12 - xlen - 8,
+                                                            hd.data() + old, isize, &got) != 0 || got != isize))
+                    return;
+                p += blen;
+            }
+            if (start < 0) return;
+        }
+        if (hook_.stream_rows_begin(stream_, start, n_ref, rp_.min_map_quality, rp_.min_base_quality) != 0) return;
+        for (auto &c : chunks_) {
+            c.rows = (dcr_rec_row *)hook_.host_alloc(hook_.user, kRowsCap * sizeof(dcr_rec_row));
+            if (!c.rows) return;
+        }
+        rows_on_ = true;
     }
     bool host_chunk(size_t k) const { return host_every_ > 1 && k % (size_t)host_every_ == (size_t)host_every_ - 1; }
     void scan_members(size_t p, const size_t cend) {
@@ -680,6 +850,7 @@
         cv_.notify_all();
     }
     double scan_s = 0, index_parse_s = 0, runs_s = 0;
+    std::atomic<int64_t> row_spans{0}, row_spans_declined{0}, row_recs{0}, row_recs_host{0};
 
   private:
     void loop() {
@@ -833,8 +1004,25 @@
         if (c.item_runs.size() < items) c.item_runs.resize(items);
         spool_->run(items, [&](size_t k) {
             const size_t b = k * chunk, e = std::min(offs_.size(), (k + 1) * chunk);
-            for (size_t i = b; i < e; ++i)
-                c.recs[i].perr = (uint8_t)rp_.parse_at(base, kHead + offs_[i], c.recs[i]);
+            if (c.rinfo.n_seg > 0) {
+                RowCursor cur(c.rows, c.rinfo, (int64_t)offs_[b]);
+                int64_t used = 0;
+                for (size_t i = b; i < e; ++i) {
+                    const dcr_rec_row *w = cur.at((int64_t)offs_[i]);
+                    if (w && (i + 1 >= offs_.size() || offs_[i] + w->len == offs_[i + 1])) {
+                        rec_from_row(*w, kHead + offs_[i], c.recs[i]);
+                        ++used;
+                    } else {
+                        c.recs[i].perr = (uint8_t)rp_.parse_at(base, kHead + offs_[i], c.recs[i]);
+                    }
+                }
+                row_recs.fetch_add(used, std::memory_order_relaxed);
+                row_recs_host.fetch_add((int64_t)(e - b) - used, std::memory_order_relaxed);
+            } else {
+                for (size_t i = b; i < e; ++i)
+                    c.recs[i].perr = (uint8_t)rp_.parse_at(base, kHead + offs_[i], c.recs[i]);
+                if (rows_on_) row_recs_host.fetch_add((int64_t)(e - b), std::memory_order_relaxed);
+            }
             std::vector<Run> &L = c.item_runs[k];
             L.clear();
             for (size_t i = b; i < e; ++i) {
@@ -900,6 +1088,7 @@
     }
     void fill(Chunk &c) {
         c.len = 0;
+        c.rinfo.n_seg = 0;
         c.eof = false;
         c.err.clear();
         struct Blk { size_t coff, clen, doff; uint32_t isize, crc; };
@@ -965,7 +1154,14 @@
             ok = pool_->run(blks.size(), host_inflate);
         } else if (stream_ && !blks.empty()) {
             const size_t out_blocks = blks.back().doff + blks.back().isize - kHead;
-            const int rc = hook_.stream_fetch(stream_, stream_out_, (int64_t)out_blocks, dst + kHead);
+            c.rinfo.n_seg = 0;
+            const int rc = rows_on_ ? hook_.stream_fetch_rows(stream_, stream_out_, (int64_t)out_blocks, dst + kHead,
+                                                              c.rows, (int64_t)kRowsCap, &c.rinfo)
+                                    : hook_.stream_fetch(stream_, stream_out_, (int64_t)out_blocks, dst + kHead);
+            if (rows_on_ && rc == 0) {
+                row_spans += c.rinfo.spans_rows;
+                row_spans_declined += c.rinfo.spans_declined;
+            }
             if (rc != 0) {
                 c.err = rc > 0 ? "BGZF block failed to inflate or CRC mismatch" : "GPU inflate failed";
                 return;
@@ -1054,6 +1250,7 @@
     std::thread mth_;
     std::atomic<bool> stop_members_{false};
     int64_t stream_out_ = 0;
+    bool rows_on_ = false;
     double frac_ = 0.5;
     int host_every_ = 0;
     size_t fill_k_ = 0;
@@ -2213,6 +2410,102 @@
     return DCR_IO_OK;
 }
 
+int dcr_ingest_rec_rows(dcr_ingest *ing, int64_t *out4) {
+    if (!ing || !out4 || !ing->infl) return fail(DCR_IO_EARG, "NULL argument");
+    out4[0] = ing->infl->row_spans.load();
+    out4[1] = ing->infl->row_spans_declined.load();
+    out4[2] = ing->infl->row_recs.load();
+    out4[3] = ing->infl->row_recs_host.load();
+    return DCR_IO_OK;
+}
+
+int64_t dcr_rec_rows_host_parse(const uint8_t *buf, int64_t n, const int64_t *offs, int64_t n_offs,
+                                int32_t min_map_quality, int32_t min_base_quality, dcr_rec_row *rows) {
+    if (!buf || n < 0 || n_offs < 0 || (n_offs && (!offs || !rows))) return -1;
+    RecParser rp;
+    rp.min_map_quality = min_map_quality;
+    rp.min_base_quality = min_base_quality;
+    for (int64_t i = 0; i < n_offs; ++i) {
+        if (offs[i] < 0 || offs[i] + 36 > n || offs[i] + 4 + (int64_t)(uint32_t)rdi32(buf + offs[i]) > n) return -1;
+        Rec r{};
+        r.perr = (uint8_t)rp.parse_at(buf, (size_t)offs[i], r);
+        row_from_rec(r, (uint32_t)offs[i], buf[offs[i] + 12], rows[i]);
+    }
+    return n_offs;
+}
+
+int64_t dcr_rec_rows_model(const uint8_t *buf, int64_t n, int64_t start_off, const uint8_t *part, int32_t n_ref,
+                           int32_t min_map_quality, int32_t min_base_quality, dcr_rec_row *rows, int64_t cap,
+                           int64_t *out4) {
+    if (!buf || n < 0 || start_off < -4 || (start_off < 0 && !part) || n_ref < 0 || cap < 0 || (cap && !rows) || !out4 ||
+        n > 0x7fffffff)
+        return -1;
+    const uint64_t nout = (uint64_t)n;
+    if (start_off < 0) {
+        rr::Cell c{};
+        c.valid = 1;
+        c.npart = (int32_t)(-1 - start_off);
+        for (int i = 0; i < c.npart; ++i) c.part[i] = part[i];
+        if (!rr::chain_start(buf, nout, c, start_off)) {
+            out4[0] = rr::NO_START;
+            out4[1] = out4[2] = out4[3] = 0;
+            return 0;
+        }
+    }
+    std::vector<uint32_t> cand;
+    for (uint64_t p = 0; p + 4 <= nout; ++p) {
+        const uint32_t bs = rr::ld32(buf + p);
+        if (rr::plausible(buf, nout, p, bs, n_ref)) cand.push_back((uint32_t)p);
+    }
+    const uint32_t nc = (uint32_t)cand.size();
+    std::vector<uint32_t> j0(nc + 1, nc), j1(nc + 1, nc);
+    std::vector<uint8_t> reach(nc + 1, 0);
+    for (uint32_t i = 0; i < nc; ++i) {
+        const uint64_t q = (uint64_t)cand[i] + 4 + rr::ld32(buf + cand[i]);
+        const uint32_t j = rr::lower_bound(cand.data(), nc, q);
+        j0[i] = (j < nc && cand[j] == q) ? j : nc;
+    }
+    uint32_t seed = nc;
+    if ((uint64_t)start_off < nout) {
+        const uint32_t s = rr::lower_bound(cand.data(), nc, (uint64_t)start_off);
+        if (s < nc && cand[s] == (uint64_t)start_off) {
+            seed = s;
+            reach[s] = 1;
+        }
+    }
+    int rounds = 1;
+    while (((uint64_t)1 << rounds) < (uint64_t)nc + 1) ++rounds;
+    for (int r = 0; r < rounds; ++r) {
+        const std::vector<uint8_t> was = reach;
+        for (uint32_t i = 0; i < nc; ++i) {
+            const uint32_t j = j0[i];
+            if (j < nc && was[i]) reach[j] = 1;
+            j1[i] = j < nc ? j0[j] : nc;
+        }
+        j0.swap(j1);
+    }
+    (void)seed;
+    const rr::Cfg cfg{n_ref, min_map_quality, min_base_quality};
+    int64_t n_rows = 0;
+    uint64_t q = (uint64_t)start_off;
+    for (uint32_t i = 0; i < nc; ++i) {
+        if (!reach[i]) continue;
+        dcr_rec_row w;
+        rr::row_parse(buf + cand[i], cand[i], cfg, w);
+        if (n_rows < cap) rows[n_rows] = w;
+        ++n_rows;
+        q = (uint64_t)cand[i] + w.len;
+    }
+    rr::Cell next{};
+    int64_t next_start = 0;
+    const int32_t st = rr::chain_end(buf, nout, q, next, next_start);
+    out4[0] = st;
+    out4[1] = st == rr::OK ? n_rows : 0;
+    out4[2] = nc;
+    out4[3] = next_start;
+    return out4[1];
+}
+
 int dcr_py_sample(uint32_t *mt, int32_t *index, int32_t n, int32_t k, int32_t *out) {
     if (!mt || !index || !out || n < 0 || k < 0 || k > n) return fail(DCR_IO_EARG, "bad sample arguments");
     PyRandom r;
diff --git a/duplexumiconsensusreads_amd/csrc/dcr_rec_rows.h b/duplexumiconsensusreads_amd/csrc/dcr_rec_rows.h
--- /dev/null
+++ b/duplexumiconsensusreads_amd/csrc/dcr_rec_rows.h
@@ -0,0 +1,286 @@
+#ifndef DCR_REC_ROWS_H
+#define DCR_REC_ROWS_H
+
+#include <cstdint>
+
+#include "../../include/dcr_inflate.h"
+
+#if defined(__HIPCC__)
+#define DCR_RR_HD __host__ __device__ inline
+#else
+#define DCR_RR_HD inline
+#endif
+
+namespace rr {
+
+struct Cfg {
+    int32_t n_ref, min_map_quality, min_base_quality;
+};
+
+enum : int32_t {
+    OK = 0,
+    NO_START = 1,
+    OVERFLOW = 2,
+    BAD_RECORD = 3,
+};
+
+struct Cell {
+    int64_t start;
+    int32_t valid;
+    int32_t npart;
+    uint8_t part[4];
+    int32_t pad;
+};
+
+struct Meta {
+    int32_t status;
+    uint32_t n_rows, n_cand;
+    uint32_t seed;
+    int64_t start;
+    int64_t end_q;
+    int64_t next_start;
+};
+
+DCR_RR_HD uint32_t ld32(const uint8_t *p) {
+    return (uint32_t)p[0] | ((uint32_t)p[1] << 8) | ((uint32_t)p[2] << 16) | ((uint32_t)p[3] << 24);
+}
+DCR_RR_HD uint32_t ld16(const uint8_t *p) { return (uint32_t)p[0] | ((uint32_t)p[1] << 8); }
+
+DCR_RR_HD bool plausible(const uint8_t *d, uint64_t nout, uint64_t p, uint32_t bs, int32_t n_ref) {
+    if (bs < 32 || bs > 0x7fffffffu || p + 4 + (uint64_t)bs > nout) return false;
+    const uint8_t *r = d + p + 4;
+    const int32_t tid = (int32_t)ld32(r), ntid = (int32_t)ld32(r + 20), l_seq = (int32_t)ld32(r + 16);
+    if (tid < -1 || tid >= n_ref || ntid < -1 || ntid >= n_ref || l_seq < 0) return false;
+    const uint32_t l_rn = r[8], n_cig = ld16(r + 12);
+    if (l_rn < 1) return false;
+    const uint64_t need = 32 + (uint64_t)l_rn + 4 * (uint64_t)n_cig + (((uint64_t)l_seq + 1) >> 1) + (uint64_t)l_seq;
+    if (need > bs) return false;
+    return r[32 + l_rn - 1] == 0;
+}
+
+DCR_RR_HD uint32_t lower_bound(const uint32_t *a, uint32_t n, uint64_t v) {
+    uint32_t lo = 0, hi = n;
+    while (lo < hi) {
+        const uint32_t mid = lo + ((hi - lo) >> 1);
+        if ((uint64_t)a[mid] < v) lo = mid + 1;
+        else hi = mid;
+    }
+    return lo;
+}
+
+DCR_RR_HD int32_t chain_end(const uint8_t *d, uint64_t nout, uint64_t q, Cell &next, int64_t &next_start) {
+    next.valid = 1;
+    next.npart = 0;
+    next.start = 0;
+    next.pad = 0;
+    for (int i = 0; i < 4; ++i) next.part[i] = 0;
+    if (q >= nout) {
+        next.start = (int64_t)(q - nout);
+        next_start = next.start;
+        return OK;
+    }
+    if (q + 4 > nout) {
+        next.npart = (int32_t)(nout - q);
+        for (int i = 0; i < next.npart; ++i) next.part[i] = d[q + (uint64_t)i];
+        next_start = -1 - next.npart;
+        return OK;
+    }
+    const uint32_t bs = ld32(d + q);
+    if (bs >= 32 && bs <= 0x7fffffffu && q + 4 + (uint64_t)bs > nout) {
+        next.start = (int64_t)(q + 4 + (uint64_t)bs - nout);
+        next_start = next.start;
+        return OK;
+    }
+    next.valid = 0;
+    next_start = 0;
+    return BAD_RECORD;
+}
+
+DCR_RR_HD bool chain_start(const uint8_t *d, uint64_t nout, const Cell &c, int64_t &start) {
+    if (!c.valid) return false;
+    if (c.npart == 0) {
+        start = c.start;
+        return true;
+    }
+    if ((uint64_t)(4 - c.npart) > nout) return false;
+    uint8_t b[4];
+    for (int i = 0; i < 4; ++i) b[i] = i < c.npart ? c.part[i] : d[i - c.npart];
+    const uint32_t bs = ld32(b);
+    if (bs < 32 || bs > 0x7fffffffu) return false;
+    start = (int64_t)(4 - c.npart) + (int64_t)bs;
+    return true;
+}
+
+DCR_RR_HD int32_t clip_total(const uint8_t *c, int n) {
+    if (n == 0) return 0;
+    const int first = 0, last = n - 1;
+    int32_t c5 = 0;
+    const int op0 = (int)(ld32(c) & 15);
+    if (op0 == 4) c5 = (int32_t)(ld32(c) >> 4);
+    else if (op0 == 5 && n > 1 && (ld32(c + 4) & 15) == 4) c5 = (int32_t)(ld32(c + 4) >> 4);
+    const int i5 = op0 == 4 ? first : first + 1;
+    int c3i = -1;
+    const int opl = (int)(ld32(c + 4 * last) & 15);
+    if (opl == 4) c3i = last;
+    else if (opl == 5 && n > 1) c3i = last - 1;
+    int32_t c3 = 0;
+    if (c3i >= first && (ld32(c + 4 * c3i) & 15) == 4 && !(c5 > 0 && c3i == i5)) c3 = (int32_t)(ld32(c + 4 * c3i) >> 4);
+    return c5 + c3;
+}
+
+DCR_RR_HD bool eqx_after_trim(const uint8_t *c, uint32_t n_cig, int32_t l_seq, const uint8_t *sq, const uint8_t *ql,
+                              int min_base_quality) {
+    bool any = false;
+    for (uint32_t i = 0; i < n_cig; ++i) {
+        const uint32_t op = ld32(c + 4 * i) & 15;
+        any |= (op == 7 || op == 8);
+    }
+    if (!any || l_seq == 0) return false;
+    int32_t s5 = 0, s3 = 0;
+    bool inseq = false;
+    int64_t expanded = 0;
+    for (uint32_t i = 0; i < n_cig; ++i) {
+        const uint32_t w = ld32(c + 4 * i), op = w & 15, ln = w >> 4;
+        if (op == 5) continue;
+        if (op == 4) {
+            if (!inseq) s5 = (int32_t)ln; else s3 = (int32_t)ln;
+        } else {
+            inseq = true;
+            expanded += ln;
+        }
+    }
+    int32_t b = s5, e = l_seq - s3;
+    if (s3 == 0) e = l_seq;
+    if (e < b) e = b;
+    int32_t tn = 0;
+    for (int32_t i = e - 1; i >= b; --i) {
+        const int code = (sq[i >> 1] >> ((i & 1) ? 0 : 4)) & 15;
+        if (code == 15 || (int)ql[i] < min_base_quality) ++tn;
+        else break;
+    }
+    int64_t keep = expanded - tn;
+    if (keep < 0) {
+        keep = expanded + keep;
+        if (keep < 0) keep = 0;
+    }
+    int64_t pos = 0;
+    for (uint32_t i = 0; i < n_cig && pos < keep; ++i) {
+        const uint32_t w = ld32(c + 4 * i), op = w & 15, ln = w >> 4;
+        if (op == 4 || op == 5) continue;
+        if (op == 7 || op == 8) return true;
+        pos += ln;
+    }
+    return false;
+}
+
+DCR_RR_HD void row_parse(const uint8_t *base, uint32_t off, const Cfg &cfg, dcr_rec_row &w) {
+    const uint8_t *r = base + 4;
+    w.off = off;
+    w.len = 4u + ld32(base);
+    w.tid = (int32_t)ld32(r);
+    w.pos = (int32_t)ld32(r + 4);
+    w.l_rn = r[8];
+    w.mapq = r[9];
+    w.n_cig = (uint16_t)ld16(r + 12);
+    w.flag = (uint16_t)ld16(r + 14);
+    w.l_seq = (int32_t)ld32(r + 16);
+    w.clip = 0;
+    w.o_mi = w.o_rx = 0;
+    w.l_mi = w.l_rx = w.l_code = 0;
+    w.mi_type = w.rx_type = 0;
+    w.fmsg = w.perr = w.eqx = 0;
+    w.pf = 0;
+    w.pad = 0;
+    for (int i = 0; i < 24; ++i) w.code[i] = 0;
+    if (w.l_seq < 0) { w.perr = 1; return; }
+    const uint32_t len = w.len;
+    const uint32_t o_cig = 36u + w.l_rn;
+    const uint32_t o_seq = o_cig + 4u * w.n_cig;
+    const uint32_t o_qual = o_seq + (uint32_t)((w.l_seq + 1) >> 1);
+    uint64_t p = (uint64_t)o_qual + (uint64_t)(uint32_t)w.l_seq;
+    if (p > len) { w.perr = 2; return; }
+    uint32_t o_mi = 0, o_rx = 0;
+    uint16_t l_mi = 0, l_rx = 0;
+    uint8_t mi_type = 0, rx_type = 0;
+    int perr = 0;
+    while (p + 3 <= len) {
+        const uint8_t t0 = base[p], t1 = base[p + 1], ty = base[p + 2];
+        const uint64_t v = p + 3;
+        uint64_t e = 0;
+        switch (ty) {
+            case 'A': case 'c': case 'C': e = v + 1; break;
+            case 's': case 'S': e = v + 2; break;
+            case 'i': case 'I': case 'f': e = v + 4; break;
+            case 'd': e = v + 8; break;
+            case 'Z': case 'H': {
+                uint64_t z = v;
+                while (z < len && base[z] != 0) ++z;
+                if (z >= len) perr = 3;
+                e = z + 1;
+                break;
+            }
+            case 'B': {
+                if (v + 5 > len) { perr = 4; break; }
+                const uint8_t sub = base[v];
+                const uint32_t n = ld32(base + v + 1);
+                const uint64_t es = (sub == 'c' || sub == 'C') ? 1 : (sub == 's' || sub == 'S') ? 2 : 4;
+                e = v + 5 + es * (uint64_t)n;
+                break;
+            }
+            default: perr = 5; break;
+        }
+        if (!perr && e > len) perr = 6;
+        if (perr) break;
+        if (t0 == 'M' && t1 == 'I' && !mi_type) {
+            mi_type = ty;
+            o_mi = (uint32_t)v;
+            l_mi = (uint16_t)(ty == 'Z' ? e - v - 1 : 0);
+        } else if (t0 == 'R' && t1 == 'X' && !rx_type) {
+            rx_type = ty;
+            o_rx = (uint32_t)v;
+            l_rx = (uint16_t)(ty == 'Z' ? e - v - 1 : 0);
+        }
+        p = e;
+    }
+    if (perr) { w.perr = (uint8_t)perr; return; }
+    w.o_mi = o_mi;
+    w.o_rx = o_rx;
+    w.l_mi = l_mi;
+    w.l_rx = l_rx;
+    w.mi_type = mi_type;
+    w.rx_type = rx_type;
+    uint16_t l_code = l_mi;
+    if (mi_type == 'Z')
+        for (uint32_t i = 0; i < l_mi; ++i)
+            if (base[o_mi + i] == '/') { l_code = (uint16_t)i; break; }
+    w.l_code = l_code;
+    if (mi_type == 'Z' && l_code <= 24)
+        for (uint32_t i = 0; i < l_code; ++i) w.code[i] = (char)base[o_mi + i];
+    const uint8_t *c = base + o_cig;
+    int msg = 0, pf = 0;
+    if (!mi_type) { msg = 1; pf = -1; }
+    else if (!rx_type) { msg = 2; pf = -1; }
+    else if (w.n_cig == 0) { msg = 3; pf = -1; }
+    else {
+        for (uint32_t i = 0; i < w.n_cig && !msg; ++i) {
+            const uint32_t op = ld32(c + 4 * i) & 15;
+            if (op == 3 || op == 6 || op >= 9) msg = 4;
+        }
+        for (uint32_t i = 1; i + 1 < w.n_cig && !msg; ++i)
+            if ((ld32(c + 4 * i) & 15) == 4) msg = 5;
+        if (msg) pf = -1;
+        else {
+            const uint32_t fl = w.flag;
+            pf = (fl & 1) && (fl & 2) && !(fl & 4) && !(fl & 8) && !(fl & 2048) && !(fl & 512) &&
+                 (int)w.mapq >= cfg.min_map_quality;
+        }
+    }
+    w.pf = (int8_t)pf;
+    w.fmsg = (uint8_t)msg;
+    w.clip = clip_total(c, (int)w.n_cig);
+    w.eqx = pf == 1 && eqx_after_trim(c, w.n_cig, w.l_seq, base + o_seq, base + o_qual, cfg.min_base_quality);
+}
+
+}
+
+#endif
diff --git a/duplexumiconsensusreads_amd/csrc/dcr_span_stream.h b/duplexumiconsensusreads_amd/csrc/dcr_span_stream.h
--- a/duplexumiconsensusreads_amd/csrc/dcr_span_stream.h
+++ b/duplexumiconsensusreads_amd/csrc/dcr_span_stream.h
@@ -9,6 +9,7 @@
 #include <mutex>
 #include <string>
 #include <thread>
+#include <type_traits>
 #include <vector>
 
 #include "../../include/dcr_inflate.h"
@@ -16,6 +17,17 @@
 namespace dcr_span {
 
 constexpr int kSlots = 4;
+
+struct RowSink {
+    dcr_rec_row *rows;
+    int64_t cap;
+    dcr_rows_info *info;
+    int64_t used = 0;
+};
+template <class B, class = void>
+struct has_rows : std::false_type {};
+template <class B>
+struct has_rows<B, std::void_t<decltype(B::kRows)>> : std::true_type {};
 
 constexpr int32_t kSpanMembers = 4096;
 constexpr size_t kSpanIn = (size_t)128 << 20;
@@ -153,7 +165,7 @@
         cv.notify_all();
     }
 
-    int fetch(int64_t out_off, int64_t n, uint8_t *dst) {
+    int fetch(int64_t out_off, int64_t n, uint8_t *dst, RowSink *sink = nullptr) {
         if (n == 0) return 0;
         const int64_t end = out_off + n;
         bool queued = false;
@@ -190,6 +202,8 @@
                     }
                 sp.checked = true;
                 be.account(ms, sp.m1 - sp.m0, 0);
+                if constexpr (has_rows<B>::value)
+                    if (sink) ++(be.rows_declined(slot) ? sink->info->spans_declined : sink->info->spans_rows);
             }
             if (sp.rc) {
                 be.error("BGZF member " + std::to_string(sp.rc - 1) + " failed to inflate or CRC mismatch");
@@ -198,6 +212,30 @@
             const int64_t a = std::max(out_off, sp.out0), b = std::min(end, sp.out1);
             if (!be.copy_out(dst + (a - out_off), slot, a - sp.out0, b - a)) return leave(-1);
             queued = true;
+            if constexpr (has_rows<B>::value) {
+                if (sink && sink->info->n_seg < DCR_ROWS_MAX_SEG && !be.rows_declined(slot)) {
+                    int32_t ia, ib;
+                    {
+                        std::lock_guard<std::mutex> g(mu);
+                        auto lb = [&](int64_t v) {
+                            return (int32_t)(std::lower_bound(m.begin() + sp.m0, m.begin() + sp.m1, v,
+                                                              [](const dcr_bgzf_member &x, int64_t y) {
+                                                                  return x.out_off < y;
+                                                              }) -
+                                             m.begin());
+                        };
+                        ia = lb(a);
+                        ib = b == sp.out1 ? sp.m1 : lb(b);
+                    }
+                    const uint32_t r0 = be.rows_first(slot, ia - sp.m0), r1 = be.rows_first(slot, ib - sp.m0);
+                    const int64_t cnt = std::min<int64_t>((int64_t)r1 - (int64_t)r0, sink->cap - sink->used);
+                    if (cnt > 0) {
+                        if (!be.rows_copy_out(sink->rows + sink->used, slot, r0, (uint32_t)cnt)) return leave(-1);
+                        sink->info->seg[sink->info->n_seg++] = dcr_rows_seg{sp.out0 - out_off, sink->used, cnt};
+                        sink->used += cnt;
+                    }
+                }
+            }
             if (b == sp.out1) {
                 if (!be.sync_out()) return -1;
                 queued = false;
diff --git a/duplexumiconsensusreads_amd/native_io.py b/duplexumiconsensusreads_amd/native_io.py
--- a/duplexumiconsensusreads_amd/native_io.py
+++ b/duplexumiconsensusreads_amd/native_io.py
@@ -110,6 +110,9 @@
             "dcr_io_set_inflate_hook": (_i32, [_vp]),
             "dcr_ingest_gpu_inflate": (_i32, [_vp]),
             "dcr_ingest_set_state_gate": (_i32, [_vp, _vp, _vp]),
+            "dcr_ingest_rec_rows": (_i32, [_vp, _vp]),
+            "dcr_rec_rows_host_parse": (_i64, [_vp, _i64, _vp, _i64, _i32, _i32, _vp]),
+            "dcr_rec_rows_model": (_i64, [_vp, _i64, _i64, ctypes.c_char_p, _i32, _i32, _i32, _vp, _i64, _vp]),
         }
         for name, (res, args) in sig.items():
             fn = getattr(lib, name)
@@ -301,6 +304,11 @@
         return dict(passed=int(out[0]), excluded=int(out[1]), processed=int(out[2]), filtered=int(out[3]),
                     records=int(out[4]))
 
+    def rec_rows(self):
+        out = np.zeros(4, np.int64)
+        load().dcr_ingest_rec_rows(self._h, out.ctypes.data)
+        return dict(spans=int(out[0]), declined=int(out[1]), from_rows=int(out[2]), host_parsed=int(out[3]))
+
     def close(self):
         if getattr(self, "_h", None):
             load().dcr_ingest_close(self._h)
diff --git a/include/dcr_inflate.h b/include/dcr_inflate.h
--- a/include/dcr_inflate.h
+++ b/include/dcr_inflate.h
@@ -17,6 +17,32 @@
     uint32_t pad;
 } dcr_bgzf_member;
 
+typedef struct dcr_rec_row {
+    uint32_t off;
+    uint32_t len;
+    int32_t tid, pos, l_seq;
+    int32_t clip;
+    uint32_t o_mi, o_rx;
+    uint16_t flag, n_cig, l_mi, l_rx, l_code;
+    uint8_t l_rn, mapq, mi_type, rx_type;
+    uint8_t fmsg, perr, eqx;
+    int8_t pf;
+    uint16_t pad;
+    char code[24];
+} dcr_rec_row;
+
+#define DCR_ROWS_MAX_SEG 64
+typedef struct dcr_rows_seg {
+    int64_t base, first, count;
+} dcr_rows_seg;
+typedef struct dcr_rows_info {
+    int32_t n_seg;
+    int32_t spans_rows;
+    int32_t spans_declined;
+    int32_t pad;
+    dcr_rows_seg seg[DCR_ROWS_MAX_SEG];
+} dcr_rows_info;
+
 typedef struct dcr_inflate_hook {
     void *user;
     int (*run)(void *user, const uint8_t *in, int64_t in_bytes, const dcr_bgzf_member *m, int32_t n, uint8_t *out,
@@ -27,7 +53,12 @@
     int (*stream_add)(void *stream, const dcr_bgzf_member *m, int32_t n, int32_t last);
     int (*stream_fetch)(void *stream, int64_t out_off, int64_t n, uint8_t *dst);
     void (*stream_close)(void *stream);
+    int (*stream_rows_begin)(void *stream, int64_t start_off, int32_t n_ref, int32_t min_map_quality,
+                             int32_t min_base_quality);
+    int (*stream_fetch_rows)(void *stream, int64_t out_off, int64_t n, uint8_t *dst, dcr_rec_row *rows,
+                             int64_t rows_cap, dcr_rows_info *info);
 } dcr_inflate_hook;
+
 
 typedef struct dcr_inflater dcr_inflater;
 dcr_inflater *dcr_inflater_create(int device);
@@ -40,6 +71,13 @@
 int dcr_inflate_stream_add(dcr_inflate_stream *st, const dcr_bgzf_member *m, int32_t n, int32_t last);
 int dcr_inflate_stream_fetch(dcr_inflate_stream *st, int64_t out_off, int64_t n, uint8_t *dst);
 void dcr_inflate_stream_close(dcr_inflate_stream *st);
+int dcr_inflate_stream_rows_begin(dcr_inflate_stream *st, int64_t start_off, int32_t n_ref, int32_t min_map_quality,
+                                  int32_t min_base_quality);
+int dcr_inflate_stream_fetch_rows(dcr_inflate_stream *st, int64_t out_off, int64_t n, uint8_t *dst,
+                                  dcr_rec_row *rows, int64_t rows_cap, dcr_rows_info *info);
+int dcr_inflater_rec_rows(dcr_inflater *h, const uint8_t *bytes, int64_t n, int64_t start_off, const uint8_t *part,
+                          int32_t n_ref, int32_t min_map_quality, int32_t min_base_quality, dcr_rec_row *rows,
+                          int64_t cap, int64_t *out4);
 int dcr_inflater_last(dcr_inflater *h, float *kernel_ms, int32_t *n_members);
 int dcr_inflater_totals(dcr_inflater *h, double *out4, int reset);
 
diff --git a/include/dcr_io.h b/include/dcr_io.h
--- a/include/dcr_io.h
+++ b/include/dcr_io.h
@@ -102,6 +102,13 @@
 struct dcr_inflate_hook;
 int dcr_io_set_inflate_hook(const struct dcr_inflate_hook *hook);
 int dcr_ingest_gpu_inflate(dcr_ingest *ing);
+int dcr_ingest_rec_rows(dcr_ingest *ing, int64_t *out4);
+struct dcr_rec_row;
+int64_t dcr_rec_rows_host_parse(const uint8_t *buf, int64_t n, const int64_t *offs, int64_t n_offs,
+                                int32_t min_map_quality, int32_t min_base_quality, struct dcr_rec_row *rows);
+int64_t dcr_rec_rows_model(const uint8_t *buf, int64_t n, int64_t start_off, const uint8_t *part, int32_t n_ref,
+                           int32_t min_map_quality, int32_t min_base_quality, struct dcr_rec_row *rows, int64_t cap,
+                           int64_t *out4);
 
 int dcr_split_points(const char *path, int32_t n_parts, const dcr_ingest_cfg *cfg, int64_t *voff);
 dcr_ingest *dcr_ingest_open_range(const char *path, const dcr_ingest_cfg *cfg, int64_t start_voff, int64_t end_voff);
```

Measured after the change: 439.0 million. 0.958x the previous value.
